# ilya16/MultINN

Measured on AMD Instinct MI355X. Metric: piano-roll timesteps/sec (train step), 5-track LSTM-NADE, higher is better.
Workload: dtype fp16; 1 GPU; TGT joint LSTM-NADE [1024,256,88,5]; global_batch=1024, per_gpu_batch=1024, seq_len=256, pitches=88, tracks=5, nade_hidden=256, optimizer=TF-Adam lr 0.01 eps 1e-4 clip 5.0, parallelism=dp1

## Files before the change

### include/multinn_hip.h

```cpp
#ifndef MULTINN_HIP_H
#define MULTINN_HIP_H

#include <stddef.h>
#include <stdint.h>

#ifdef __cplusplus
extern "C" {
#endif

#define MNN_OK 0
#define MNN_ERR_INVALID (-1)
#define MNN_ERR_HIP (-2)

typedef void* mnn_stream_t;

typedef enum { MNN_F32 = 0, MNN_BF16 = 1, MNN_U8 = 2, MNN_F16 = 3 } mnn_dtype;

enum { MNN_STREAM_DROPOUT = 0, MNN_STREAM_NADE = 1, MNN_STREAM_RBM_H = 2, MNN_STREAM_RBM_V = 3,
       MNN_STREAM_DBN_ENC = 4, MNN_STREAM_DBN_DEC = 5 };

#define MNN_ABI_VERSION 124
int mnn_version(void);
const char* mnn_last_error(void);

// ... 46 lines not shown
                     const void* wh_p, const float* gates, const float* c, const float* c0, float* dz,
                     void* dz_T , float* dh0, float* dc0, void* workspace, void* dzT_t, int ld_t,
                     float* db_p);

typedef struct { int units; const float* xproj; const void* wh_t; const void* h0; const float* c0; float* gates; float* c; void* h;
                 void* hT; int ld_hT; void* y; const uint8_t* mask; const void* wx_t; int ld_w; const float* bias_p;
                 void* yT; int ld_yT;
                 int xproj_bf16;
                 int f16;
               } mnn_lstm_fwd_layer;
typedef struct { int units; const float* dh_ext; const void* wh_p; const float* gates; const float* c; const float* c0; float* dz;
                 void* dz_T; void* workspace; void* dzT_t; int ld_t; float* db_p; const uint8_t* mask; const void* wx_p;
                 int f16;
               } mnn_lstm_bwd_layer;
int mnn_lstm2_seq_fwd(mnn_stream_t s, int T, int B, const mnn_lstm_fwd_layer* L1, const mnn_lstm_fwd_layer* L2, float keep_prob,
                      int s_begin, int s_end);
int mnn_lstm2_seq_bwd(mnn_stream_t s, int T, int B, const mnn_lstm_bwd_layer* L1, const mnn_lstm_bwd_layer* L2, float keep_prob,
                      int k_begin, int k_end);

int mnn_lstm2_persist_ok(int B, int units1, int units2);
int mnn_lstm_rows_gate_minor(mnn_stream_t s, int dtype, int units, int ld, const void* wx_t, const float* bias_p, void* wx_gm, float* bias_gm);
size_t mnn_lstm2_persist_workspace_bytes(int T, int B, int units1, int units2);
int mnn_lstm2_persist_status(const void* workspace, int B, int units1, int units2, int* status);
int mnn_lstm2_persist_fwd(mnn_stream_t s, int T, int B, const mnn_lstm_fwd_layer* L1, const mnn_lstm_fwd_layer* L2, float keep_prob,
                          void* workspace);
int mnn_lstm2_persist_bwd(mnn_stream_t s, int T, int B, const mnn_lstm_bwd_layer* L1, const mnn_lstm_bwd_layer* L2, float keep_prob,
                          void* workspace);
int mnn_lstm_rowpar_ok(int B, int units);
size_t mnn_lstm_rowpar_workspace_bytes(int T, int B, int units);
int mnn_lstm_rowpar_status(const void* workspace, int* status);
int mnn_lstm_rowpar_fwd(mnn_stream_t s, int T, int B, const mnn_lstm_fwd_layer* L, float keep_prob, void* workspace);
int mnn_lstm_rowpar_bwd(mnn_stream_t s, int T, int B, const mnn_lstm_bwd_layer* L, float keep_prob, void* workspace);
int mnn_lstm_resident_ok(int B, int units);
int mnn_lstm_resident_fwd(mnn_stream_t s, int T, int B, const mnn_lstm_fwd_layer* L, float keep_prob);
int mnn_lstm_resident_bwd(mnn_stream_t s, int T, int B, const mnn_lstm_bwd_layer* L, float keep_prob);
int mnn_lstm_resident_bwd_state(mnn_stream_t s, int T, int B, const mnn_lstm_bwd_layer* L, float keep_prob, float* dc0);
int mnn_lstm_cluster_ok(int B, int units);
int mnn_lstm_cluster_fwd(mnn_stream_t s, int T, int B, const mnn_lstm_fwd_layer* L, float keep_prob, void* workspace);
int mnn_lstm_cluster_bwd_ok(int B, int units);
int mnn_lstm_cluster_bwd(mnn_stream_t s, int T, int B, const mnn_lstm_bwd_layer* L, float keep_prob, void* workspace);
int mnn_lstm_cluster_bwd_state(mnn_stream_t s, int T, int B, const mnn_lstm_bwd_layer* L, float keep_prob, void* workspace, float* dc0);
int mnn_lstm_resident_fwd_multi(mnn_stream_t s, int T, int B, int njobs, const mnn_lstm_fwd_layer* L, float keep_prob);
int mnn_lstm_resident_bwd_multi(mnn_stream_t s, int T, int B, int njobs, const mnn_lstm_bwd_layer* L, float keep_prob);
int mnn_lstm_cluster_fwd_multi(mnn_stream_t s, int T, int B, int njobs, const mnn_lstm_fwd_layer* L, float keep_prob, void* const* workspaces);
int mnn_lstm_cluster_bwd_multi(mnn_stream_t s, int T, int B, int njobs, const mnn_lstm_bwd_layer* L, float keep_prob, void* const* workspaces);
int mnn_lstm_cluster_bwd_multi_ok(int B, int units, int njobs);
int mnn_lstm_resident_bwd_state_multi(mnn_stream_t s, int T, int B, int njobs, const mnn_lstm_bwd_layer* L, float keep_prob, float* const* dc0);
int mnn_lstm_cluster_bwd_state_multi(mnn_stream_t s, int T, int B, int njobs, const mnn_lstm_bwd_layer* L, float keep_prob, void* const* workspaces,
                                     float* const* dc0);
int mnn_dropout_mask(mnn_stream_t s, uint8_t* mask, int T, int B, int units, float keep_prob, uint64_t seed, const int32_t* step_dev,
                     uint32_t row0, int layer);

int mnn_dropout_fwd(mnn_stream_t s, int dtype, const void* h, void* y, int T, int B, int units, float keep_prob,
                    uint64_t seed, const int32_t* step_dev, uint32_t row0, int layer, int t_offset);
int mnn_dropout_bwd(mnn_stream_t s, const float* dy, float* dh, int T, int B, int units, float keep_prob, uint64_t seed,
                    const int32_t* step_dev, uint32_t row0, int layer, int accumulate, int t_offset);

int mnn_nade_mfma_ok(int Hn);
int mnn_nade_logprob_fwd_mfma(mnn_stream_t s, int tracks, int N, int D, int Hn, const uint8_t* v, long v_track_stride, const float* bias,
                              int ld_bias, const float* w_enc, const void* w_dec_bf16, const float* row_weight, float* nll, float* cond_p,
                              float* d_bias, float* a_final);
#define MNN_DENSITY_SLOTS 256
int mnn_density_gate(mnn_stream_t s, const uint8_t* v, long n, long threshold, int* gate, unsigned* count);
int mnn_nade_logprob_fwd_gated(mnn_stream_t s, int tracks, int N, int D, int Hn, const uint8_t* v, long v_track_stride,
                               const float* bias, int ld_bias, const float* w_enc, const float* w_dec, const float* row_weight,
                               float* nll, float* cond_p, float* d_bias, float* a_final, const int* gate, int run_if,
                               const int* n_rows_dev ,
                               int* unsafe );
int mnn_nade_logprob_fwd_mfma_gated(mnn_stream_t s, int tracks, int N, int D, int Hn, const uint8_t* v, long v_track_stride, const float* bias,
                                    int ld_bias, const float* w_enc, const void* w_dec_bf16, const float* row_weight, float* nll, float* cond_p,
                                    float* d_bias, float* a_final, const int* gate, int run_if, const int* n_rows_dev);
int mnn_nade_f32_pack(mnn_stream_t s, const float* w_dec, long rows, int Hn, float* w_dec_packed);
int mnn_nade_logprob_fwd_mfma_f32(mnn_stream_t s, int tracks, int N, int D, int Hn, const uint8_t* v, long v_track_stride, const float* bias,
                                  int ld_bias, const float* w_enc, const void* w_dec_packed, const float* row_weight, float* nll, float* cond_p,
                                  float* d_bias, float* a_final, const int* gate, int run_if, const int* n_rows_dev);

int mnn_nade_logprob_fwd(mnn_stream_t s, int tracks, int N, int D, int Hn, const uint8_t* v, long v_track_stride,
                         const float* bias, int ld_bias, const float* w_enc, const float* w_dec, const float* row_weight,
                         float* nll, float* cond_p, float* d_bias, float* a_final);
int mnn_nade_logprob_bwd(mnn_stream_t s, int tracks, int N, int D, int Hn, const uint8_t* v, long v_track_stride,
                         const float* bias, int ld_bias, const float* w_enc, const float* w_dec, const float* a_final,
                         float* d_bias, float* d_w_enc, float* d_w_dec, const int* n_rows_dev ,
                         const int* unsafe );
int mnn_nade_sample(mnn_stream_t s, int tracks, int N, int D, int Hn, const float* bias, int ld_bias, const float* w_enc,
                    const float* w_dec, float temperature, uint64_t seed, uint32_t row0, uint32_t sub, uint8_t* samples,
                    long s_track_stride, int s_row_stride, int s_elem_stride, float* nll, const uint8_t* given);
#define MNN_TEMPS_MAX 8
typedef struct {
    int n;
    int by_visible;
    float t[MNN_TEMPS_MAX];
} mnn_temps;
int mnn_nade_sample_temps(mnn_stream_t s, int tracks, int N, int D, int Hn, const float* bias, int ld_bias, const float* w_enc,
                          const float* w_dec, const mnn_temps* temps, uint64_t seed, uint32_t row0, uint32_t sub, uint8_t* samples,
                          long s_track_stride, int s_row_stride, int s_elem_stride, float* nll, const uint8_t* given);
typedef struct {
    const float* bias; int ld_bias;
    const float* w_enc; const float* w_dec;
    uint64_t seed;
    uint8_t* samples; float* nll;
    const uint8_t* given;
} mnn_nade_sample_job;
int mnn_nade_sample_multi(mnn_stream_t s, int njobs, const mnn_nade_sample_job* jobs, int N, int D, int Hn, float temperature,
                          uint32_t row0, uint32_t sub, long s_row_stride, int s_elem_stride);
int mnn_nade_sample_multi_temps(mnn_stream_t s, int njobs, const mnn_nade_sample_job* jobs, int N, int D, int Hn, const mnn_temps* temps,
                                uint32_t row0, uint32_t sub, long s_row_stride, int s_elem_stride);

size_t mnn_rbm_workspace_bytes(int D, int Hn);
int mnn_rbm_gibbs(mnn_stream_t s, int N, int D, int Hn, int k, const uint8_t* v0, const float* W, const float* bh, int ld_bh,
                  const float* bv, int ld_bv, uint64_t seed, uint32_t row0, const uint32_t* row_ids, uint32_t sub0,
                  float* p_v, uint8_t* v_out, void* workspace, const uint8_t* given, int ld_given);
int mnn_rbm_gibbs_temp(mnn_stream_t s, int N, int D, int Hn, int k, const uint8_t* v0, const float* W, const float* bh, int ld_bh,
                       const float* bv, int ld_bv, uint64_t seed, uint32_t row0, const uint32_t* row_ids, uint32_t sub0,
                       float* p_v, uint8_t* v_out, void* workspace, const uint8_t* given, int ld_given, float temperature);
int mnn_rbm_gibbs_stepped(mnn_stream_t s, int N, int D, int Hn, int k, const uint8_t* v0, const float* W, const float* bh, int ld_bh,
                  const float* bv, int ld_bv, uint64_t seed, uint32_t row0, const uint32_t* row_ids, uint32_t sub0,
                  float* p_v, uint8_t* v_out, void* workspace, const int* seed_step);
int mnn_rbm_hidden(mnn_stream_t s, int N, int D, int Hn, const void* v, int v_dtype, const float* W, const float* bh,
                   int ld_bh, int stream_id, uint64_t seed, uint32_t row0, uint32_t sub, float* p_h, uint8_t* h);
int mnn_rbm_visible(mnn_stream_t s, int N, int D, int Hn, const void* h, int h_dtype, const float* W, const float* bv,
                    int ld_bv, int stream_id, uint64_t seed, uint32_t row0, uint32_t sub, float* p_v, uint8_t* v,
                    void* workspace);
int mnn_rbm_free_energy(mnn_stream_t s, int N, int D, int Hn, const uint8_t* v, const float* W, const float* bh, int ld_bh,
                        const float* bv, int ld_bv, float* F, float* p_h );
typedef struct {
    const float* W;
    const float* bh;
    const float* bv;
    uint64_t seed;
    const uint8_t* v0;
    float* p_v;
    uint8_t* v_out;
    const uint8_t* given;
} mnn_rbm_gibbs_job;
int mnn_rbm_gibbs_multi(mnn_stream_t s, int njobs, const mnn_rbm_gibbs_job* jobs, int N, int D, int Hn, int k, int ld_bh, int ld_bv,
                        uint32_t row0, const uint32_t* row_ids, uint32_t sub0, const int* seed_step, long row_stride, int elem_stride,
                        long given_row_stride, void* workspace);
int mnn_rbm_gibbs_multi_temps(mnn_stream_t s, int njobs, const mnn_rbm_gibbs_job* jobs, int N, int D, int Hn, int k, int ld_bh, int ld_bv,
                              uint32_t row0, const uint32_t* row_ids, uint32_t sub0, const int* seed_step, long row_stride, int elem_stride,
                              long given_row_stride, void* workspace, const float* temps);
typedef struct {
    const uint8_t* v;
    const float* W;
    const float* bh;
    const float* bv;
    float* F;
    float* p_h;
} mnn_rbm_free_energy_job;
int mnn_rbm_free_energy_multi(mnn_stream_t s, int njobs, const mnn_rbm_free_energy_job* jobs, int N, int D, int Hn, int ld_bh, int ld_bv);
int mnn_rbm_cd_bias_delta(mnn_stream_t s, int N, int D, int Hn, const uint8_t* v, const float* p_v, const uint8_t* h, const float* p_h,
                          float scale, float* dbv, float* dbh);
int mnn_axpby_f32(mnn_stream_t s, long n, float a, const float* x, float b, const float* y, float* out);
int mnn_rbm_visible_bias_init(mnn_stream_t s, int D, const float* colsum, float count, float* bv);
int mnn_rbm_cd_rows(mnn_stream_t s, int N, int D, int Hn, int ld, const uint8_t* v, const uint8_t* v_s, const float* sv, const float* ss,
                    const float* row_weight, float scale, float* d_out, float* pos, float* neg);

size_t mnn_rbm_ais_workspace_bytes(int N, int D, int Hn, int n_chains, int n_betas);
int mnn_rbm_ais(mnn_stream_t s, int N, int D, int Hn, int n_chains, int n_betas, const float* betas, const float* W, const float* bh, int ld_bh,
                const float* bv, int ld_bv, uint64_t seed, uint32_t row0, const uint32_t* row_ids, float* log_z, float* log_w, uint8_t* v_out,
                float* stats, void* workspace);

int mnn_rbm_raise(mnn_stream_t s, int N, int D, int Hn, int n_chains, int n_betas, const float* betas, const float* W, const float* bh, int ld_bh,
                  const float* bv, int ld_bv, const uint8_t* v, uint64_t seed, uint32_t row0, const uint32_t* row_ids, float* log_z, float* log_w,
                  uint8_t* v_out, float* stats, void* workspace);

int mnn_sigmoid_grad_f32(mnn_stream_t s, long n, const float* dy, const float* y, float* dz);
// ... 76 lines not shown
```

### multinn_amd/_lib.py

```python
import ctypes as C
import os

HERE = os.path.dirname(os.path.abspath(__file__))
LIB_PATH = os.environ.get("MULTINN_HIP_LIB", os.path.join(HERE, "libmultinn_hip.so"))

ABI_VERSION = 124
F32, BF16, U8, F16 = 0, 1, 2, 3
GEMM_ACCUMULATE, GEMM_ATOMIC, GEMM_A_KBLOCK32 = 1, 2, 8

_p, _i, _l, _f, _u64, _u32, _sz = C.c_void_p, C.c_int, C.c_long, C.c_float, C.c_uint64, C.c_uint32, C.c_size_t

SIGNATURES = {
    "mnn_version": (_i, []),
    "mnn_last_error": (C.c_char_p, []),
    "mnn_gemm_tn": (_i, [_p, _i, _i, _i, _i, _p, _i, _p, _i, _p, _i, _i, _p, _i, _i]),
    "mnn_gemm_tn_rows": (_i, [_p, _i, _i, _i, _i, _p, _i, _p, _i, _p, _i, _i, _p, _i, _i, _p, _p]),
    "mnn_transpose": (_i, [_p, _p, _i, _i, _i, _i, _p, _i, _i]),
    "mnn_convert2d": (_i, [_p, _p, _i, _i, _p, _i, _i, _i, _i]),
    "mnn_pianoroll_shift_timemajor": (_i, [_p, _p, _i, _i, _i, _p, _p, _i, _i, _p, _p, _l]),
    "mnn_pianoroll_shift_timemajor_t": (_i, [_p, _p, _i, _i, _i, _p, _p, _i, _p, _i, _p, _p, _l, _i, _p, _p, _p]),
    "mnn_ragged_index": (_i, [_p, _p, _i, _i, _p, _f, _p, _p, _p]),
    "mnn_rows_gather16": (_i, [_p, _p, _i, _p, _p, _i, _i, _p, _i, _p, _i]),
    "mnn_rows_scatter_f32": (_i, [_p, _p, _p, _p, _i, _i, _p]),
    "mnn_pianoroll_split_tracks": (_i, [_p, _p, _i, _i, _i, _i, _p]),
    "mnn_lstm_pack_weights": (_i, [_p, _p, _p, _i, _i, _i, _i, _p, _p, _p, _p, _p]),
    "mnn_lstm_unpack_grads": (_i, [_p, _p, _p, _p, _i, _i, _i, _p, _p]),
    "mnn_lstm_unpack_grads_consume": (_i, [_p, _p, _p, _p, _i, _i, _i, _p, _p]),
    "mnn_lstm_unpack_grads_cat": (_i, [_p, _p, _p, _i, _i, _i, _p, _p]),
    "mnn_lstm_seq_fwd": (_i, [_p, _i, _i, _i, _i, _i, _i, _p, _p, _p, _p, _p, _p, _p, _p, _i]),
    "mnn_lstm_fused_outputs": (_i, [_i, _i]),
    "mnn_lstm_seq_bwd_workspace_bytes": (_sz, [_i, _i]),
    "mnn_lstm_seq_bwd": (_i, [_p, _i, _i, _i, _i, _i, _i, _p, _p, _p, _p, _p, _p, _p, _p, _p, _p, _p, _i, _p]),
    "mnn_dropout_fwd": (_i, [_p, _i, _p, _p, _i, _i, _i, _f, _u64, _p, _u32, _i, _i]),
    "mnn_dropout_bwd": (_i, [_p, _p, _p, _i, _i, _i, _f, _u64, _p, _u32, _i, _i, _i]),
    "mnn_nade_logprob_fwd": (_i, [_p, _i, _i, _i, _i, _p, _l, _p, _i, _p, _p, _p, _p, _p, _p, _p]),
    "mnn_nade_logprob_bwd": (_i, [_p, _i, _i, _i, _i, _p, _l, _p, _i, _p, _p, _p, _p, _p, _p, _p, _p]),
    "mnn_nade_sample": (_i, [_p, _i, _i, _i, _i, _p, _i, _p, _p, _f, _u64, _u32, _u32, _p, _l, _i, _i, _p, _p]),
    "mnn_rbm_workspace_bytes": (_sz, [_i, _i]),
    "mnn_rbm_gibbs": (_i, [_p, _i, _i, _i, _i, _p, _p, _p, _i, _p, _i, _u64, _u32, _p, _u32, _p, _p, _p, _p, _i]),
    "mnn_rbm_gibbs_stepped": (_i, [_p, _i, _i, _i, _i, _p, _p, _p, _i, _p, _i, _u64, _u32, _p, _u32, _p, _p, _p, _p]),
    "mnn_rbm_hidden": (_i, [_p, _i, _i, _i, _p, _i, _p, _p, _i, _i, _u64, _u32, _u32, _p, _p]),
    "mnn_rbm_visible": (_i, [_p, _i, _i, _i, _p, _i, _p, _p, _i, _i, _u64, _u32, _u32, _p, _p, _p]),
    "mnn_rbm_free_energy": (_i, [_p, _i, _i, _i, _p, _p, _p, _i, _p, _i, _p, _p]),
    "mnn_sumsq": (_i, [_p, _p, _l, _p]),
    "mnn_weighted_sum": (_i, [_p, _p, _p, _l, _p]),
    "mnn_clip_adam_step": (_i, [_p, _p, _p, _p, _p, _l, _p, _f, _f, _f, _f, _f, _i, _p, _i, _p]),
    "mnn_step_increment": (_i, [_p, _p, _p, _f, _p, _p, _i]),
    "mnn_bias_grad": (_i, [_p, _p, _i, _i, _i, _p, _i]),
    "mnn_grad_rows_fanout": (_i, [_p, _p, _i, _i, _i, _i, _p, _i, _p, _i, _p, _i]),
    "mnn_fill_f32": (_i, [_p, _p, _l, _f]),
    "mnn_lstm_step_det": (_i, [_p, _i, _i, _p]),
    "mnn_dense_det": (_i, [_p, _i, _i, _p]),
    "mnn_nade_sample_multi": (_i, [_p, _i, _p, _i, _i, _i, _f, _u32, _u32, _l, _i]),
    "mnn_generate_scan_workspace_bytes": (_sz, [_i, _i, _i, _p, _i]),
    "mnn_det_lstm_pack_bytes": (_sz, [_i, _i]),
    "mnn_det_lstm_pack": (_i, [_p, _p, _i, _i, _p]),
    "mnn_det_dense_pack_bytes": (_sz, [_i, _i]),
    "mnn_det_dense_pack": (_i, [_p, _p, _i, _i, _i, _p]),
    "mnn_generate_scan": (_i, [_p, _i, _i, _i, _p, _i, _i, _p, _p, _p, _i, _i, _i, _i, _p, _p, _f, _u64, _u32, _p, _p, _sz, _p]),
    "mnn_generate_scan_state": (_i, [_p, _i, _i, _i, _p, _i, _i, _p, _p, _p, _i, _i, _i, _i, _p, _p, _f, _u64, _u32, _p, _p, _sz, _p,
                                     C.POINTER(C.c_void_p), C.POINTER(C.c_void_p)]),
    "mnn_comm_unique_id": (_i, [_p]),
    "mnn_comm_init": (_i, [C.POINTER(_p), _i, _i, _p]),
    "mnn_allreduce_flat": (_i, [_p, _p, _p, _l]),
    "mnn_comm_destroy": (_i, [_p]),
}

class DetLstmJob(C.Structure):
    _fields_ = [("x", _p), ("x_dtype", _i), ("n_x", _i), ("ld_x", _i), ("es_x", _i), ("x2", _p), ("n_x2", _i), ("ld_x2", _i), ("h_prev", _p), ("c_prev", _p),
                ("W", _p), ("bias", _p), ("c_out", _p), ("h_out", _p), ("units", _i), ("Wp", _p)]


class NadeSampleJob(C.Structure):
    _fields_ = [("bias", _p), ("ld_bias", _i), ("w_enc", _p), ("w_dec", _p), ("seed", _u64), ("samples", _p), ("nll", _p), ("given", _p)]


class Temps(C.Structure):
    _fields_ = [("n", _i), ("by_visible", _i), ("t", _f * 8)]


class RbmGibbsJob(C.Structure):
    _fields_ = [("W", _p), ("bh", _p), ("bv", _p), ("seed", _u64), ("v0", _p), ("p_v", _p), ("v_out", _p), ("given", _p)]


class RbmFreeEnergyJob(C.Structure):
    _fields_ = [("v", _p), ("W", _p), ("bh", _p), ("bv", _p), ("F", _p), ("p_h", _p)]


class ScanLstmLayer(C.Structure):
    _fields_ = [("W", _p), ("bias", _p), ("units", _i)]


class DetDenseJob(C.Structure):
    _fields_ = [("x", _p), ("ld_x", _i), ("K", _i), ("W", _p), ("ld_w", _i), ("N", _i), ("bias", _p), ("out", _p), ("ld_out", _i), ("Wp", _p)]


class LstmFwdLayer(C.Structure):
    _fields_ = [("units", _i), ("xproj", _p), ("wh_t", _p), ("h0", _p), ("c0", _p), ("gates", _p), ("c", _p), ("h", _p), ("hT", _p), ("ld_hT", _i), ("y", _p), ("mask", _p),
                ("wx_t", _p), ("ld_w", _i), ("bias_p", _p), ("yT", _p), ("ld_yT", _i), ("xproj_bf16", _i), ("f16", _i)]


class LstmBwdLayer(C.Structure):
    _fields_ = [("units", _i), ("dh_ext", _p), ("wh_p", _p), ("gates", _p), ("c", _p), ("c0", _p), ("dz", _p), ("dz_T", _p), ("workspace", _p),
                ("dzT_t", _p), ("ld_t", _i), ("db_p", _p), ("mask", _p), ("wx_p", _p), ("f16", _i)]


SIGNATURES["mnn_lstm2_seq_fwd"] = (_i, [_p, _i, _i, C.POINTER(LstmFwdLayer), C.POINTER(LstmFwdLayer), _f, _i, _i])
SIGNATURES["mnn_lstm2_seq_bwd"] = (_i, [_p, _i, _i, C.POINTER(LstmBwdLayer), C.POINTER(LstmBwdLayer), _f, _i, _i])
SIGNATURES["mnn_lstm_rows_gate_minor"] = (_i, [_p, _i, _i, _i, _p, _p, _p, _p])
SIGNATURES["mnn_lstm2_persist_ok"] = (_i, [_i, _i, _i])
SIGNATURES["mnn_lstm2_persist_workspace_bytes"] = (_sz, [_i, _i, _i, _i])
SIGNATURES["mnn_lstm2_persist_status"] = (_i, [_p, _i, _i, _i, C.POINTER(C.c_int)])
SIGNATURES["mnn_lstm2_persist_fwd"] = (_i, [_p, _i, _i, C.POINTER(LstmFwdLayer), C.POINTER(LstmFwdLayer), _f, _p])
SIGNATURES["mnn_lstm2_persist_bwd"] = (_i, [_p, _i, _i, C.POINTER(LstmBwdLayer), C.POINTER(LstmBwdLayer), _f, _p])
SIGNATURES["mnn_lstm_rowpar_ok"] = (_i, [_i, _i])
SIGNATURES["mnn_lstm_rowpar_workspace_bytes"] = (_sz, [_i, _i, _i])
SIGNATURES["mnn_lstm_rowpar_status"] = (_i, [_p, C.POINTER(C.c_int)])
SIGNATURES["mnn_lstm_rowpar_fwd"] = (_i, [_p, _i, _i, C.POINTER(LstmFwdLayer), _f, _p])
SIGNATURES["mnn_lstm_rowpar_bwd"] = (_i, [_p, _i, _i, C.POINTER(LstmBwdLayer), _f, _p])
SIGNATURES["mnn_lstm_resident_ok"] = (_i, [_i, _i])
SIGNATURES["mnn_lstm_resident_fwd"] = (_i, [_p, _i, _i, C.POINTER(LstmFwdLayer), _f])
SIGNATURES["mnn_lstm_resident_bwd"] = (_i, [_p, _i, _i, C.POINTER(LstmBwdLayer), _f])
SIGNATURES["mnn_lstm_cluster_ok"] = (_i, [_i, _i])
SIGNATURES["mnn_lstm_cluster_bwd_ok"] = (_i, [_i, _i])
SIGNATURES["mnn_lstm_cluster_bwd_multi_ok"] = (_i, [_i, _i, _i])
SIGNATURES["mnn_lstm_resident_fwd_multi"] = (_i, [_p, _i, _i, _i, C.POINTER(LstmFwdLayer), _f])
SIGNATURES["mnn_lstm_resident_bwd_multi"] = (_i, [_p, _i, _i, _i, C.POINTER(LstmBwdLayer), _f])
SIGNATURES["mnn_lstm_cluster_fwd_multi"] = (_i, [_p, _i, _i, _i, C.POINTER(LstmFwdLayer), _f, C.POINTER(C.c_void_p)])
SIGNATURES["mnn_lstm_cluster_bwd_multi"] = (_i, [_p, _i, _i, _i, C.POINTER(LstmBwdLayer), _f, C.POINTER(C.c_void_p)])
SIGNATURES["mnn_lstm_cluster_fwd"] = (_i, [_p, _i, _i, C.POINTER(LstmFwdLayer), _f, _p])
SIGNATURES["mnn_lstm_cluster_bwd"] = (_i, [_p, _i, _i, C.POINTER(LstmBwdLayer), _f, _p])
SIGNATURES["mnn_lstm_resident_bwd_state"] = (_i, [_p, _i, _i, C.POINTER(LstmBwdLayer), _f, _p])
SIGNATURES["mnn_lstm_cluster_bwd_state"] = (_i, [_p, _i, _i, C.POINTER(LstmBwdLayer), _f, _p, _p])
SIGNATURES["mnn_lstm_resident_bwd_state_multi"] = (_i, [_p, _i, _i, _i, C.POINTER(LstmBwdLayer), _f, C.POINTER(C.c_void_p)])
SIGNATURES["mnn_lstm_cluster_bwd_state_multi"] = (_i, [_p, _i, _i, _i, C.POINTER(LstmBwdLayer), _f, C.POINTER(C.c_void_p), C.POINTER(C.c_void_p)])
SIGNATURES["mnn_nade_mfma_ok"] = (_i, [_i])
SIGNATURES["mnn_nade_logprob_fwd_mfma"] = (_i, [_p, _i, _i, _i, _i, _p, _l, _p, _i, _p, _p, _p, _p, _p, _p, _p])
SIGNATURES["mnn_density_gate"] = (_i, [_p, _p, _l, _l, _p, _p])
SIGNATURES["mnn_nade_logprob_fwd_gated"] = (_i, [_p, _i, _i, _i, _i, _p, _l, _p, _i, _p, _p, _p, _p, _p, _p, _p, _p, _i, _p, _p])
SIGNATURES["mnn_nade_logprob_fwd_mfma_gated"] = (_i, [_p, _i, _i, _i, _i, _p, _l, _p, _i, _p, _p, _p, _p, _p, _p, _p, _p, _i, _p])
SIGNATURES["mnn_nade_logprob_fwd_mfma_f32"] = (_i, [_p, _i, _i, _i, _i, _p, _l, _p, _i, _p, _p, _p, _p, _p, _p, _p, _p, _i, _p])
SIGNATURES["mnn_nade_f32_pack"] = (_i, [_p, _p, _l, _i, _p])
SIGNATURES["mnn_musical_bar_stats"] = (_i, [_p, _p, _i, _i, _i, _i, _i, _p, _p, _p, _p, _p, _p, _p, _p])
SIGNATURES["mnn_musical_note_stats"] = (_i, [_p, _p, _i, _i, _i, _i, _i, _p, _p])
SIGNATURES["mnn_eval_counts"] = (_i, [_p, _p, _p, _l, _p])
SIGNATURES["mnn_log_loss_rows"] = (_i, [_p, _p, _p, _i, _i, _i, _p])
SIGNATURES["mnn_rbm_cd_bias_delta"] = (_i, [_p, _i, _i, _i, _p, _p, _p, _p, _f, _p, _p])
SIGNATURES["mnn_rbm_visible_bias_init"] = (_i, [_p, _i, _p, _f, _p])
SIGNATURES["mnn_sigmoid_grad_f32"] = (_i, [_p, _l, _p, _p, _p])
SIGNATURES["mnn_rbm_ais_workspace_bytes"] = (_sz, [_i, _i, _i, _i, _i])
SIGNATURES["mnn_rbm_ais"] = (_i, [_p, _i, _i, _i, _i, _i, _p, _p, _p, _i, _p, _i, _u64, _u32, _p, _p, _p, _p, _p, _p])
SIGNATURES["mnn_rbm_raise"] = (_i, [_p, _i, _i, _i, _i, _i, _p, _p, _p, _i, _p, _i, _p, _u64, _u32, _p, _p, _p, _p, _p, _p])
SIGNATURES["mnn_rbm_gibbs_multi"] = (_i, [_p, _i, _p, _i, _i, _i, _i, _i, _i, _u32, _p, _u32, _p, _l, _i, _l, _p])
SIGNATURES["mnn_rbm_free_energy_multi"] = (_i, [_p, _i, _p, _i, _i, _i, _i, _i])
SIGNATURES["mnn_rbm_cd_rows"] = (_i, [_p, _i, _i, _i, _i, _p, _p, _p, _p, _p, _f, _p, _p, _p])
SIGNATURES["mnn_probe_sigmoid"] = (_i, [_p, _i, _i, _p])
SIGNATURES["mnn_axpby_f32"] = (_i, [_p, _l, _f, _p, _f, _p, _p])
SIGNATURES["mnn_dropout_mask"] = (_i, [_p, _p, _i, _i, _i, _f, _u64, _p, _u32, _i])
SIGNATURES["mnn_nade_sample_temps"] = (_i, [_p, _i, _i, _i, _i, _p, _i, _p, _p, _p, _u64, _u32, _u32, _p, _l, _i, _i, _p, _p])
SIGNATURES["mnn_nade_sample_multi_temps"] = (_i, [_p, _i, _p, _i, _i, _i, _p, _u32, _u32, _l, _i])
SIGNATURES["mnn_generate_scan_temps"] = (_i, [_p, _i, _i, _i, _p, _i, _i, _p, _p, _p, _i, _i, _i, _i, _p, _p, _p, _u64, _u32, _p, _p, _sz, _p,
                                              C.POINTER(C.c_void_p), C.POINTER(C.c_void_p)])
SIGNATURES["mnn_rbm_gibbs_temp"] = (_i, [_p, _i, _i, _i, _i, _p, _p, _p, _i, _p, _i, _u64, _u32, _p, _u32, _p, _p, _p, _p, _i, _f])
SIGNATURES["mnn_rbm_gibbs_multi_temps"] = (_i, [_p, _i, _p, _i, _i, _i, _i, _i, _i, _u32, _p, _u32, _p, _l, _i, _l, _p, C.POINTER(C.c_float)])
TEMPS_MAX = 8

_lib = None


class MnnError(RuntimeError):
    pass


class MnnUnsupported(MnnError, NotImplementedError):
    """A request this build has no path for (e.g. conditional generation of a model that does not live on a ROCm device): caught by both
    `except MnnError` and `except NotImplementedError`."""


def load():
    global _lib
    if _lib is not None:
        return _lib
    if not os.path.exists(LIB_PATH):
        raise MnnError(f"{LIB_PATH} is missing: run `python -c 'import __graft_entry__ as g; g.build()'` "
                       "(multinn_amd has no CPU fallback)")
    lib = C.CDLL(LIB_PATH)
    for name, (res, args) in SIGNATURES.items():
        fn = getattr(lib, name)
        fn.restype, fn.argtypes = res, args
    if lib.mnn_version() != ABI_VERSION:
        raise MnnError(f"{LIB_PATH} has ABI version {lib.mnn_version()}, this loader binds {ABI_VERSION} (include/multinn_hip.h): rebuild it")
    _lib = lib
    return lib


def check(rc, what=""):
    if rc != 0:
        raise MnnError(f"{what} failed ({rc}): {load().mnn_last_error().decode()}")


TIMING = None


def call(name, *args):
    lib = load()
    if TIMING is not None:
        import torch
        e0, e1 = torch.cuda.Event(enable_timing=True), torch.cuda.Event(enable_timing=True)
        e0.record()
        rc = getattr(lib, name)(*args)
        e1.record()
        TIMING.setdefault(name, []).append((e0, e1))
    else:
        rc = getattr(lib, name)(*args)
    if rc != 0:
        raise MnnError(f"{name} failed ({rc}): {lib.mnn_last_error().decode()}")
```

### multinn_amd/csrc/nade.hip

```cpp
#include "common.h"

#define NADE_EPS 1e-6f
#define LN2 0.6931471805599453f

__device__ __forceinline__ float fast_ln(float x) { return __builtin_amdgcn_logf(x) * LN2; }

__device__ __forceinline__ bool nade_rows_beyond(const int* __restrict__ n_rows_dev, int first_row) {
    return n_rows_dev != nullptr && first_row >= *n_rows_dev;
}
__device__ __forceinline__ void nade_zero_rows(float* __restrict__ d_bias, int ld_bias, int col0, int ncol, int row0, int nrow, int N, int nthreads) {
    if (d_bias == nullptr) return;
    for (int e = threadIdx.x; e < nrow * ncol; e += nthreads) {
        const int n = e / ncol, i = e - n * ncol;
        if (row0 + n < N) d_bias[(size_t)(row0 + n) * ld_bias + col0 + i] = 0.f;
    }
}

__device__ __forceinline__ float dpp_xor8(float x) { return __int_as_float(__builtin_amdgcn_update_dpp(0, __float_as_int(x), 0x128, 0xf, 0xf, false)); }
__device__ __forceinline__ float swz_xor4(float x) { return __int_as_float(__builtin_amdgcn_ds_swizzle(__float_as_int(x), 0x101F)); }
__device__ __forceinline__ float dpp_xor4(float x) {
    int t = __builtin_amdgcn_update_dpp(0, __float_as_int(x), 0x104, 0xf, 0x5, false);
    t = __builtin_amdgcn_update_dpp(t, __float_as_int(x), 0x114, 0xf, 0xa, false);
    return __int_as_float(t);
}
__device__ __forceinline__ float dpp_xor2(float x) { return __int_as_float(__builtin_amdgcn_update_dpp(0, __float_as_int(x), 0x4E, 0xf, 0xf, false)); }
__device__ __forceinline__ float dpp_xor1(float x) { return __int_as_float(__builtin_amdgcn_update_dpp(0, __float_as_int(x), 0xB1, 0xf, 0xf, false)); }

__device__ __forceinline__ float rows8(float (&x)[8], int lane) {
#pragma unroll
    for (int k = 0; k < 4; ++k) {
        auto r = __builtin_amdgcn_permlane32_swap(__float_as_uint(x[k]), __float_as_uint(x[k + 4]), false, false);
        x[k] = __uint_as_float(r[0]) + __uint_as_float(r[1]);
    }
#pragma unroll
    for (int k = 0; k < 2; ++k) {
        auto r = __builtin_amdgcn_permlane16_swap(__float_as_uint(x[k]), __float_as_uint(x[k + 2]), false, false);
        x[k] = __uint_as_float(r[0]) + __uint_as_float(r[1]);
    }
    const float t = x[0] + dpp_xor8(x[0]), u = x[1] + dpp_xor8(x[1]);
    return (lane & 8) ? u : t;
}
__device__ __forceinline__ float vis8(float (&y)[8], int lane) {
    const bool b2 = lane & 4, b1 = lane & 2, b0 = lane & 1;
#pragma unroll
    for (int k = 0; k < 4; ++k) {
        const float t = y[k] + swz_xor4(y[k]), u = y[k + 4] + swz_xor4(y[k + 4]);
        y[k] = b2 ? u : t;
    }
#pragma unroll
    for (int k = 0; k < 2; ++k) {
        const float t = y[k] + dpp_xor2(y[k]), u = y[k + 2] + dpp_xor2(y[k + 2]);
        y[k] = b1 ? u : t;
    }
    const float t = y[0] + dpp_xor1(y[0]), u = y[1] + dpp_xor1(y[1]);
    return b0 ? u : t;
}

#define FWD_R 8
template <int HQ>
struct WStage {
    static constexpr int W = HQ * 64;
    static constexpr int NE = (8 * W) / 512;
    float rd[NE], re[NE];
    __device__ __forceinline__ void gload(const float* __restrict__ wd, const float* __restrict__ we, int i0, int D, int Hn, int ld = 0) {
        if (ld == 0) ld = Hn;
#pragma unroll
        for (int k = 0; k < NE; ++k) {
            const int e = threadIdx.x + k * 512;
            const int ii = e / W, j = e - ii * W, i = i0 + ii;
            const bool ok = i >= 0 && i < D && j < Hn;
            const size_t o = (size_t)min(max(i, 0), D - 1) * ld + min(j, Hn - 1);
            const float xd = wd[o], xe = we[o];
            rd[k] = ok ? xd : 0.f;
            re[k] = ok ? xe : 0.f;
        }
    }
    __device__ __forceinline__ void lstore(float* __restrict__ sd, float* __restrict__ se) const {
#pragma unroll
        for (int k = 0; k < NE; ++k) {
            sd[threadIdx.x + k * 512] = rd[k];
            se[threadIdx.x + k * 512] = re[k];
        }
    }
};

template <int HQ, bool UT>
__global__ void __launch_bounds__(512)
nade_fwd_kernel(int tracks, int N, int D, int Hn, const uint8_t* __restrict__ v, long v_track_stride, const float* __restrict__ bias,
                int ld_bias, const float* __restrict__ w_enc, const float* __restrict__ w_dec, const float* __restrict__ row_weight,
                float* __restrict__ nll, float* __restrict__ cond_p, float* __restrict__ d_bias, float* __restrict__ a_final,
                const int* __restrict__ gate, int run_if, const int* __restrict__ n_rows_dev, int* __restrict__ unsafe) {
    constexpr int W = HQ * 64;
    __shared__ float wl[2][2][8 * W];
    if (gate != nullptr && *gate != run_if) {
        if (unsafe != nullptr && blockIdx.x == 0 && blockIdx.y == 0 && threadIdx.x == 0) atomicAdd(unsafe, 1);
        return;
    }
    const int m = blockIdx.y;
    if (nade_rows_beyond(n_rows_dev, blockIdx.x * 64)) {
        nade_zero_rows(d_bias, ld_bias, tracks * Hn + m * D, D, blockIdx.x * 64, 64, N, 512);
        if (nll != nullptr && threadIdx.x < 64 && blockIdx.x * 64 + threadIdx.x < N) nll[(size_t)m * N + blockIdx.x * 64 + threadIdx.x] = 0.f;
        return;
    }
    const int lane = threadIdx.x & 63;
    const int w = __builtin_amdgcn_readfirstlane(threadIdx.x >> 6);
    const int rbase = blockIdx.x * 64 + w * FWD_R;
    const uint8_t* __restrict__ vm = v + (size_t)m * v_track_stride;
    const float* __restrict__ we = w_enc + (size_t)m * D * Hn;
    const float* __restrict__ wd = w_dec + (size_t)m * D * Hn;
    const int bd_off = tracks * Hn + m * D;

    float a[FWD_R][HQ], h[FWD_R][HQ];
#pragma unroll
    for (int r = 0; r < FWD_R; ++r)
#pragma unroll
        for (int q = 0; q < HQ; ++q)
            a[r][q] = bias[(size_t)min(rbase + r, N - 1) * ld_bias + m * Hn + min(lane + 64 * q, Hn - 1)];
#pragma unroll
    for (int r = 0; r < FWD_R; ++r)
#pragma unroll
        for (int q = 0; q < HQ; ++q) {
            const int j = lane + 64 * q, row = rbase + r;
            if (!(row < N && j < Hn)) a[r][q] = 0.f;
            h[r][q] = fast_sigmoid(a[r][q]);
        }
    float u[UT ? FWD_R : 1][UT ? HQ : 1];
    float amax = 0.f;
    bool passed40 = false;
    if constexpr (UT) {
#pragma unroll
        for (int r = 0; r < FWD_R; ++r)
#pragma unroll
            for (int q = 0; q < HQ; ++q) {
                u[r][q] = fast_exp2(-MNN_LOG2E * a[r][q]);
                amax = fmaxf(amax, fabsf(a[r][q]));
            }
    }
    const int frow = rbase + (lane >> 3), fi = lane & 7;
    const bool fvalid = frow < N;
    const int frr = fvalid ? frow : N - 1;
    const float rw = (row_weight != nullptr && fvalid) ? row_weight[frow] : 0.f;
    float lp = 0.f;

    WStage<HQ> st;
    st.gload(wd, we, 0, D, Hn);
    st.lstore(wl[0][0], wl[0][1]);
    bool vcur = fvalid && fi < D && vm[(size_t)frr * D + fi] != 0;
    float bcur = fi < D ? bias[(size_t)frr * ld_bias + bd_off + fi] : 0.f;
    __syncthreads();
    const int nch = (D + 7) / 8;
    for (int c = 0; c < nch; ++c) {
        const int i0 = c * 8;
        const int inext = i0 + 8 + fi;
        st.gload(wd, we, i0 + 8, D, Hn);
        const int inc = min(inext, D - 1);
        const uint8_t vraw = vm[(size_t)frr * D + inc];
        const float braw = bias[(size_t)frr * ld_bias + bd_off + inc];
        const unsigned long long mask = __ballot(vcur);
        const float* __restrict__ sd = wl[c & 1][0];
        const float* __restrict__ se = wl[c & 1][1];
        float y[8];
#pragma unroll
        for (int ii = 0; ii < 8; ++ii) {
            float wdv[HQ], pr[8];
#pragma unroll
            for (int q = 0; q < HQ; ++q) wdv[q] = sd[ii * W + lane + 64 * q];
            if constexpr (UT) {
                const bool any = (mask & (0x0101010101010101ull << ii)) != 0ull;
                float wev[HQ], ewv[HQ];
                if (any) {
#pragma unroll
                    for (int q = 0; q < HQ; ++q) {
                        wev[q] = se[ii * W + lane + 64 * q];
                        ewv[q] = fast_exp2(-MNN_LOG2E * wev[q]);
                    }
                }
#pragma unroll
                for (int r = 0; r < FWD_R; ++r) {
                    float acc = h[r][0] * wdv[0];
#pragma unroll
                    for (int q = 1; q < HQ; ++q) acc = fmaf(h[r][q], wdv[q], acc);
                    pr[r] = acc;
                    if ((mask >> (r * 8 + ii)) & 1ull) {
#pragma unroll
                        for (int q = 0; q < HQ; ++q) {
                            a[r][q] += wev[q];
                            u[r][q] *= ewv[q];
                            h[r][q] = fast_rcp(1.0f + u[r][q]);
                            amax = fmaxf(amax, fabsf(a[r][q]));
                        }
                    }
                }
                if (any && __any(amax > 40.0f)) {
                    amax = 0.f;
                    passed40 = true;
#pragma unroll
                    for (int r = 0; r < FWD_R; ++r)
#pragma unroll
                        for (int q = 0; q < HQ; ++q) {
                            u[r][q] = fast_exp2(-MNN_LOG2E * a[r][q]);
                            h[r][q] = fast_rcp(1.0f + u[r][q]);
                        }
                }
            } else {
#pragma unroll
                for (int r = 0; r < FWD_R; ++r) {
                    float acc = h[r][0] * wdv[0];
#pragma unroll
                    for (int q = 1; q < HQ; ++q) acc = fmaf(h[r][q], wdv[q], acc);
                    pr[r] = acc;
                    if ((mask >> (r * 8 + ii)) & 1ull) {
#pragma unroll
                        for (int q = 0; q < HQ; ++q) {
                            a[r][q] += se[ii * W + lane + 64 * q];
                            h[r][q] = fast_sigmoid(a[r][q]);
                        }
                    }
                }
            }
            y[ii] = rows8(pr, lane);
        }
        const float tot = vis8(y, lane);
        const int i = i0 + fi;
        if (i < D) {
            const float l = bcur + tot;
            const float pr = fast_sigmoid(l);
            const float qr = fast_sigmoid(-l);
            lp += vcur ? fast_ln(NADE_EPS + pr) : fast_ln(NADE_EPS + qr);
            if (fvalid) {
                if (cond_p != nullptr) cond_p[((size_t)m * N + frow) * D + i] = pr;
                if (d_bias != nullptr) {
                    const float dnll_dp = vcur ? -fast_rcp(NADE_EPS + pr) : fast_rcp(NADE_EPS + qr);
                    d_bias[(size_t)frow * ld_bias + bd_off + i] = rw * dnll_dp * pr * qr;
                }
            }
        }
        st.lstore(wl[(c + 1) & 1][0], wl[(c + 1) & 1][1]);
        vcur = fvalid && inext < D && vraw != 0;
        bcur = inext < D ? braw : 0.f;
        __syncthreads();
    }
    lp += dpp_xor1(lp);
    lp += dpp_xor2(lp);
    lp += swz_xor4(lp);
    if (fi == 0 && fvalid && nll != nullptr) nll[(size_t)m * N + frow] = -lp;
    if (a_final != nullptr) {
#pragma unroll
        for (int r = 0; r < FWD_R; ++r)
#pragma unroll
            for (int q = 0; q < HQ; ++q) {
                const int j = lane + 64 * q, row = rbase + r;
                if (row < N && j < Hn) a_final[((size_t)m * N + row) * Hn + j] = a[r][q];
            }
    }
    if (unsafe != nullptr) {
        const bool ok = UT ? !__any(passed40 || amax > 40.0f) : !(blockIdx.x == 0 && blockIdx.y == 0 && w == 0);
        if (!ok && lane == 0) atomicAdd(unsafe, 1);
    }
}

extern "C" int mnn_nade_logprob_fwd(mnn_stream_t s, int tracks, int N, int D, int Hn, const uint8_t* v, long v_track_stride,
                                    const float* bias, int ld_bias, const float* w_enc, const float* w_dec, const float* row_weight,
                                    float* nll, float* cond_p, float* d_bias, float* a_final) {
    return mnn_nade_logprob_fwd_gated(s, tracks, N, D, Hn, v, v_track_stride, bias, ld_bias, w_enc, w_dec, row_weight, nll, cond_p, d_bias, a_final,
                                      nullptr, 0, nullptr, nullptr);
}

extern "C" int mnn_nade_logprob_fwd_gated(mnn_stream_t s, int tracks, int N, int D, int Hn, const uint8_t* v, long v_track_stride,
                                          const float* bias, int ld_bias, const float* w_enc, const float* w_dec, const float* row_weight,
                                          float* nll, float* cond_p, float* d_bias, float* a_final, const int* gate, int run_if, const int* n_rows_dev,
                                          int* unsafe) {
    MNN_REQUIRE(tracks > 0 && N > 0 && D > 0 && Hn > 0 && Hn <= 256, "mnn_nade_logprob_fwd: need tracks,N,D>0 and 0<Hn<=256 (Hn=%d)", Hn);
    MNN_REQUIRE(v && bias && w_enc && w_dec, "mnn_nade_logprob_fwd: null pointer");
    MNN_REQUIRE(ld_bias >= tracks * (Hn + D), "mnn_nade_logprob_fwd: ld_bias %d < tracks*(Hn+D)", ld_bias);
    MNN_REQUIRE(d_bias == nullptr || row_weight != nullptr, "mnn_nade_logprob_fwd: d_bias needs row_weight");
    dim3 grid(cdiv(N, 64), tracks);
    hipStream_t st = (hipStream_t)s;
#define FWD(HQ, UT) hipLaunchKernelGGL((nade_fwd_kernel<HQ, UT>), grid, dim3(512), 0, st, tracks, N, D, Hn, v, v_track_stride, bias, ld_bias, w_enc, \
                                       w_dec, row_weight, nll, cond_p, d_bias, a_final, gate, run_if, n_rows_dev, unsafe)
    if (unsafe != nullptr) MNN_HIP(mnn_zero_async(unsafe, sizeof(int), sizeof(int), 1, st));
    static const bool no_ut = getenv("MNN_NADE_FWD_NO_UT") != nullptr;
    if (Hn <= 64) FWD(1, false);
    else if (Hn <= 128) FWD(2, false);
    else if (gate != nullptr && run_if == 1 && !no_ut) FWD(4, true);
    else FWD(4, false);
#undef FWD
    MNN_LAUNCH_CHECK();
    return MNN_OK;
}

template <int HQ> struct LaneVec;
template <> struct LaneVec<2> { typedef float2 T; };
template <> struct LaneVec<4> { typedef float4 T; };
template <int HQ>
__device__ __forceinline__ void lv_store(float* p, const float (&x)[HQ]) {
    if constexpr (HQ == 4) *reinterpret_cast<float4*>(p) = make_float4(x[0], x[1], x[2], x[3]);
    else *reinterpret_cast<float2*>(p) = make_float2(x[0], x[1]);
}
template <int HQ>
__device__ __forceinline__ void lv_load(const float* p, float (&x)[HQ]) {
    if constexpr (HQ == 4) { const float4 t = *reinterpret_cast<const float4*>(p); x[0] = t.x; x[1] = t.y; x[2] = t.z; x[3] = t.w; }
    else { const float2 t = *reinterpret_cast<const float2*>(p); x[0] = t.x; x[1] = t.y; }
}
template <int HQ>
__device__ __forceinline__ void bwd_gload(WStage<HQ>& st, const float* __restrict__ wd, const float* __restrict__ we, int i0, int D, int Hn, int ld) {
    if constexpr (HQ >= 2) {
        const int i = i0 + (int)__builtin_amdgcn_readfirstlane(threadIdx.x >> 6), l = threadIdx.x & 63;
        const int ic = min(max(i, 0), D - 1);
        const float* __restrict__ pd = wd + (size_t)ic * ld;
        const float* __restrict__ pe = we + (size_t)ic * ld;
#pragma unroll
        for (int q = 0; q < HQ; ++q) {
            const int col = min(l + 64 * q, Hn - 1);
            st.rd[q] = pd[col];
            st.re[q] = pe[col];
        }
    } else {
        st.gload(wd, we, i0, D, Hn, ld);
    }
}
template <int HQ>
__device__ __forceinline__ void bwd_lstore(const WStage<HQ>& st, float* __restrict__ sd, float* __restrict__ se) {
    if constexpr (HQ >= 2) {
        const int pos = (int)(threadIdx.x >> 6) * (64 * HQ) + HQ * (int)(threadIdx.x & 63);
        lv_store<HQ>(sd + pos, st.rd);
        lv_store<HQ>(se + pos, st.re);
    } else {
        st.lstore(sd, se);
    }
}

template <int HQ, int RG, bool USEU>
__global__ void __launch_bounds__(512)
nade_bwd_kernel(int tracks, int N, int D, int HnT, int nslice, const uint8_t* __restrict__ v, long v_track_stride, const float* __restrict__ bias,
                int ld_bias, const float* __restrict__ w_enc, const float* __restrict__ w_dec, const float* __restrict__ a_final,
                float* __restrict__ d_bias, float* __restrict__ d_w_enc, float* __restrict__ d_w_dec, const int* __restrict__ n_rows_dev,
                const int* __restrict__ unsafe) {
    constexpr int W = HQ * 64;
    __shared__ __attribute__((aligned(16))) float wl[2][2][8 * W];
    if (unsafe != nullptr && (*unsafe == 0) != USEU) return;
    constexpr int NRED = HQ <= 2 ? 2 : 1;
    __shared__ __attribute__((aligned(16))) float red_[NRED][8][4][2][W];
    const int m = blockIdx.y / nslice, hb = (blockIdx.y - m * nslice) * W;
    const int Hn = min(W, HnT - hb);
    if (nade_rows_beyond(n_rows_dev, blockIdx.x * (64 * RG))) {
        nade_zero_rows(d_bias, ld_bias, m * HnT + hb, Hn, blockIdx.x * (64 * RG), 64 * RG, N, 512);
        return;
    }
    const int Nv = n_rows_dev != nullptr ? min(*n_rows_dev, N) : N;
    const int lane = threadIdx.x & 63;
    const int w = __builtin_amdgcn_readfirstlane(threadIdx.x >> 6);
    constexpr int BWD_R = 8 * RG;
    const int rbase = blockIdx.x * (64 * RG) + w * BWD_R;
    const uint8_t* __restrict__ vm = v + (size_t)m * v_track_stride;
    const float* __restrict__ we = w_enc + (size_t)m * D * HnT + hb;
    const float* __restrict__ wd = w_dec + (size_t)m * D * HnT + hb;
    const int dl_off = tracks * HnT + m * D;

    constexpr bool useu = USEU;
    float a[BWD_R][HQ], h[BWD_R][HQ], c[BWD_R][HQ], G[BWD_R][HQ];
#pragma unroll
    for (int r = 0; r < BWD_R; ++r)
#pragma unroll
        for (int q = 0; q < HQ; ++q)
            a[r][q] = a_final[((size_t)m * N + min(rbase + r, N - 1)) * HnT + hb + min(lane + 64 * q, Hn - 1)];
#pragma unroll
    for (int r = 0; r < BWD_R; ++r)
#pragma unroll
        for (int q = 0; q < HQ; ++q) {
            const int j = lane + 64 * q, row = rbase + r;
            if (!(row < Nv && j < Hn)) a[r][q] = 0.f;
            h[r][q] = fast_sigmoid(a[r][q]);
            if constexpr (useu) a[r][q] = fast_exp2(-MNN_LOG2E * a[r][q]);
            G[r][q] = 0.f;
            c[r][q] = 0.f;
        }
    const int fi = lane & 7;
    int frr[RG];
    bool fvalid[RG];
#pragma unroll
    for (int g = 0; g < RG; ++g) {
        const int frow = rbase + 8 * g + (lane >> 3);
        fvalid[g] = frow < N;
        frr[g] = fvalid[g] ? frow : N - 1;
    }
    const int nch = (D + 7) / 8;
    WStage<HQ> st;
    bwd_gload<HQ>(st, wd, we, (nch - 1) * 8, D, Hn, HnT);
    bwd_lstore<HQ>(st, wl[0][0], wl[0][1]);
    const int icur = (nch - 1) * 8 + fi;
    bool vcur[RG];
    float dcur[RG];
#pragma unroll
    for (int g = 0; g < RG; ++g) {
        vcur[g] = fvalid[g] && icur < D && vm[(size_t)frr[g] * D + icur] != 0;
        dcur[g] = (fvalid[g] && icur < D) ? d_bias[(size_t)frr[g] * ld_bias + dl_off + icur] : 0.f;
    }
    __syncthreads();
    for (int cc = 0; cc < nch; ++cc) {
        const int i0 = (nch - 1 - cc) * 8;
        const int inext = i0 - 8 + fi;
        bwd_gload<HQ>(st, wd, we, i0 - 8, D, Hn, HnT);
        uint8_t vraw[RG];
        float draw[RG];
        unsigned long long mask[RG], many = 0ull;
        const int inc = max(inext, 0);
#pragma unroll
        for (int g = 0; g < RG; ++g) {
            vraw[g] = vm[(size_t)frr[g] * D + inc];
            draw[g] = d_bias[(size_t)frr[g] * ld_bias + dl_off + inc];
            mask[g] = __ballot(vcur[g]);
            many |= mask[g];
        }
        const float* __restrict__ sd = wl[cc & 1][0];
        const float* __restrict__ se = wl[cc & 1][1];
#pragma unroll
        for (int half = 1; half >= 0; --half) {
            float accd[4][HQ], acce[4][HQ];
#pragma unroll
            for (int k = 3; k >= 0; --k) {
                const int ii = half * 4 + k;
                const int i = i0 + ii;
#pragma unroll
                for (int q = 0; q < HQ; ++q) { accd[k][q] = 0.f; acce[k][q] = 0.f; }
                if (i >= D) continue;
                float wev[HQ], wdv[HQ];
                if constexpr (HQ >= 2) {
                    lv_load<HQ>(sd + ii * W + HQ * lane, wdv);
                    lv_load<HQ>(se + ii * W + HQ * lane, wev);
// ... 35 lines not shown
                                    h[r][q] = fast_sigmoid(a[r][q]);
                                }
                            }
                        }
                    }
                }
#pragma unroll
                for (int r = 0; r < BWD_R; ++r) {
                    const float dl = __int_as_float(__builtin_amdgcn_readlane(__float_as_int(dcur[r >> 3]), (r & 7) * 8 + ii));
#pragma unroll
                    for (int q = 0; q < HQ; ++q) {
                        accd[k][q] = fmaf(dl, h[r][q], accd[k][q]);
                        c[r][q] = fmaf(dl, wdv[q], c[r][q]);
                    }
                }
            }
            if (half == 1) bwd_lstore<HQ>(st, wl[(cc + 1) & 1][0], wl[(cc + 1) & 1][1]);
            float (*red)[4][2][W] = red_[(2 * cc + 1 - half) & (NRED - 1)];
            if (NRED == 1) __syncthreads();
            if constexpr (HQ >= 2) {
#pragma unroll
                for (int k = 0; k < 4; ++k) {
                    lv_store<HQ>(&red[w][k][0][HQ * lane], accd[k]);
                    lv_store<HQ>(&red[w][k][1][HQ * lane], acce[k]);
                }
                __syncthreads();
                {
                    const int k = threadIdx.x >> 7, which = (threadIdx.x >> 6) & 1;
                    const int i = i0 + half * 4 + k;
                    float sum[HQ];
#pragma unroll
                    for (int q = 0; q < HQ; ++q) sum[q] = 0.f;
#pragma unroll
                    for (int ww = 0; ww < 8; ++ww) {
                        float pq[HQ];
                        lv_load<HQ>(&red[ww][k][which][HQ * lane], pq);
#pragma unroll
                        for (int q = 0; q < HQ; ++q) sum[q] += pq[q];
                    }
                    if (i < D) {
                        float* dst = (which == 0 ? d_w_dec : d_w_enc) + ((size_t)m * D + i) * HnT + hb + lane;
#ifdef NADE_BWD_NO_ATOMIC
                        if (sum[0] == 1.2345e30f) dst[0] = sum[0];
#else
#pragma unroll
                        for (int q = 0; q < HQ; ++q)
                            if (lane + 64 * q < Hn) atomicAdd(dst + 64 * q, sum[q]);
#endif
                    }
                }
            } else {
#pragma unroll
                for (int k = 0; k < 4; ++k)
#pragma unroll
                    for (int q = 0; q < HQ; ++q) {
                        red[w][k][0][lane + 64 * q] = accd[k][q];
                        red[w][k][1][lane + 64 * q] = acce[k][q];
                    }
                __syncthreads();
                for (int e = threadIdx.x; e < 4 * 2 * W; e += 512) {
                    const int k = e / (2 * W), which = (e / W) & 1, j = e % W;
                    const int i = i0 + half * 4 + k;
                    if (j < Hn && i < D) {
                        float sum = 0.f;
#pragma unroll
                        for (int ww = 0; ww < 8; ++ww) sum += red[ww][k][which][j];
                        atomicAdd((which == 0 ? d_w_dec : d_w_enc) + ((size_t)m * D + i) * HnT + hb + j, sum);
                    }
                }
            }
        }
#pragma unroll
        for (int g = 0; g < RG; ++g) {
            const bool ok = fvalid[g] && inext >= 0;
            vcur[g] = ok && vraw[g] != 0;
            dcur[g] = ok ? draw[g] : 0.f;
        }
        if (NRED == 1) __syncthreads();
    }
#pragma unroll
    for (int r = 0; r < BWD_R; ++r)
#pragma unroll
        for (int q = 0; q < HQ; ++q) G[r][q] = fmaf(c[r][q], fmaf(-h[r][q], h[r][q], h[r][q]), G[r][q]);
#pragma unroll
    for (int r = 0; r < BWD_R; ++r)
#pragma unroll
        for (int q = 0; q < HQ; ++q) {
            const int j = lane + 64 * q, row = rbase + r;
            if (row < N && j < Hn) __builtin_nontemporal_store(G[r][q], &d_bias[(size_t)row * ld_bias + m * HnT + hb + j]);
        }
}

extern "C" int mnn_nade_logprob_bwd(mnn_stream_t s, int tracks, int N, int D, int Hn, const uint8_t* v, long v_track_stride,
                                    const float* bias, int ld_bias, const float* w_enc, const float* w_dec, const float* a_final,
                                    float* d_bias, float* d_w_enc, float* d_w_dec, const int* n_rows_dev, const int* unsafe) {
    MNN_REQUIRE(tracks > 0 && N > 0 && D > 0 && Hn > 0 && Hn <= 256, "mnn_nade_logprob_bwd: need tracks,N,D>0 and 0<Hn<=256 (Hn=%d)", Hn);
    MNN_REQUIRE(v && bias && w_enc && w_dec && a_final && d_bias && d_w_enc && d_w_dec, "mnn_nade_logprob_bwd: null pointer");
    MNN_REQUIRE(ld_bias >= tracks * (Hn + D), "mnn_nade_logprob_bwd: ld_bias too small");
    hipStream_t st = (hipStream_t)s;
#define BWD(HQ, NS, U, S) hipLaunchKernelGGL((nade_bwd_kernel<HQ, 1, U>), dim3(cdiv(N, 64), tracks * (NS)), dim3(512), 0, st, tracks, N, D, Hn, NS, v, \
                                             v_track_stride, bias, ld_bias, w_enc, w_dec, a_final, d_bias, d_w_enc, d_w_dec, n_rows_dev, S)
    if (Hn <= 64) BWD(1, 1, false, nullptr);
    else {
        if (unsafe != nullptr) BWD(2, cdiv(Hn, 128), true, unsafe);
        BWD(2, cdiv(Hn, 128), false, unsafe);
    }
#undef BWD
    MNN_LAUNCH_CHECK();
    return MNN_OK;
}

__device__ __forceinline__ float wave_xor_sum(float x) {
    {
        auto r = __builtin_amdgcn_permlane32_swap(__float_as_uint(x), __float_as_uint(x), false, false);
        x = __uint_as_float(r[0]) + __uint_as_float(r[1]);
    }
    {
        auto r = __builtin_amdgcn_permlane16_swap(__float_as_uint(x), __float_as_uint(x), false, false);
        x = __uint_as_float(r[0]) + __uint_as_float(r[1]);
    }
    x = x + dpp_xor8(x);
    x = x + dpp_xor4(x);
    x = x + dpp_xor2(x);
    x = x + dpp_xor1(x);
    return x;
}

__device__ __forceinline__ float sig_approx(float x) {
    return __builtin_amdgcn_rcpf(1.0f + __builtin_amdgcn_exp2f(-x * 1.4426950408889634f));
}
__device__ __forceinline__ bool draw_below(float u, float x) {
    const float r = sig_approx(x);
    const float d = u - r;
    if (__builtin_amdgcn_ballot_w64(fabsf(d) > 1e-4f * r + 1e-30f) != 0ull) return __builtin_amdgcn_ballot_w64(d < 0.f) != 0ull;
    return __builtin_amdgcn_ballot_w64(u < det_sigmoid(x)) != 0ull;
}
__device__ __forceinline__ bool prob_at_least_half(float x) {
    const float d = sig_approx(x) - 0.5f;
    if (__builtin_amdgcn_ballot_w64(fabsf(d) > 1e-4f) != 0ull) return __builtin_amdgcn_ballot_w64(d > 0.f) != 0ull;
    return __builtin_amdgcn_ballot_w64(det_sigmoid(x) >= 0.5f) != 0ull;
}

struct SampleJob {
    const float* bias; int ld_bias; int enc_off, dec_off;
    const float* w_enc; const float* w_dec;
    uint64_t seed; uint32_t elem0;
    uint8_t* samples; float* nll;
    const uint8_t* given;
};
#define SAMPLE_MAX_JOBS 8
struct SampleJobs { SampleJob job[SAMPLE_MAX_JOBS]; };
struct SampleTemps { float t[SAMPLE_MAX_JOBS]; int n; int by_visible; };
__device__ __forceinline__ void sample_temps_park(const SampleTemps& TT, int lane, float* stt) {
    float tv = TT.t[0];
#pragma unroll
    for (int k = 1; k < SAMPLE_MAX_JOBS; ++k) tv = (lane & (SAMPLE_MAX_JOBS - 1)) == k ? TT.t[k] : tv;
    if (lane < SAMPLE_MAX_JOBS) stt[lane] = tv;
}

template <int TMODE, bool FULL, bool SPEC, bool GIVEN>
__global__ void __launch_bounds__(256)
nade_sample_kernel(SampleJobs J, int N, int D, int Hn, SampleTemps TT, uint32_t row0, uint32_t sub, long s_row_stride, int s_elem_stride) {
    extern __shared__ __attribute__((aligned(16))) unsigned char nade_sample_smem[];
    const SampleJob& jb = J.job[blockIdx.y];
    const float* __restrict__ bias = jb.bias;
    const int ld_bias = jb.ld_bias;
    const uint64_t seed = jb.seed;
    uint8_t* __restrict__ samples = jb.samples;
    float* __restrict__ nll = jb.nll;
    const int lane = threadIdx.x & 63, wv = threadIdx.x >> 6;
    const int row = blockIdx.x * 4 + wv;
    if (row >= N) return;
    const int Dp = (D + 3) & ~3;
    float* sp = reinterpret_cast<float*>(nade_sample_smem) + (size_t)wv * Dp;
    float* sbd = reinterpret_cast<float*>(nade_sample_smem) + (size_t)(4 + wv) * Dp;
    unsigned char* son = nade_sample_smem + (size_t)32 * Dp + (size_t)wv * Dp;
    float* su = reinterpret_cast<float*>(nade_sample_smem + (size_t)36 * Dp) + wv * 256;
    unsigned char* sg = nade_sample_smem + (size_t)36 * Dp + 4096 + (size_t)wv * Dp;
    float* stt = reinterpret_cast<float*>(nade_sample_smem + (size_t)36 * Dp + 4096 + (GIVEN ? (size_t)4 * Dp : 0));
    const float* __restrict__ we = jb.w_enc;
    const float* __restrict__ wd = jb.w_dec;
    const float* __restrict__ bd = bias + (size_t)row * ld_bias + jb.dec_off;
    float a[4], h[4];
    bool in[4];
// ... 488 lines not shown
```

### multinn_amd/csrc/nade_mfma.hip

```cpp
#include "common.h"
typedef float nm_f4 __attribute__((ext_vector_type(4)));
#define NM_ST4(dst, a) __builtin_nontemporal_store((nm_f4){a[0], a[1], a[2], a[3]}, reinterpret_cast<nm_f4*>(dst))
#define NM_ST1(dst, x) __builtin_nontemporal_store((float)(x), dst)
#include <algorithm>
#include <type_traits>

typedef __bf16 bf16x8_t __attribute__((ext_vector_type(8)));
typedef float f32x4_t __attribute__((ext_vector_type(4)));
typedef __attribute__((address_space(1))) const void* gas_ptr_t;
typedef __attribute__((address_space(3))) void* lds_ptr_t;

#ifdef NM_TRACE
__device__ long long nm_trace[16];
#define NM_T(k) do { if (tid == 0 && blockIdx.x == NM_TRACE) { const long long now_ = wall_clock64(); nm_trace[k] += now_ - tprev_; tprev_ = now_; } } while (0)
#else
#define NM_T(k) do { } while (0)
#endif
#define NADE_EPS 1e-6f
#define LN2F 0.6931471805599453f
#define NM_H 256
#define NM_PITCH 264
#define NM_LP 36

__device__ __forceinline__ void lds_barrier() { asm volatile("s_waitcnt lgkmcnt(0)\n\ts_barrier" ::: "memory"); }

__device__ __forceinline__ float nm_ln(float x) { return __builtin_amdgcn_logf(x) * LN2F; }

typedef _Float16 f16x8_t __attribute__((ext_vector_type(8)));
struct NmPairB { f16x8_t hi, lo; };
template <bool SPLIT> struct NmState;
template <> struct NmState<false> { typedef bf16_t T; static constexpr int PITCH = NM_PITCH; };
template <> struct NmState<true> { typedef unsigned T; static constexpr int PITCH = 260; };
__device__ __forceinline__ unsigned nm_pack_hl(float x) {
    const float hi = __uint_as_float(__float_as_uint(x) & 0xFFFFE000u);
    return __builtin_bit_cast(unsigned, __builtin_amdgcn_cvt_pkrtz(hi, x - hi));
}

template <bool SPLIT>
struct NadeFwdSmemT {
    float sA[SPLIT ? 1 : 32][NM_H];
    typename NmState<SPLIT>::T sH[32][NmState<SPLIT>::PITCH];
    typename NmState<SPLIT>::T sF[32][NmState<SPLIT>::PITCH];
    float sLb[32][NM_LP];
    float sLf[32][NM_LP];
    unsigned sMask[2][32];
    unsigned sSb[2][33];
    unsigned short sFl[2][1024];
    unsigned short sPs[2][34];
    unsigned sAct[2][32];
};

__device__ __forceinline__ void nm_load_a(const bf16_t (*tile)[NM_PITCH], int mi, int lane, bf16x8_t (&a)[8]) {
    const bf16_t* p = &tile[16 * mi + (lane & 15)][8 * (lane >> 4)];
#pragma unroll
    for (int s = 0; s < 8; ++s) a[s] = *reinterpret_cast<const bf16x8_t*>(p + 32 * s);
}
template <bool SPLIT> __device__ __forceinline__ typename NmState<SPLIT>::T nm_state(float h) {
    if constexpr (SPLIT) return nm_pack_hl(h);
    else return f32_to_bf16(h);
}
__device__ __forceinline__ f32x4_t nm_dot(const bf16x8_t (&af)[8], const bf16x8_t (&bfr)[8]) {
    f32x4_t acc = {0.f, 0.f, 0.f, 0.f};
#pragma unroll
    for (int s = 0; s < 8; ++s) acc = __builtin_amdgcn_mfma_f32_16x16x32_bf16(af[s], bfr[s], acc, 0, 0, 0);
    return acc;
}
__device__ __forceinline__ f32x4_t nm_dot_hl(const unsigned (*tile)[260], int mi, int lane, const NmPairB (&bw)[8]) {
    const unsigned* p = &tile[16 * mi + (lane & 15)][8 * (lane >> 4)];
    f32x4_t accm = {0.f, 0.f, 0.f, 0.f}, accs = {0.f, 0.f, 0.f, 0.f};
#pragma unroll
    for (int s = 0; s < 8; ++s) {
        const uint4 q0 = *reinterpret_cast<const uint4*>(p + 32 * s), q1 = *reinterpret_cast<const uint4*>(p + 32 * s + 4);
        uint4 uh, ul;
        uh.x = __builtin_amdgcn_perm(q0.y, q0.x, 0x05040100u); ul.x = __builtin_amdgcn_perm(q0.y, q0.x, 0x07060302u);
        uh.y = __builtin_amdgcn_perm(q0.w, q0.z, 0x05040100u); ul.y = __builtin_amdgcn_perm(q0.w, q0.z, 0x07060302u);
        uh.z = __builtin_amdgcn_perm(q1.y, q1.x, 0x05040100u); ul.z = __builtin_amdgcn_perm(q1.y, q1.x, 0x07060302u);
        uh.w = __builtin_amdgcn_perm(q1.w, q1.z, 0x05040100u); ul.w = __builtin_amdgcn_perm(q1.w, q1.z, 0x07060302u);
        const f16x8_t ah = __builtin_bit_cast(f16x8_t, uh), al = __builtin_bit_cast(f16x8_t, ul);
        accs = __builtin_amdgcn_mfma_f32_16x16x32_f16(ah, bw[s].lo, accs, 0, 0, 0);
        accm = __builtin_amdgcn_mfma_f32_16x16x32_f16(ah, bw[s].hi, accm, 0, 0, 0);
        accs = __builtin_amdgcn_mfma_f32_16x16x32_f16(al, bw[s].hi, accs, 0, 0, 0);
    }
    return accm + accs;
}
template <bool SPLIT, typename Tile, typename B>
__device__ __forceinline__ void nm_logit_tile(const Tile& tile, int w, int lane, const B& bfr, float (*out)[NM_LP]) {
    const int ni = w >> 1, mi = w & 1;
    f32x4_t acc;
    if constexpr (SPLIT) {
        acc = nm_dot_hl(tile, mi, lane, bfr);
    } else {
        bf16x8_t af[8];
        nm_load_a(tile, mi, lane, af);
        acc = nm_dot(af, bfr);
    }
#pragma unroll
    for (int i = 0; i < 4; ++i) out[16 * mi + 4 * (lane >> 4) + i][16 * ni + (lane & 15)] = acc[i];
}

template <bool SPLIT>
__device__ __forceinline__ void
nade_fwd_mfma_body(int tracks, int N, int D, const uint8_t* __restrict__ v, long v_track_stride, const float* __restrict__ bias, int ld_bias,
                     const float* __restrict__ w_enc, const bf16_t* __restrict__ w_dec_bf, const float* __restrict__ row_weight,
                     float* __restrict__ nll, float* __restrict__ cond_p, float* __restrict__ d_bias, float* __restrict__ a_final,
                     const int* __restrict__ gate, int run_if, const int* __restrict__ n_rows_dev) {
    extern __shared__ __attribute__((aligned(16))) char smem_raw[];
    typedef NadeFwdSmemT<SPLIT> NadeFwdSmem;
    typedef typename NmState<SPLIT>::T state_t;
    typedef typename std::conditional<SPLIT, NmPairB, bf16x8_t>::type bfrag_t;
    constexpr int KS = 8;
    NadeFwdSmem& S = *reinterpret_cast<NadeFwdSmem*>(smem_raw);
    if (gate != nullptr && *gate != run_if) return;
    constexpr int Hn = NM_H;
    const int m = blockIdx.y;
    const int tid = threadIdx.x, lane = tid & 63, w = __builtin_amdgcn_readfirstlane(tid >> 6);
    const int ni = w >> 1;
    const int rb = blockIdx.x * 32;
    const uint8_t* __restrict__ vm = v + (size_t)m * v_track_stride;
    const float* __restrict__ we = w_enc + (size_t)m * D * Hn;
    const bf16_t* __restrict__ wd = w_dec_bf + (size_t)m * D * Hn * (SPLIT ? 2 : 1);
    const int bd_off = tracks * Hn + m * D;
    const int ntile = (D + 31) / 32;
    if (n_rows_dev != nullptr && rb >= *n_rows_dev) {
        if (d_bias != nullptr)
            for (int e = tid; e < 32 * D; e += 256) {
                const int n = e / D, i = e - n * D;
                if (rb + n < N) d_bias[(size_t)(rb + n) * ld_bias + bd_off + i] = 0.f;
            }
        if (nll != nullptr && tid < 32 && rb + tid < N) nll[(size_t)m * N + rb + tid] = 0.f;
        return;
    }

    float areg[SPLIT ? 32 : 1];
    {
        float av[32];
#pragma unroll
        for (int n = 0; n < 32; ++n) av[n] = bias[(size_t)min(rb + n, N - 1) * ld_bias + m * Hn + tid];
#pragma unroll
        for (int n = 0; n < 32; ++n) {
            const float x = rb + n < N ? av[n] : 0.f;
            if constexpr (SPLIT) areg[n] = x;
            else S.sA[n][tid] = x;
            S.sH[n][tid] = nm_state<SPLIT>(fast_sigmoid(x));
        }
    }
    auto load_v = [&](int c, unsigned char (&vb)[4]) {
#pragma unroll
        for (int i = 0; i < 4; ++i) {
            const int row = min(rb + 8 * w + 2 * i + (lane >> 5), N - 1), dd = min(32 * c + (lane & 31), D - 1);
            vb[i] = vm[(size_t)row * D + dd];
        }
    };
    auto ballots = [&](int c, const unsigned char (&vb)[4], unsigned (&msk)[32]) {
#pragma unroll
        for (int i = 0; i < 4; ++i) {
            const int row = rb + 8 * w + 2 * i + (lane >> 5), dd = 32 * c + (lane & 31);
            const unsigned long long bal = __ballot(row < N && dd < D && vb[i] != 0);
            if (lane == 0) { msk[8 * w + 2 * i] = (unsigned)bal; msk[8 * w + 2 * i + 1] = (unsigned)(bal >> 32); }
        }
    };
    auto build_list = [&](int buf) {
        if (w == 0) {
            const unsigned mk = lane < 32 ? S.sMask[buf][lane] : 0u;
            const int cnt = __popc(mk);
            unsigned rest = mk;
            int base = 0;
            for (int j = 0; j < 32; ++j) {
                const unsigned act = (unsigned)__ballot(cnt > j);
                if (lane == 0) { S.sPs[buf][j] = (unsigned short)base; S.sAct[buf][j] = act; }
                if (act == 0u) break;
                if (cnt > j) {
                    const int pos = base + __popc(act & ((1u << lane) - 1u));
                    const int dpos = __builtin_ctz(rest);
                    rest &= rest - 1;
                    S.sFl[buf][pos] = (unsigned short)((lane << 5) | dpos);
                }
                base += __popc(act);
            }
            if (lane == 0) S.sSb[buf][32] = (unsigned)base;
        }
    };
    auto load_b = [&](int c, bfrag_t (&b)[KS]) {
        const int d = min(32 * c + 16 * ni + (lane & 15), D - 1);
        if constexpr (SPLIT) {
            const f16_t* p = reinterpret_cast<const f16_t*>(wd) + (size_t)d * 2 * Hn + 8 * (lane >> 4);
#pragma unroll
            for (int s = 0; s < KS; ++s) {
                b[s].hi = *reinterpret_cast<const f16x8_t*>(p + 32 * s);
                b[s].lo = *reinterpret_cast<const f16x8_t*>(p + Hn + 32 * s);
            }
        } else {
            const bf16_t* p = wd + (size_t)d * Hn + 8 * (lane >> 4);
#pragma unroll
            for (int s = 0; s < KS; ++s) b[s] = *reinterpret_cast<const bf16x8_t*>(p + 32 * s);
        }
    };
    const __amdgpu_buffer_rsrc_t we_rs = __builtin_amdgcn_make_buffer_rsrc(const_cast<float*>(we), 0, D * Hn * 4, 0x00020000);
    auto load_we = [&](int c, int buf, int k0, float (&wv)[32]) {
        const int F = (int)S.sSb[buf][32];
        const int entv = (int)S.sFl[buf][(k0 + (lane & 31) < F) ? k0 + (lane & 31) : 0];
#pragma unroll
        for (int u = 0; u < 32; ++u) {
            const int e = __builtin_amdgcn_readlane(entv, u);
            wv[u] = __builtin_bit_cast(float, __builtin_amdgcn_raw_buffer_load_b32(we_rs, tid * 4, min(32 * c + (e & 31), D - 1) * (Hn * 4), 0));
        }
    };
    unsigned char vb[4];
    bfrag_t bfr[KS];
    float wev[32];
    load_v(0, vb);
    load_b(0, bfr);
    ballots(0, vb, S.sMask[0]);
    if (ntile > 1) load_v(1, vb);
    __syncthreads();
    build_list(0);
    __syncthreads();
    load_we(0, 0, 0, wev);

    const int en = tid >> 3, ed0 = 4 * (tid & 7), erow = rb + en;
    const bool evalid = erow < N;
    const int err = evalid ? erow : N - 1;
    const float rw = (row_weight != nullptr && evalid) ? row_weight[erow] : 0.f;
    float lp = 0.f;
#ifdef NM_TRACE
    long long tprev_ = wall_clock64();
#endif
    for (int c = 0; c < ntile; ++c) {
        const int buf = c & 1, nbuf = buf ^ 1;
        float bdec[4];
        {
            const float* bp = bias + (size_t)err * ld_bias + bd_off + 32 * c + ed0;
            if (32 * c + ed0 + 3 < D && (((size_t)bp) & 15) == 0) {
                const float4 b4 = *reinterpret_cast<const float4*>(bp);
                bdec[0] = b4.x; bdec[1] = b4.y; bdec[2] = b4.z; bdec[3] = b4.w;
            } else {
#pragma unroll
                for (int k = 0; k < 4; ++k) bdec[k] = bias[(size_t)err * ld_bias + bd_off + min(32 * c + ed0 + k, D - 1)];
            }
        }
        __builtin_amdgcn_sched_barrier(0);
        nm_logit_tile<SPLIT>(S.sH, w, lane, bfr, S.sLb);
        if (c + 1 < ntile) {
            ballots(c + 1, vb, S.sMask[nbuf]);
            if (c + 2 < ntile) load_v(c + 2, vb);
        }
        NM_T(0);
        lds_barrier();
        NM_T(1);
        const int F = (int)S.sSb[buf][32];
        const unsigned mk = S.sMask[buf][en];
        float lsel[4];
        int jj[4];
#pragma unroll
        for (int k = 0; k < 4; ++k) {
            jj[k] = __popc(mk & ((1u << (ed0 + k)) - 1u));
            lsel[k] = S.sLb[en][ed0 + k];
        }
        int slot_of[4];
#pragma unroll
        for (int k = 0; k < 4; ++k) {
            const int pj = max(jj[k] - 1, 0);
            slot_of[k] = jj[k] > 0 ? (int)S.sPs[buf][pj] + __popc(S.sAct[buf][pj] & ((1u << en) - 1u)) : -1;
        }
        for (int k0 = 0; k0 < F; k0 += 32) {
            if (k0 > 0) load_we(c, buf, k0, wev);
            const int cnt = min(32, F - k0);
            const int flv = (int)S.sFl[buf][min(k0 + (lane & 31), F - 1)];
#pragma unroll
            for (int u0 = 0; u0 < 32; u0 += 8) {
                if (u0 < cnt) {
                    int n[8];
#pragma unroll
                    for (int i = 0; i < 8; ++i) n[i] = __builtin_amdgcn_readlane(flv, u0 + i) >> 5;
                    if constexpr (SPLIT) {
                        float x[8];
#pragma unroll
                        for (int i = 0; i < 8; ++i) {
                            x[i] = areg[n[i]] + ((u0 + i < cnt) ? wev[u0 + i] : 0.f);
                            areg[n[i]] = x[i];
                        }
                        state_t hb[8];
#pragma unroll
                        for (int i = 0; i < 8; ++i) hb[i] = nm_state<SPLIT>(fast_sigmoid(x[i]));
#pragma unroll
                        for (int i = 0; i < 8; ++i) {
                            if (u0 + i < cnt) {
                                S.sF[u0 + i][tid] = hb[i];
                                S.sH[n[i]][tid] = hb[i];
                            }
                        }
                    } else {
                        bool indep = u0 + 8 <= cnt;
#pragma unroll
                        for (int i = 0; i < 7; ++i) indep = indep && n[i] < n[i + 1];
                        if (indep) {
                            float x[8];
#pragma unroll
                            for (int i = 0; i < 8; ++i) x[i] = S.sA[n[i]][tid];
#pragma unroll
                            for (int i = 0; i < 8; ++i) x[i] += wev[u0 + i];
                            state_t hb[8];
#pragma unroll
                            for (int i = 0; i < 8; ++i) hb[i] = nm_state<SPLIT>(fast_sigmoid(x[i]));
#pragma unroll
                            for (int i = 0; i < 8; ++i) {
                                S.sA[n[i]][tid] = x[i];
                                S.sF[u0 + i][tid] = hb[i];
                                S.sH[n[i]][tid] = hb[i];
                            }
                        } else {
#pragma unroll
                            for (int i = 0; i < 8; ++i) {
                                if (u0 + i < cnt) {
                                    const float av = S.sA[n[i]][tid] + wev[u0 + i];
                                    S.sA[n[i]][tid] = av;
                                    const state_t hb1 = nm_state<SPLIT>(fast_sigmoid(av));
                                    S.sF[u0 + i][tid] = hb1;
                                    S.sH[n[i]][tid] = hb1;
                                }
                            }
                        }
                    }
                }
            }
            NM_T(2);
            if (k0 == 0 && c + 1 < ntile) build_list(nbuf);
            NM_T(3);
            lds_barrier();
            NM_T(4);
            nm_logit_tile<SPLIT>(S.sF, w, lane, bfr, S.sLf);
            if (k0 == 0 && F <= 32 && c + 1 < ntile) load_we(c + 1, nbuf, 0, wev);
            NM_T(5);
            lds_barrier();
            NM_T(6);
#pragma unroll
            for (int k = 0; k < 4; ++k) {
                const int slot = slot_of[k] - k0;
                if (slot_of[k] >= 0 && slot >= 0 && slot < 32) lsel[k] = S.sLf[slot][ed0 + k];
            }
        }
        if (F == 0 && c + 1 < ntile) {
            build_list(nbuf);
            lds_barrier();
            load_we(c + 1, nbuf, 0, wev);
        } else if (F > 32 && c + 1 < ntile) {
            load_we(c + 1, nbuf, 0, wev);
        }
#pragma unroll
        for (int k = 0; k < 4; ++k) asm volatile("" :: "v"(bdec[k]));
        if (c + 1 < ntile) load_b(c + 1, bfr);
        NM_T(7);
        float prv[4], dbv[4];
#pragma unroll
        for (int k = 0; k < 4; ++k) {
            const int dpos = ed0 + k, gd = 32 * c + dpos;
            prv[k] = 0.f; dbv[k] = 0.f;
            if (gd >= D) continue;
            const float l = bdec[k] + lsel[k];
            const bool on = (mk >> dpos) & 1u;
            const float pr = fast_sigmoid(l);
            const float qr = fast_sigmoid(-l);
            lp += on ? nm_ln(NADE_EPS + pr) : nm_ln(NADE_EPS + qr);
            prv[k] = pr;
            const float dnll_dp = on ? -fast_rcp(NADE_EPS + pr) : fast_rcp(NADE_EPS + qr);
            dbv[k] = rw * dnll_dp * pr * qr;
        }
        if (evalid) {
            const int gd0 = 32 * c + ed0;
            const bool full = gd0 + 3 < D;
            if (cond_p != nullptr) {
                float* dst = cond_p + ((size_t)m * N + erow) * D + gd0;
                if (full && (((size_t)dst) & 15) == 0) NM_ST4(dst, prv);
                else {
#pragma unroll
                    for (int k = 0; k < 4; ++k) if (gd0 + k < D) dst[k] = prv[k];
                }
            }
            if (d_bias != nullptr) {
                float* dst = d_bias + (size_t)erow * ld_bias + bd_off + gd0;
                if (full && (((size_t)dst) & 15) == 0) NM_ST4(dst, dbv);
                else {
#pragma unroll
                    for (int k = 0; k < 4; ++k) if (gd0 + k < D) dst[k] = dbv[k];
                }
            }
        }
        NM_T(8);
    }
    lp += __shfl_xor(lp, 1);
    lp += __shfl_xor(lp, 2);
    lp += __shfl_xor(lp, 4);
    if ((tid & 7) == 0 && evalid && nll != nullptr) nll[(size_t)m * N + erow] = -lp;
    if (a_final != nullptr) {
#pragma unroll
        for (int n = 0; n < 32; ++n)
            if (rb + n < N) NM_ST1(&a_final[((size_t)m * N + rb + n) * Hn + tid], SPLIT ? areg[SPLIT ? n : 0] : S.sA[SPLIT ? 0 : n][tid]);
    }
}

template <bool SPLIT> __global__ void nade_fwd_mfma_kernel(int, int, int, const uint8_t*, long, const float*, int, const float*, const bf16_t*, const float*,
                                                           float*, float*, float*, float*, const int*, int, const int*);
template <>
__global__ void __launch_bounds__(256)
nade_fwd_mfma_kernel<false>(int tracks, int N, int D, const uint8_t* __restrict__ v, long v_track_stride, const float* __restrict__ bias, int ld_bias,
                            const float* __restrict__ w_enc, const bf16_t* __restrict__ w_dec_bf, const float* __restrict__ row_weight,
                            float* __restrict__ nll, float* __restrict__ cond_p, float* __restrict__ d_bias, float* __restrict__ a_final,
                            const int* __restrict__ gate, int run_if, const int* __restrict__ n_rows_dev) {
    nade_fwd_mfma_body<false>(tracks, N, D, v, v_track_stride, bias, ld_bias, w_enc, w_dec_bf, row_weight, nll, cond_p, d_bias, a_final, gate, run_if, n_rows_dev);
}
template <>
__global__ void __launch_bounds__(256) __attribute__((amdgpu_waves_per_eu(2, 2)))
nade_fwd_mfma_kernel<true>(int tracks, int N, int D, const uint8_t* __restrict__ v, long v_track_stride, const float* __restrict__ bias, int ld_bias,
                           const float* __restrict__ w_enc, const bf16_t* __restrict__ w_dec_bf, const float* __restrict__ row_weight,
                           float* __restrict__ nll, float* __restrict__ cond_p, float* __restrict__ d_bias, float* __restrict__ a_final,
                           const int* __restrict__ gate, int run_if, const int* __restrict__ n_rows_dev) {
    nade_fwd_mfma_body<true>(tracks, N, D, v, v_track_stride, bias, ld_bias, w_enc, w_dec_bf, row_weight, nll, cond_p, d_bias, a_final, gate, run_if, n_rows_dev);
}

extern "C" int mnn_nade_mfma_ok(int Hn) { return Hn == NM_H ? 1 : 0; }

extern "C" int mnn_nade_logprob_fwd_mfma(mnn_stream_t s, int tracks, int N, int D, int Hn, const uint8_t* v, long v_track_stride,
                                         const float* bias, int ld_bias, const float* w_enc, const void* w_dec_bf16, const float* row_weight,
                                         float* nll, float* cond_p, float* d_bias, float* a_final) {
    return mnn_nade_logprob_fwd_mfma_gated(s, tracks, N, D, Hn, v, v_track_stride, bias, ld_bias, w_enc, w_dec_bf16, row_weight, nll, cond_p, d_bias,
                                           a_final, nullptr, 0, nullptr);
}

template <bool SPLIT>
static int nm_launch(mnn_stream_t s, int tracks, int N, int D, int Hn, const uint8_t* v, long v_track_stride, const float* bias, int ld_bias,
                     const float* w_enc, const void* w_dec16, const float* row_weight, float* nll, float* cond_p, float* d_bias, float* a_final,
                     const int* gate, int run_if, const int* n_rows_dev) {
    MNN_REQUIRE(tracks > 0 && N > 0 && D > 0 && Hn == NM_H, "mnn_nade_logprob_fwd_mfma: need tracks,N,D>0 and Hn == 256 (Hn=%d)", Hn);
    MNN_REQUIRE(v && bias && w_enc && w_dec16, "mnn_nade_logprob_fwd_mfma: null pointer");
    MNN_REQUIRE(ld_bias >= tracks * (Hn + D), "mnn_nade_logprob_fwd_mfma: ld_bias %d < tracks*(Hn+D)", ld_bias);
    MNN_REQUIRE(d_bias == nullptr || row_weight != nullptr, "mnn_nade_logprob_fwd_mfma: d_bias needs row_weight");
    MNN_REQUIRE(((uintptr_t)w_dec16 & 15) == 0, "mnn_nade_logprob_fwd_mfma: the 16-bit decoder weights must be 16-byte aligned");
    static bool attr_set[64];
    int dev = 0;
    MNN_HIP(hipGetDevice(&dev));
    MNN_REQUIRE(dev >= 0 && dev < 64, "mnn_nade_logprob_fwd_mfma: device index %d", dev);
    if (!attr_set[dev]) {
        MNN_HIP(hipFuncSetAttribute((const void*)nade_fwd_mfma_kernel<SPLIT>, hipFuncAttributeMaxDynamicSharedMemorySize, (int)sizeof(NadeFwdSmemT<SPLIT>)));
        attr_set[dev] = true;
    }
    dim3 grid(cdiv(N, 32), tracks);
    hipLaunchKernelGGL(nade_fwd_mfma_kernel<SPLIT>, grid, dim3(256), sizeof(NadeFwdSmemT<SPLIT>), (hipStream_t)s, tracks, N, D, v, v_track_stride, bias,
                       ld_bias, w_enc, (const bf16_t*)w_dec16, row_weight, nll, cond_p, d_bias, a_final, gate, run_if, n_rows_dev);
    MNN_LAUNCH_CHECK();
    return MNN_OK;
}

extern "C" int mnn_nade_logprob_fwd_mfma_gated(mnn_stream_t s, int tracks, int N, int D, int Hn, const uint8_t* v, long v_track_stride,
                                               const float* bias, int ld_bias, const float* w_enc, const void* w_dec_bf16, const float* row_weight,
                                               float* nll, float* cond_p, float* d_bias, float* a_final, const int* gate, int run_if, const int* n_rows_dev) {
    return nm_launch<false>(s, tracks, N, D, Hn, v, v_track_stride, bias, ld_bias, w_enc, w_dec_bf16, row_weight, nll, cond_p, d_bias, a_final, gate, run_if, n_rows_dev);
}

extern "C" int mnn_nade_logprob_fwd_mfma_f32(mnn_stream_t s, int tracks, int N, int D, int Hn, const uint8_t* v, long v_track_stride,
                                             const float* bias, int ld_bias, const float* w_enc, const void* w_dec_packed, const float* row_weight,
                                             float* nll, float* cond_p, float* d_bias, float* a_final, const int* gate, int run_if, const int* n_rows_dev) {
    return nm_launch<true>(s, tracks, N, D, Hn, v, v_track_stride, bias, ld_bias, w_enc, w_dec_packed, row_weight, nll, cond_p, d_bias, a_final, gate, run_if, n_rows_dev);
}

__global__ void __launch_bounds__(256) nade_f32_pack_kernel(const float* __restrict__ w, long n, int Hn, float* __restrict__ out) {
    f16_t* o = reinterpret_cast<f16_t*>(out);
    for (long e = blockIdx.x * 256L + threadIdx.x; e < n; e += (long)gridDim.x * 256) {
        const long row = e / Hn;
        const int k = (int)(e - row * Hn);
        const float x = w[e];
        const f16_t hi = (f16_t)x;
        o[row * 2 * Hn + k] = hi;
        o[row * 2 * Hn + Hn + k] = (f16_t)(x - (float)hi);
    }
}
extern "C" int mnn_nade_f32_pack(mnn_stream_t s, const float* w_dec, long rows, int Hn, float* out) {
    MNN_REQUIRE(w_dec && out && rows > 0 && Hn > 0 && Hn % 8 == 0, "mnn_nade_f32_pack: bad arguments (Hn must be a multiple of 8)");
    MNN_REQUIRE(((uintptr_t)out & 15) == 0, "mnn_nade_f32_pack: the packed buffer must be 16-byte aligned");
    const long n = rows * Hn;
    hipLaunchKernelGGL(nade_f32_pack_kernel, dim3((int)std::min(2048L, (n + 255) / 256)), dim3(256), 0, (hipStream_t)s, w_dec, n, Hn, out);
    MNN_LAUNCH_CHECK();
    return MNN_OK;
}
```

### multinn_amd/generators.py

```python
import abc
import collections
import math
import os

import weakref

import torch

from . import ops
from .common import Model, RNN, NADE, RBM, ParamStore, ScanGraphs, sampling_temperature, temperature_key, glorot_uniform, zeros_init, default_device, capture_train_step
from .training import compute_gradients, world, dp_active, AdamOptimizer
from ._lib import MnnUnsupported
from .lstm_stack import LstmStack, _SINGLE, drive, drive_group, _det_f32, det_steps

_RnnEstimatorStateTuple = collections.namedtuple("RnnEstimatorStateTuple", ("b_enc", "b_dec", "rnn_state"))


class RnnEstimatorStateTuple(_RnnEstimatorStateTuple):
    dense = None

    @property
    def dtype(self):
        return self.b_enc.dtype

# ... 291 lines not shown
            self.backward()
            return self._loss

        def opt():
            self._grad_sumsq = compute_gradients(optimizer, self.store, self.clip_norm, lr, reduce=False)
        return capture_train_step(feed, step, warmup, [self], lambda: [self.store], split=dp_active(), fwd_bwd=fwd_bwd, opt=opt, **kw)

    def estimate_nll(self, x, lengths=None, num_chains=64, num_betas=1000, betas=None, seed=None, method="ais"):
        nll_sides(method)
        refuse_host_model(self.store.device, "estimate_nll")
        dev = self.store.device if self.store.device is not None else default_device()
        inputs, targets = shifted_sequences(x.to(dev))
        self.build(inputs, targets, lengths, is_train=False, mode="eval")
        return self._nll_rows_built(num_chains=num_chains, num_betas=num_betas, betas=betas, seed=seed, method=method)

    def _step_input(self, B, device):
        buf = getattr(self, "_xstep", None)
        if buf is None or buf.shape[0] != B or buf.device != torch.device(device) or buf.shape[1] != self._stack.ld0 \
                or torch.cuda.is_current_stream_capturing() != getattr(self, "_xstep_captured", False):
            buf = self._xstep = torch.zeros((B, self._stack.ld0), device=device, dtype=self.dtype)
            self._xstep_captured = torch.cuda.is_current_stream_capturing()
        return buf

    def generate(self, x, num_steps, given=None, temperature=1.0):
        if given is not None:
            n_out = getattr(self, "_num_output", self.num_dims)
            if given.dtype != torch.uint8 or tuple(given.shape) != (x.shape[0], int(num_steps), n_out):
                raise ValueError(f"given must be u8 [{x.shape[0]}, {int(num_steps)}, {n_out}], got {given.dtype} {tuple(given.shape)}")
            given = given.contiguous()
        temperature = self._temperature(temperature)
        if not ScanGraphs.enabled(x):
            return self._generate_scan(x, num_steps, given, temperature)
        if getattr(self, "_scan_graphs", None) is None:
            self._scan_graphs = ScanGraphs()
        key = (tuple(x.shape), x.dtype, int(num_steps), self.seed, self.row0)
        if given is not None:
            key = key + ("given",)
        key = key + temperature_key(temperature)

        def scan(sx, sg=None):
            self._packed_step = -1
            return self._generate_scan(sx, num_steps, sg, temperature)

        def after():
            self._packed_step = -1

        def warm(sx, sg=None):
            n = min(int(num_steps), 2)
            return self._generate_scan(sx, n, None if sg is None else sg[:, :n].contiguous(), temperature)

        return self._scan_graphs.run(key, x, scan, warm, after, extra=given)

    def _generate_scan(self, x, num_steps, given=None, temperature=1.0):
        self._materialize(x.shape[-1])
        self._rnn.build_cell(False)
        if self.det_sampling:
            whole = self._scan_in_one_call(x, num_steps, given, temperature)
            if whole is not None:
                return whole
            state = self.steps(x)
        else:
            self._ensure_packed()
            state = self._get_state(x, lengths=None, last_outputs=True)
        intro = x[:, -1, :]
        out = []
        for s in range(num_steps):
            self._gen_step = s
            kw = {} if temperature == 1.0 else dict(temperature=temperature)
            if given is not None:
                kw["given"] = given[:, s]
            samples, _ = self.sample_single(intro, state, **kw)
            state = self.single_step(samples, state)
            intro = samples
            out.append(samples)
        return torch.stack(out, 1)


class RnnNade(RnnEstimator):

    def __init__(self, num_dims, num_hidden, num_hidden_rnn, keep_prob=1.0, internal_bias=False, name="rnn-nade", track_name="all", **kw):
        self._tracks = getattr(self, "_tracks", ["all"])
        super().__init__(num_dims, num_hidden, num_hidden_rnn, keep_prob, internal_bias, name, track_name, **kw)
        self._num_output = self.num_tracks * self.num_dims

    tracks = property(lambda self: self._tracks)
    num_tracks = property(lambda self: len(self._tracks))

    def _init_estimator(self):
        self._nades = [NADE(self.num_dims, self.num_hidden[-1], internal_bias=False, name=f"nade_{m}") for m in range(self.num_tracks)]
        self._nade = self._nades[0]

    def _declare(self, num_inputs):
        M, D, Hn, R = self.num_tracks, self.num_dims, self.num_hidden[-1], self.num_hidden_rnn[-1]
        self._rnn.declare(self.store, num_inputs, self._gen)
        from .common import truncated_normal
        std = 1.0 / (D ** 0.5)
        self.store.declare("nade/w_enc", (M, D, Hn), truncated_normal(self._gen, std))
        self.store.declare("nade/w_dec", (M, D, Hn), truncated_normal(self._gen, std))
        if self.internal_bias:
            self.store.declare("nade/b_enc", (M, Hn), truncated_normal(self._gen, std))
            self.store.declare("nade/b_dec", (M, D), truncated_normal(self._gen, std))
        n_out = M * (D + Hn)
        self.store.declare("dense/kernel", (R, n_out), glorot_uniform(self._gen, R, n_out))
        self.store.declare("dense/bias", (n_out,), zeros_init)
        self.n_out = n_out
        self.ldo = ops.round_up(n_out, 64)

    def _materialize(self, num_inputs):
        first = self.store.theta is None
        super()._materialize(num_inputs)
        if first:
            for m, nd in enumerate(self._nades):
                nd._w_enc_t, nd._w_dec_t = self.store["nade/w_enc"][m], self.store["nade/w_dec"][m]

    def _pack_estimator(self):
        dev = self.store.theta.device
        R = self.num_hidden_rnn[-1]
        self._fc_t = torch.empty((self.n_out, R), device=dev, dtype=self.dtype)
        ops.transpose(self.store["dense/kernel"], self._fc_t)
        self._fc_p = torch.zeros((R, self.ldo), device=dev, dtype=self.dtype)
        ops.convert2d(self.store["dense/kernel"], self._fc_p[:, :self.n_out])
        if self.internal_bias:
            self._fc_bias = torch.empty(self.n_out, device=dev)
            ops.axpby(1.0, self.store["dense/bias"], 1.0, self._internal_flat(self.store.theta), self._fc_bias)
        else:
            self._fc_bias = self.store["dense/bias"]
        if self._nade_mfma():
            M, D, Hn = self.num_tracks, self.num_dims, self.num_hidden[-1]
            if self._nade_exact():
                self._wdec_bf = torch.empty((M, D, Hn), device=dev, dtype=torch.float32)
                ops.nade_f32_pack(self.store["nade/w_dec"].view(M * D, Hn), self._wdec_bf.view(M * D, Hn))
            else:
                self._wdec_bf = torch.empty((M, D, Hn), device=dev, dtype=torch.bfloat16)
                ops.convert2d(self.store["nade/w_dec"].view(M * D, Hn), self._wdec_bf.view(M * D, Hn))

    def _internal_flat(self, flat):
        o = self.store.offset("nade/b_enc")
        return flat[o:o + self.n_out]

    nade_mfma = os.environ.get("MULTINN_NADE_MFMA", "1") != "0"

    nade_dense_above = float(os.environ.get("MULTINN_NADE_DENSE_ABOVE", "0.07"))

    def _nade_fwd(self, v, out, rw, nll, cond_p, d_out, a_fin, n_rows_dev=None, unsafe=None):
        M, D, Hn = self.num_tracks, self.num_dims, self.num_hidden[-1]
        exact = self._nade_exact()
        if self.nade_dense_above >= 1.0:
            return ops.nade_logprob_fwd_auto(v, out, self.store["nade/w_enc"], self.store["nade/w_dec"], self._wdec_bf, M, D, Hn, None, None,
                                             1.0, rw, nll, cond_p, d_out, a_fin, exact=exact, n_rows_dev=n_rows_dev)
        if getattr(self, "_gate", None) is None or self._gate.device != out.device:
            self._gate = torch.zeros(1 + ops.DENSITY_SLOTS, device=out.device, dtype=torch.int32)
        counted = bool(getattr(self, "_v_counted", False)) and rw is not None
        return ops.nade_logprob_fwd_auto(v, out, self.store["nade/w_enc"], self.store["nade/w_dec"], self._wdec_bf, M, D, Hn, self._gate[:1],
                                         self._gate[1:], self.nade_dense_above, rw, nll, cond_p, d_out, a_fin, exact=exact, counted=counted,
                                         n_rows_dev=n_rows_dev, unsafe=unsafe)

    nade_exact = os.environ.get("MULTINN_NADE_EXACT_MFMA", "1") != "0"

    def _nade_mfma(self):
        if not (self.nade_mfma and ops.nade_mfma_ok(self.num_hidden[-1])):
            return False
        return self.dtype == torch.bfloat16 or (self.dtype == torch.float16 and self.nade_exact)

    def _nade_exact(self):
        return self.dtype == torch.float16

    def build(self, x=None, y=None, lengths=None, is_train=None, mode="eval"):
        return drive(self._build_co(x, y, lengths, is_train, mode))

    def _build_co(self, x=None, y=None, lengths=None, is_train=None, mode="eval"):
        Generator.build(self, x, y, lengths, is_train, mode)
        self._materialize(x.shape[-1] if x is not None else self._num_inputs)
        self._rnn.build_cell(is_train)
        if mode in ("train", "eval"):
            B, T, _ = x.shape
            M, D = self.num_tracks, self.num_dims
            x_tm = self._to_time_major_inputs(x)
            v = y.to(torch.uint8).transpose(0, 1).reshape(T, B, D, M).permute(3, 0, 1, 2).contiguous() if M > 1 \
                else y.to(torch.uint8).transpose(0, 1).contiguous().view(1, T, B, D)
            compact = None
            if lengths is not None and mode == "train" and self.dtype in ops.H16 and self.ragged_compact and x.is_cuda:
                dev = x.device
                len_dev = lengths.to(device=dev, dtype=torch.int32).contiguous()
                n_total_dev = None
                if dp_active():
                    n_total_dev = len_dev.clamp(0, T).sum().float().reshape(1)
                    torch.distributed.all_reduce(n_total_dev)
                idx, inv, hdr = ops.ragged_index(len_dev, B, T, n_total_dev, self._stack.loss_scale_rows if self.dtype == torch.float16 else 0.0)
                compact = dict(idx=idx, inv=inv, hdr=hdr, hdr_f=hdr.view(torch.float32))
                v = v.view(M, T * B, D).index_select(1, idx.long()).view(M, T, B, D)
                k = torch.arange(T * B, device=dev, dtype=torch.int32)
                rw = torch.where(k < hdr[0], compact["hdr_f"][1], torch.zeros((), device=dev))
                lengths = len_dev
                self._n_valid = None
            else:
                rw = self._row_weight(lengths, B, T, x.device)
            yield from self._forward_tm_co(x_tm, v, rw, lengths, B, T, train=(mode == "train"), compact=compact)
        self._is_built = True

    ragged_compact = os.environ.get("MULTINN_RAGGED_COMPACT", "1") != "0"
    ragged_gemm_rows = os.environ.get("MULTINN_RAGGED_GEMM_ROWS", "1") != "0"

    def build_pianoroll(self, x_u8, lengths=None, is_train=True, mode="train", n_total_dev=None):
        if self.num_tracks != 1:
            raise ValueError("build_pianoroll is the joint (single NADE) path")
        B, T, P, Mtr = x_u8.shape
        D = P * Mtr
        self._materialize(D)
        Generator.build(self, None, None, lengths, is_train, mode)
        self._rnn.build_cell(is_train)
        dev = x_u8.device
        x_tm = torch.empty((T, B, self._stack.ld0), device=dev, dtype=self.dtype)
        v = torch.empty((T, B, D), device=dev, dtype=torch.uint8)
        rw = torch.empty(T * B, device=dev)
        compact = None
        if lengths is not None and mode == "train" and self.dtype in ops.H16 and self.ragged_compact:
            len_dev = lengths.to(device=dev, dtype=torch.int32).contiguous()
            if n_total_dev is None and dp_active():
                n_total_dev = len_dev.clamp(0, T).sum().float().reshape(1)
                torch.distributed.all_reduce(n_total_dev)
            idx, inv, hdr = ops.ragged_index(len_dev, B, T, n_total_dev, self._stack.loss_scale_rows if self.dtype == torch.float16 else 0.0)
            compact = dict(idx=idx, inv=inv, hdr=hdr, hdr_f=hdr.view(torch.float32))
            lengths = len_dev
            n_valid = 0
            self._n_valid = None
        elif lengths is not None:
            n_tot = lengths.sum().to(dev).float()
            if dp_active():
                torch.distributed.all_reduce(n_tot)
            n_valid = int(n_tot)
            self._n_valid = max(n_valid, 1)
        else:
            n_valid = B * T * world()[1]
            self._n_valid = max(n_valid, 1)
        x_tmT = None
        if mode == "train" and self.dtype in ops.H16:
            self._ensure_packed()
            x_tmT = self._stack.input_T(T, B, dev)
            if x_tmT is None:
                Np = ops.round_up(T * B, 64)
                x_tmT = (torch.zeros if Np != T * B else torch.empty)((self._stack.ld0, Np), device=dev, dtype=self.dtype)
        cnt = None
        if x_tmT is not None and self._nade_mfma() and self.nade_dense_above < 1.0:
            if getattr(self, "_gate", None) is None or self._gate.device != dev:
                self._gate = torch.zeros(1 + ops.DENSITY_SLOTS, device=dev, dtype=torch.int32)
            cnt = self._gate[1:]
        self._v_counted = ops.pianoroll_shift_timemajor(x_u8.view(B, T, D), lengths, x_tm, v, rw, n_valid, inputs_t=x_tmT, count=cnt,
                                                        compact=(compact["inv"], compact["hdr"]) if compact else None)
        self._forward_tm(x_tm, v.view(1, T, B, D), rw, lengths, B, T, train=(mode == "train"), x_tmT=x_tmT, compact=compact)
        self._v_counted = False
        self._is_built = True

    def _forward_tm(self, x_tm, v, rw, lengths, B, T, train, x_tmT=None, compact=None):
        return drive(self._forward_tm_co(x_tm, v, rw, lengths, B, T, train, x_tmT, compact))

    def _forward_tm_co(self, x_tm, v, rw, lengths, B, T, train, x_tmT=None, compact=None):
        M, D, Hn = self.num_tracks, self.num_dims, self.num_hidden[-1]
        N, dev = T * B, x_tm.device
        self._ensure_packed()
        kp = self._rnn.effective_keep_prob()
        y, ctx, _ = yield from self._stack.forward_co(x_tm, kp, self.seed, self.row0, save=train, state0=self._state0(B),
                                                      step_dev=self.store.step_dev, state_grad=train)
        if ctx and x_tmT is not None:
            ctx[0]["inT"] = x_tmT
        nrows = None
        if compact is not None:
            R = y.shape[-1]
            Np = ops.round_up(N, 64)
            y_c = torch.empty((N, R), device=dev, dtype=self.dtype)
            y_cT = (torch.zeros if Np != N else torch.empty)((R, Np), device=dev, dtype=self.dtype) if train else None
            ops.rows_gather16(y.view(N, R), compact["idx"], compact["hdr"], y_c, y_cT)
            compact["y_cT"] = y_cT
            y_dense, nrows = y_c, compact["hdr"]
        else:
            y_dense = y.view(N, -1)
        out = torch.empty((N, self.ldo), device=dev)
        ops.gemm_tn(y_dense, self._fc_t, out[:, :self.n_out], bias=self._fc_bias, m_rows=nrows if self.ragged_gemm_rows else None)
        nll = torch.empty((M, N), device=dev)
        cond_p = None if train else torch.empty((M, N, D), device=dev)
        rw_m = rw / M if M > 1 else rw
        d_out = None
        if train:
            d_out = torch.empty((N, self.ldo), device=dev)
            if self.ldo != self.n_out and self.dtype == torch.float32:
                d_out[:, self.n_out:].zero_()
        a_fin = torch.empty((M, N, Hn), device=dev) if train else None
        dyn = self.store.ls_dyn if (train and self.dtype == torch.float16) else None
        if compact is not None:
            ls = compact["hdr_f"][2:3] if (train and self.dtype == torch.float16) else 1.0
            if torch.is_tensor(ls):
                rw_g = rw_m * (ls * dyn[0:1] * self.grad_scale)
                ls = compact["hdr_f"][3:4] * dyn[1:2]
            else:
                rw_g = rw_m if self.grad_scale == 1.0 else rw_m * self.grad_scale
        elif train and self._n_valid is None and self.dtype == torch.float16:
            rw_g = rw_m * (self._ls_dev * dyn[0:1] * self.grad_scale)
            ls = dyn[1:2] / self._ls_dev
        else:
            ls = self._stack.loss_scale(self._n_valid) if (train and self._n_valid is not None) else 1.0
            gs = self.grad_scale * ls
            if dyn is not None:
                rw_g = rw_m * (dyn[0:1] * gs)
                ls = dyn[1:2] * (1.0 / ls)
            else:
                rw_g = rw_m if gs == 1.0 else rw_m * gs
        if self._nade_mfma():
            unsafe = torch.empty(1, device=dev, dtype=torch.int32) if (train and self.nade_dense_above < 1.0) else None
            self._nade_fwd(v.view(M, N, D), out, rw_g if train else None, nll, cond_p, d_out, a_fin, n_rows_dev=nrows, unsafe=unsafe)
        else:
            assert compact is None or Hn <= 256, "compacted rows: the f32 scan covers Hn <= 256"
            ops.nade_logprob_fwd(v.view(M, N, D), out, self.store["nade/w_enc"], self.store["nade/w_dec"], M, D, Hn,
                                 rw_g if train else None, nll, cond_p, d_out, a_fin, n_rows_dev=nrows)
        loss = torch.zeros(1, device=dev)
        ops.weighted_sum(nll.view(-1), rw_m.repeat(M) if M > 1 else rw_m, loss)
        self._ctx = dict(x_tm=x_tm, v=v, rw=rw_m, y=y, lstm=ctx, out=out, d_out=d_out, a_fin=a_fin, kp=kp, seed=self.seed, B=B, T=T, ls=ls,
                         compact=compact, unsafe=unsafe if self._nade_mfma() else None)
        self._nll_tm, self._cond_tm, self._loss = nll, cond_p, loss
        self._flat_idx = None
        self._lengths = lengths
        self._metrics = {"batch/loss": loss, "log_likelihood": loss}
        self._metrics_upd = []

    def _idx(self):
        if self._flat_idx is None:
            fi = flat_index(self._lengths, self._ctx["B"], self._ctx["T"], self._loss.device)
            cp = self._ctx.get("compact")
            self._flat_idx = cp["inv"].long()[fi] if cp is not None else fi
        return self._flat_idx

    @property
    def log_probs(self):
        r = [self._nll_tm[m][self._idx()] for m in range(self.num_tracks)]
        return r[0] if self.num_tracks == 1 else r

    def _nll_rows_built(self, method="ais", **ais):
        nll_sides(method)
        idx = self._idx()
        est = NllEstimate(sum(self._nll_tm[m][idx] for m in range(self.num_tracks)))
        return nll_result(method, (est, est))

    @property
    def cond_probs(self):
        if self._cond_tm is None:
            cx = self._ctx
            M, D, Hn = self.num_tracks, self.num_dims, self.num_hidden[-1]
            N = cx["B"] * cx["T"]
            cp = torch.empty((M, N, D), device=cx["out"].device)
            if self._nade_mfma():
                self._nade_fwd(cx["v"].view(M, N, D), cx["out"], None, None, cp, None, None,
                               n_rows_dev=cx["compact"]["hdr"] if cx.get("compact") else None)
            else:
                ops.nade_logprob_fwd(cx["v"].view(M, N, D), cx["out"], self.store["nade/w_enc"], self.store["nade/w_dec"], M, D, Hn, None, None, cp, None,
                                     None)
            self._cond_tm = cp
        r = [self._cond_tm[m][self._idx()] for m in range(self.num_tracks)]
        return r[0] if self.num_tracks == 1 else r

    @property
    def _outputs(self):
        cp = self.cond_probs
        return (cp >= 0.5).float() if self.num_tracks == 1 else [(c >= 0.5).float() for c in cp]

    def build_metrics(self, targets, predictions, cond_probs=None, log_probs=None):
        return self._nade.build_metrics(targets, predictions, cond_probs, log_probs)

    def backward(self):
        return drive(self._backward_co())

    def _backward_co(self):
        cx = self._ctx
        if cx["d_out"] is None:
            raise RuntimeError("build(..., mode='train') must run before train()")
        M, D, Hn, R = self.num_tracks, self.num_dims, self.num_hidden[-1], self.num_hidden_rnn[-1]
        B, T = cx["B"], cx["T"]
        N, dev = B * T, cx["out"].device
        g = self.store.gviews
        self.store.grad.zero_()
        d_out = cx["d_out"]
        compact = cx.get("compact")
        ops.nade_logprob_bwd(cx["v"].view(M, N, D), cx["out"], self.store["nade/w_enc"], self.store["nade/w_dec"], M, D, Hn, cx["a_fin"],
                             d_out, g["nade/w_enc"], g["nade/w_dec"], n_rows_dev=compact["hdr"] if compact else None,
                             unsafe=cx.get("unsafe"))
        Np = ops.round_up(N, 64)
        zalloc = torch.zeros if Np != N else torch.empty
        yT = cx["lstm"][-1].get("yT") if cx["lstm"] else None
        if compact is not None:
            yT = compact["y_cT"]
        if yT is None:
            yT = zalloc((R, Np), device=dev, dtype=self.dtype)
            ops.transpose(cx["y"].view(N, R), yT)
        doT = zalloc((self.n_out, Np), device=dev, dtype=self.dtype)
        if self.dtype == torch.float32:
            ops.transpose(d_out[:, :self.n_out], doT)
            ops.bias_grad(d_out[:, :self.n_out], g["dense/bias"], accumulate=True)
            do_c = d_out
        else:
            do_c = torch.empty((N, self.ldo), device=dev, dtype=self.dtype)
            ops.grad_rows_fanout(d_out, self.n_out, do_c, doT, g["dense/bias"])
        if self.internal_bias:
            gi = self._internal_flat(self.store.grad)
            ops.axpby(1.0, gi, 1.0, g["dense/bias"], gi)
        nrows = compact["hdr"] if (compact is not None and self.ragged_gemm_rows) else None
        ops.gemm_tn(yT, doT, g["dense/kernel"], accumulate=True, split_k=LstmStack._split_k(R, self.n_out, Np), k_rows=nrows)
        del yT, doT
        dy = torch.empty((N, R), device=dev)
        ops.gemm_tn(do_c, self._fc_p, dy, m_rows=nrows)
        if compact is not None:
            dy_c, dy = dy, torch.empty((N, R), device=dev)
            ops.rows_scatter_f32(dy_c, compact["inv"], compact["hdr"], dy)
        self._dx = yield from self._lstm_backward_co(dy, cx)
        self._unscale(cx.get("ls", 1.0))

    def train_step(self, x_u8, lengths, optimizer, lr=None):
        self.build_pianoroll(x_u8, lengths, is_train=True, mode="train")
        self.train(optimizer, lr)
        return self._loss

    def capturable(self, shape, ragged):
        B, T = shape[0], shape[1]
        stack = getattr(self, "_stack", None)
        if stack is None or stack.packed is None or not (stack._persist(B, T) or stack._rowpar(B, T)):
            return False
        if self.learn_zero_state and not stack._rowpar_state0(B, T):
            return False
        return not ragged or (self.ragged_compact and self.dtype in ops.H16 and self.num_tracks == 1)

    def graphed_train_step(self, x_u8, optimizer, lr=None, warmup=2, lengths=None):
        static_x = x_u8.clone()
        ragged = lengths is not None
        if ragged and not (self.dtype in ops.H16 and self.ragged_compact):
            raise ValueError("graphed_train_step(lengths=...) needs the compacted ragged path (16-bit precision, MULTINN_RAGGED_COMPACT unset)")
        dev = x_u8.device
        T = x_u8.shape[1]
        static_len = lengths.to(device=dev, dtype=torch.int32).clone() if ragged else None
        multi = dp_active()
        static_ntot = torch.zeros(1, device=dev) if (ragged and multi) else None

        def set_total():
            if static_ntot is not None:
                static_ntot.copy_(static_len.clamp(0, T).sum().float().reshape(1))
                torch.distributed.all_reduce(static_ntot)

        me = weakref.ref(self)

        def feed(x=None, lengths=None):
            if x is not None:
                static_x.copy_(x)
            if lengths is not None:
                if not ragged:
                    raise ValueError("this step was captured for full-length windows: capture it with lengths= to feed ragged ones")
                static_len.copy_(lengths.to(device=dev, dtype=torch.int32))
                set_total()
                me().lengths_fed()

        set_total()
        run = self._capture_step(feed, lambda: self.build_pianoroll(static_x, static_len, is_train=True, mode="train", n_total_dev=static_ntot),
                                 optimizer, lr, warmup)
        run.ragged = ragged
        return run

    def zero_state(self, batch_size):
        self._materialize(self._num_inputs)
        dev = self.store.theta.device
        z = lambda n: torch.zeros((batch_size, n), device=dev)
        be = z(self.num_hidden[-1]) if self.num_tracks == 1 else [z(self.num_hidden[-1]) for _ in self._tracks]
        bd = z(self.num_dims) if self.num_tracks == 1 else [z(self.num_dims) for _ in self._tracks]
        return RnnEstimatorStateTuple(be, bd, self._get_rnn_zero_state(batch_size))

    def _build_biases(self, outputs):
        M, D, Hn = self.num_tracks, self.num_dims, self.num_hidden[-1]
        be = [outputs[:, m * Hn:(m + 1) * Hn] for m in range(M)]
        bd = [outputs[:, M * Hn + m * D:M * Hn + (m + 1) * D] for m in range(M)]
        return (be[0], bd[0]) if M == 1 else (be, bd)

    def _dense(self, h):
# ... 633 lines not shown
```

### multinn_amd/ops.py

```python
import ctypes as C
import math

import torch

from . import _lib
from ._lib import F32, BF16, U8, F16, GEMM_ACCUMULATE, GEMM_A_KBLOCK32


def call(name, *args):
    return _lib.call(name, *args)

_DT = {torch.float32: F32, torch.bfloat16: BF16, torch.uint8: U8, torch.float16: F16}
H16 = (torch.bfloat16, torch.float16)
DENSITY_SLOTS = 256


def dtype_code(t):
    return _DT[t.dtype if isinstance(t, torch.Tensor) else t]


def _stream():
    if not torch.cuda.is_available():
        raise _lib.MnnError("multinn_amd has no CPU path: no ROCm device is available")
    return C.c_void_p(torch.cuda.current_stream().cuda_stream)
# ... 385 lines not shown
    arr = ((_lib.LstmFwdLayer if fwd else _lib.LstmBwdLayer) * n)(*descs)
    dptr = None
    if dc0s is not None and any(d is not None for d in dc0s):
        _req(not fwd and len(dc0s) == n, "lstm_recurrence_multi: dc0s goes with a backward kind, one entry per job")
        for d, L in zip(dc0s, descs):
            if d is not None:
                _dc0_ok(d, B, L.units)
        dptr = (C.c_void_p * n)(*[_p0(d) for d in dc0s])
    if kind.startswith("resident"):
        if dptr is not None:
            call("mnn_lstm_resident_bwd_state_multi", _stream(), T, B, n, arr, float(keep_prob), dptr)
        else:
            call("mnn_lstm_resident_%s_multi" % ("fwd" if fwd else "bwd"), _stream(), T, B, n, arr, float(keep_prob))
    else:
        _req(wss is not None and len(wss) == n, "lstm_recurrence_multi: one workspace per job")
        for ws, d in zip(wss, descs):
            _rp_ws_ok(ws, T, B, d.units)
        ptrs = (C.c_void_p * n)(*[ws.data_ptr() for ws in wss])
        if dptr is not None:
            call("mnn_lstm_cluster_bwd_state_multi", _stream(), T, B, n, arr, float(keep_prob), ptrs, dptr)
        else:
            call("mnn_lstm_cluster_%s_multi" % ("fwd" if fwd else "bwd"), _stream(), T, B, n, arr, float(keep_prob), ptrs)
    return arr


def lstm_cluster_bwd_multi_ok(B, units, njobs):
    return bool(_lib.load().mnn_lstm_cluster_bwd_multi_ok(int(B), int(units), int(njobs)))


def lstm_cluster_fwd(T, B, L, keep_prob, ws):
    _rp_ws_ok(ws, T, B, L.units)
    call("mnn_lstm_cluster_fwd", _stream(), T, B, C.byref(L), float(keep_prob), _ptr(ws))


def lstm_cluster_bwd(T, B, L, keep_prob, ws, dc0=None):
    _rp_ws_ok(ws, T, B, L.units)
    if dc0 is None:
        call("mnn_lstm_cluster_bwd", _stream(), T, B, C.byref(L), float(keep_prob), _ptr(ws))
    else:
        _dc0_ok(dc0, B, L.units)
        call("mnn_lstm_cluster_bwd_state", _stream(), T, B, C.byref(L), float(keep_prob), _ptr(ws), _ptr(dc0))


def lstm_rowpar_check(ws):
    st = C.c_int(0)
    call("mnn_lstm_rowpar_status", _ptr(ws), C.byref(st))
    if st.value != 0:
        raise _lib.MnnError("row-parallel LSTM launch timed out waiting for a neighbouring wave (grid not co-resident?)")


def dropout_mask(mask, keep_prob, seed, row0, layer, step_dev=None):
    T, B, u = mask.shape
    _req(mask.dtype == torch.uint8 and mask.is_contiguous() and u % 4 == 0 and 0 < keep_prob < 1, "dropout_mask: u8 [T,B,u], 0<kp<1")
    _step_ok(step_dev)
    call("mnn_dropout_mask", _stream(), _ptr(mask), T, B, u, float(keep_prob), int(seed), _ptr(step_dev), int(row0), int(layer))


def dropout_fwd(h, y, keep_prob, seed, row0, layer, step_dev=None, t_offset=0):
    T, B, u = h.shape
    _req(h.is_contiguous() and y.is_contiguous() and h.shape == y.shape and h.dtype == y.dtype and u % 4 == 0, "dropout_fwd: shapes")
    _step_ok(step_dev)
    call("mnn_dropout_fwd", _stream(), dtype_code(h), _ptr(h), _ptr(y), T, B, u, float(keep_prob), int(seed), _ptr(step_dev), int(row0),
         int(layer), int(t_offset))


def dropout_bwd(dy, dh, keep_prob, seed, row0, layer, accumulate=False, step_dev=None, t_offset=0):
    T, B, u = dy.shape
    _req(dy.dtype == torch.float32 and dh.dtype == torch.float32 and dy.is_contiguous() and dh.is_contiguous() and dy.shape == dh.shape,
         "dropout_bwd: f32 [T,B,u]")
    _step_ok(step_dev)
    call("mnn_dropout_bwd", _stream(), _ptr(dy), _ptr(dh), T, B, u, float(keep_prob), int(seed), _ptr(step_dev), int(row0), int(layer),
         int(accumulate), int(t_offset))


def _nade_check(tracks, N, D, Hn, v, bias, w_enc, w_dec):
    _req(v.dtype == torch.uint8 and v.is_contiguous() and v.numel() == tracks * N * D, "nade: v must be contiguous u8 [tracks,N,D]")
    _req(bias.dtype == torch.float32 and bias.dim() == 2 and bias.shape[0] == N and bias.stride(1) == 1
         and bias.shape[1] >= tracks * (Hn + D), "nade: bias f32 [N, >=tracks*(Hn+D)]")
    for w in (w_enc, w_dec):
        _req(w.dtype == torch.float32 and w.is_contiguous() and w.numel() == tracks * D * Hn, "nade: weights f32 [tracks,D,Hn]")
    _req(0 < Hn <= 256, "nade: Hn must be in 1..256")


def nade_logprob_fwd(v, bias, w_enc, w_dec, tracks, D, Hn, row_weight=None, nll=None, cond_p=None, d_bias=None, a_final=None, n_rows_dev=None,
                     gate=None, run_if=0, unsafe=None):
    N = bias.shape[0]
    _nade_check(tracks, N, D, Hn, v, bias, w_enc, w_dec)
    if nll is not None:
        _req(nll.dtype == torch.float32 and nll.numel() == tracks * N and nll.is_contiguous(), "nade: nll f32 [tracks,N]")
    if cond_p is not None:
        _req(cond_p.dtype == torch.float32 and cond_p.numel() == tracks * N * D and cond_p.is_contiguous(), "nade: cond_p f32 [tracks,N,D]")
    if d_bias is not None:
        _req(row_weight is not None and d_bias.shape == bias.shape and d_bias.stride() == bias.stride() and d_bias.dtype == torch.float32,
             "nade: d_bias must mirror bias and needs row_weight")
    if row_weight is not None:
        _req(row_weight.dtype == torch.float32 and row_weight.numel() == N, "nade: row_weight f32 [N]")
    if a_final is not None:
        _req(a_final.dtype == torch.float32 and a_final.numel() == tracks * N * Hn and a_final.is_contiguous(), "nade: a_final f32 [tracks,N,Hn]")
    _req(unsafe is None or (unsafe.dtype == torch.int32 and unsafe.numel() == 1), "nade: unsafe int32[1]")
    if n_rows_dev is not None or gate is not None or unsafe is not None:
        call("mnn_nade_logprob_fwd_gated", _stream(), tracks, N, D, Hn, _ptr(v), N * D, _ptr(bias), bias.stride(0), _ptr(w_enc), _ptr(w_dec),
             _ptr(row_weight), _ptr(nll), _ptr(cond_p), _ptr(d_bias), _ptr(a_final), _ptr(gate), int(run_if), _ptr(n_rows_dev), _ptr(unsafe))
        return
    call("mnn_nade_logprob_fwd", _stream(), tracks, N, D, Hn, _ptr(v), N * D, _ptr(bias), bias.stride(0), _ptr(w_enc), _ptr(w_dec),
         _ptr(row_weight), _ptr(nll), _ptr(cond_p), _ptr(d_bias), _ptr(a_final))


def nade_mfma_ok(Hn):
    return bool(_lib.load().mnn_nade_mfma_ok(int(Hn)))


def nade_logprob_fwd_mfma(v, bias, w_enc, w_dec_bf, tracks, D, Hn, row_weight=None, nll=None, cond_p=None, d_bias=None, a_final=None):
    N = bias.shape[0]
    _nade_check(tracks, N, D, Hn, v, bias, w_enc, w_enc)
    _req(w_dec_bf.dtype == torch.bfloat16 and w_dec_bf.is_contiguous() and w_dec_bf.numel() == tracks * D * Hn, "nade mfma: w_dec_bf bf16 [tracks,D,Hn]")
    if nll is not None:
        _req(nll.dtype == torch.float32 and nll.numel() == tracks * N and nll.is_contiguous(), "nade: nll f32 [tracks,N]")
    if cond_p is not None:
        _req(cond_p.dtype == torch.float32 and cond_p.numel() == tracks * N * D and cond_p.is_contiguous(), "nade: cond_p f32 [tracks,N,D]")
    if d_bias is not None:
        _req(row_weight is not None and d_bias.shape == bias.shape and d_bias.stride() == bias.stride() and d_bias.dtype == torch.float32,
             "nade: d_bias must mirror bias and needs row_weight")
    if row_weight is not None:
        _req(row_weight.dtype == torch.float32 and row_weight.numel() == N, "nade: row_weight f32 [N]")
    if a_final is not None:
        _req(a_final.dtype == torch.float32 and a_final.numel() == tracks * N * Hn and a_final.is_contiguous(), "nade: a_final f32 [tracks,N,Hn]")
    call("mnn_nade_logprob_fwd_mfma", _stream(), tracks, N, D, Hn, _ptr(v), N * D, _ptr(bias), bias.stride(0), _ptr(w_enc), _ptr(w_dec_bf),
         _ptr(row_weight), _ptr(nll), _ptr(cond_p), _ptr(d_bias), _ptr(a_final))


def nade_f32_pack(w_dec, out):
    _rowmajor(w_dec, "f32_pack w_dec"); _rowmajor(out, "f32_pack out")
    rows, Hn = w_dec.shape
    _req(w_dec.dtype == torch.float32 and w_dec.is_contiguous() and out.dtype == torch.float32 and out.is_contiguous()
         and out.shape == (rows, Hn) and Hn % 8 == 0, "f32_pack: w_dec f32 [rows,Hn] -> out f32 [rows,Hn], Hn % 8 == 0")
    call("mnn_nade_f32_pack", _stream(), _ptr(w_dec), rows, Hn, _ptr(out))
    return out


def nade_logprob_fwd_auto(v, bias, w_enc, w_dec, w_dec_bf, tracks, D, Hn, gate, count, dense_above=0.07, row_weight=None, nll=None,
                          cond_p=None, d_bias=None, a_final=None, exact=False, counted=False, n_rows_dev=None, unsafe=None):
    N = bias.shape[0]
    _nade_check(tracks, N, D, Hn, v, bias, w_enc, w_dec)
    _req(w_dec_bf.dtype == (torch.float32 if exact else torch.bfloat16) and w_dec_bf.is_contiguous() and w_dec_bf.numel() == tracks * D * Hn,
         "nade auto: w_dec_bf bf16 [tracks,D,Hn] (exact form: the f32-sized [tracks,D,Hn] output of nade_f32_pack)")
    _req(gate is None or (gate.dtype == torch.int32 and gate.numel() == 1 and count.dtype == torch.int32 and count.numel() == DENSITY_SLOTS and count.is_contiguous()),
         "nade auto: gate int32[1], count int32[DENSITY_SLOTS]")
    for t, n in ((nll, tracks * N), (cond_p, tracks * N * D), (a_final, tracks * N * Hn)):
        _req(t is None or (t.dtype == torch.float32 and t.numel() == n and t.is_contiguous()), "nade auto: f32 outputs")
    if d_bias is not None:
        _req(row_weight is not None and d_bias.shape == bias.shape and d_bias.stride() == bias.stride() and d_bias.dtype == torch.float32,
             "nade: d_bias must mirror bias and needs row_weight")
    if row_weight is not None:
        _req(row_weight.dtype == torch.float32 and row_weight.numel() == N, "nade: row_weight f32 [N]")
    common = (tracks, N, D, Hn, _ptr(v), N * D, _ptr(bias), bias.stride(0), _ptr(w_enc))
    tail = (_ptr(row_weight), _ptr(nll), _ptr(cond_p), _ptr(d_bias), _ptr(a_final), _ptr(gate))
    mfma = "mnn_nade_logprob_fwd_mfma_f32" if exact else "mnn_nade_logprob_fwd_mfma_gated"
    nr = _ptr(n_rows_dev)
    if gate is None:
        call(mfma, _stream(), *common, _ptr(w_dec_bf), *tail, 0, nr)
        return
    call("mnn_density_gate", _stream(), None if counted else _ptr(v), v.numel(), int(dense_above * v.numel()), _ptr(gate), _ptr(count))
    call(mfma, _stream(), *common, _ptr(w_dec_bf), *tail, 0, nr)
    _req(unsafe is None or (unsafe.dtype == torch.int32 and unsafe.numel() == 1), "nade auto: unsafe int32[1]")
    call("mnn_nade_logprob_fwd_gated", _stream(), *common, _ptr(w_dec), *tail, 1, nr, _ptr(unsafe))


def nade_logprob_bwd(v, bias, w_enc, w_dec, tracks, D, Hn, a_final, d_bias, d_w_enc, d_w_dec, n_rows_dev=None, unsafe=None):
    _req(unsafe is None or (unsafe.dtype == torch.int32 and unsafe.numel() == 1), "nade bwd: unsafe int32[1]")
    N = bias.shape[0]
    _nade_check(tracks, N, D, Hn, v, bias, w_enc, w_dec)
    _req(d_bias.shape == bias.shape and d_bias.stride() == bias.stride() and d_bias.dtype == torch.float32, "nade bwd: d_bias")
    for w in (d_w_enc, d_w_dec):
        _req(w.dtype == torch.float32 and w.is_contiguous() and w.numel() == tracks * D * Hn, "nade bwd: grad weights f32 [tracks,D,Hn]")
    _req(a_final.dtype == torch.float32 and a_final.numel() == tracks * N * Hn and a_final.is_contiguous(), "nade bwd: a_final f32 [tracks,N,Hn]")
    call("mnn_nade_logprob_bwd", _stream(), tracks, N, D, Hn, _ptr(v), N * D, _ptr(bias), bias.stride(0), _ptr(w_enc), _ptr(w_dec),
         _ptr(a_final), _ptr(d_bias), _ptr(d_w_enc), _ptr(d_w_dec), _ptr(n_rows_dev), _ptr(unsafe))


def _temps(temperature, n_per_job, by_visible, what):
    if temperature is None or isinstance(temperature, (int, float)):
        return None
    t = tuple(float(x) for x in temperature)
    _req(1 <= len(t) <= _lib.TEMPS_MAX and all(math.isfinite(x) and x > 0.0 for x in t),
         f"{what}: 1..{_lib.TEMPS_MAX} positive finite temperatures")
    _req(by_visible or len(t) in (1, n_per_job), f"{what}: one temperature, or one per track / job ({n_per_job})")
    st = _lib.Temps()
    st.n, st.by_visible = len(t), 1 if by_visible else 0
    for i, x in enumerate(t):
        st.t[i] = x
    return st


def nade_sample(bias, w_enc, w_dec, tracks, D, Hn, temperature, seed, row0, sub, samples, track_minor=False, nll=None, given=None,
                by_visible=False):
    N = bias.shape[0]
    _req(bias.dtype == torch.float32 and bias.dim() == 2 and bias.stride(1) == 1 and bias.shape[1] >= tracks * (Hn + D), "sample: bias")
    _req(samples.dtype == torch.uint8 and samples.shape == (N, tracks * D) and samples.is_contiguous(), "sample: samples u8 [N,tracks*D]")
    for w in (w_enc, w_dec):
        _req(w.dtype == torch.float32 and w.is_contiguous() and w.numel() == tracks * D * Hn, "sample: weights")
    if nll is not None:
        _req(nll.dtype == torch.float32 and nll.numel() == tracks * N, "sample: nll")
    if given is not None:
        _req(given.dtype == torch.uint8 and tuple(given.shape) == (N, tracks * D) and given.is_contiguous() and given.device == samples.device,
             "sample: given u8 [N, tracks*D], contiguous")
    ts, es = (1, tracks) if track_minor else (D, 1)
    tt = _temps(temperature, tracks, by_visible, "sample")
    if tt is not None:
        call("mnn_nade_sample_temps", _stream(), tracks, N, D, Hn, _ptr(bias), bias.stride(0), _ptr(w_enc), _ptr(w_dec), C.byref(tt), int(seed),
             int(row0), int(sub), _ptr(samples), ts, tracks * D, es, _ptr(nll), _ptr(given))
        return
    call("mnn_nade_sample", _stream(), tracks, N, D, Hn, _ptr(bias), bias.stride(0), _ptr(w_enc), _ptr(w_dec),
         float(-1.0 if temperature is None else temperature), int(seed), int(row0), int(sub), _ptr(samples), ts, tracks * D, es, _ptr(nll), _ptr(given))


def nade_sample_multi(jobs, D, Hn, temperature, row0, sub):
    _req(1 <= len(jobs) <= 8, "nade_sample_multi: 1..8 jobs")
    arr = (_lib.NadeSampleJob * len(jobs))()
    N = jobs[0]["bias"].shape[0]
    rs, es = jobs[0]["samples"].stride()
    for a, j in zip(arr, jobs):
        b, smp, nll = j["bias"], j["samples"], j.get("nll")
        _req(b.dtype == torch.float32 and b.dim() == 2 and b.stride(1) == 1 and b.shape == (N, b.shape[1]) and b.shape[1] >= Hn + D, "sample_multi: bias")
        _req(smp.dtype == torch.uint8 and tuple(smp.shape) == (N, D) and smp.stride() == (rs, es) and es >= 1, "sample_multi: samples u8 [N, D] views of equal strides")
        for w in (j["w_enc"], j["w_dec"]):
            _req(w.dtype == torch.float32 and w.is_contiguous() and w.numel() == D * Hn, "sample_multi: weights f32 [D, Hn]")
        _req(nll is None or (nll.dtype == torch.float32 and nll.is_contiguous() and nll.numel() == N), "sample_multi: nll f32 [N]")
        gv = j.get("given")
        _req(gv is None or (gv.dtype == torch.uint8 and tuple(gv.shape) == (N, D) and gv.stride() == (rs, es) and gv.device == smp.device),
             "sample_multi: given u8 [N, D] with the strides of samples")
        a.bias, a.ld_bias, a.w_enc, a.w_dec, a.seed, a.samples, a.nll = _ptr(b), b.stride(0), _ptr(j["w_enc"]), _ptr(j["w_dec"]), int(j["seed"]), _ptr(smp), _ptr(nll)
        a.given = _ptr(gv)
    tt = _temps(temperature, len(jobs), False, "sample_multi")
    if tt is not None:
        call("mnn_nade_sample_multi_temps", _stream(), len(jobs), arr, N, D, Hn, C.byref(tt), int(row0), int(sub), rs, es)
        return
    call("mnn_nade_sample_multi", _stream(), len(jobs), arr, N, D, Hn, float(-1.0 if temperature is None else temperature), int(row0), int(sub), rs, es)


def _ldb(b, n):
    _req(b.dtype == torch.float32 and b.dim() == 2 and b.stride(1) == 1 and b.shape[1] >= n, "rbm: bias must be f32 [N or 1, n]")
    return 0 if b.shape[0] == 1 else b.stride(0)


def rbm_workspace(D, Hn, device):
    return torch.empty(_lib.load().mnn_rbm_workspace_bytes(D, Hn), dtype=torch.uint8, device=device)


def _rbm_temperature(t, what):
    _req(isinstance(t, (int, float)) and math.isfinite(t) and t > 0.0, f"{what}: the temperature of an RBM chain is a positive finite number")
    return float(t)


def rbm_gibbs(v0, W, bh, bv, k, seed, row0=0, row_ids=None, sub0=0, p_v=None, v_out=None, seed_step=None, given=None, temperature=1.0):
    N, D = v0.shape
    Hn = W.shape[1]
    _req(v0.dtype == torch.uint8 and v0.is_contiguous(), "gibbs: v0 u8 [N,D]")
    _req(W.dtype == torch.float32 and W.shape == (D, Hn) and W.is_contiguous(), "gibbs: W f32 [D,Hn]")
# ... 456 lines not shown
```

Measured before the change: 20.22 million timesteps/s.

## Fuse dense-layer gradient epilogue into NADE forward/backward kernels

The NADE forward and backward kernels gain an optional ops path. When it is enabled they also write the dense layer's output gradient in 16-bit, both row-major and transposed, and accumulate the per-column bias-gradient sums through wave reductions and atomics into slot buffers. This removes the separate transpose, conversion and bias_grad passes over d_out in the model's backward step, and can skip the f32 d_bias write when keep_f32 is off. In exchange it adds register and shared-memory pressure, scattered transposed stores and atomic contention on the bias sums inside already heavy kernels.

Result: faster. 20.56 million timesteps/s, median of 5 (+1.7%).

```diff
diff --git a/include/multinn_hip.h b/include/multinn_hip.h
--- a/include/multinn_hip.h
+++ b/include/multinn_hip.h
@@ -152,6 +152,27 @@
                          const float* bias, int ld_bias, const float* w_enc, const float* w_dec, const float* a_final,
                          float* d_bias, float* d_w_enc, float* d_w_dec, const int* n_rows_dev ,
                          const int* unsafe );
+typedef struct {
+    void* out_c; int ld_c;
+    void* out_t; int ld_t;
+    float* db;
+    int dtype;
+    int keep_f32;
+    int db_slots;
+} mnn_nade_ops;
+int mnn_nade_logprob_fwd_gated_ops(mnn_stream_t s, int tracks, int N, int D, int Hn, const uint8_t* v, long v_track_stride,
+                                   const float* bias, int ld_bias, const float* w_enc, const float* w_dec, const float* row_weight,
+                                   float* nll, float* cond_p, float* d_bias, float* a_final, const int* gate, int run_if,
+                                   const int* n_rows_dev, int* unsafe, const mnn_nade_ops* ops);
+int mnn_nade_logprob_fwd_mfma_gated_ops(mnn_stream_t s, int tracks, int N, int D, int Hn, const uint8_t* v, long v_track_stride, const float* bias,
+                                        int ld_bias, const float* w_enc, const void* w_dec_bf16, const float* row_weight, float* nll, float* cond_p,
+                                        float* d_bias, float* a_final, const int* gate, int run_if, const int* n_rows_dev, const mnn_nade_ops* ops);
+int mnn_nade_logprob_fwd_mfma_f32_ops(mnn_stream_t s, int tracks, int N, int D, int Hn, const uint8_t* v, long v_track_stride, const float* bias,
+                                      int ld_bias, const float* w_enc, const void* w_dec_packed, const float* row_weight, float* nll, float* cond_p,
+                                      float* d_bias, float* a_final, const int* gate, int run_if, const int* n_rows_dev, const mnn_nade_ops* ops);
+int mnn_nade_logprob_bwd_ops(mnn_stream_t s, int tracks, int N, int D, int Hn, const uint8_t* v, long v_track_stride,
+                             const float* bias, int ld_bias, const float* w_enc, const float* w_dec, const float* a_final,
+                             float* d_bias, float* d_w_enc, float* d_w_dec, const int* n_rows_dev, const int* unsafe, const mnn_nade_ops* ops);
 int mnn_nade_sample(mnn_stream_t s, int tracks, int N, int D, int Hn, const float* bias, int ld_bias, const float* w_enc,
                     const float* w_dec, float temperature, uint64_t seed, uint32_t row0, uint32_t sub, uint8_t* samples,
                     long s_track_stride, int s_row_stride, int s_elem_stride, float* nll, const uint8_t* given);
diff --git a/multinn_amd/_lib.py b/multinn_amd/_lib.py
--- a/multinn_amd/_lib.py
+++ b/multinn_amd/_lib.py
@@ -77,6 +77,10 @@
 
 class Temps(C.Structure):
     _fields_ = [("n", _i), ("by_visible", _i), ("t", _f * 8)]
+
+
+class NadeOps(C.Structure):
+    _fields_ = [("out_c", _p), ("ld_c", _i), ("out_t", _p), ("ld_t", _i), ("db", _p), ("dtype", _i), ("keep_f32", _i), ("db_slots", _i)]
 
 
 class RbmGibbsJob(C.Structure):
@@ -163,6 +167,9 @@
                                               C.POINTER(C.c_void_p), C.POINTER(C.c_void_p)])
 SIGNATURES["mnn_rbm_gibbs_temp"] = (_i, [_p, _i, _i, _i, _i, _p, _p, _p, _i, _p, _i, _u64, _u32, _p, _u32, _p, _p, _p, _p, _i, _f])
 SIGNATURES["mnn_rbm_gibbs_multi_temps"] = (_i, [_p, _i, _p, _i, _i, _i, _i, _i, _i, _u32, _p, _u32, _p, _l, _i, _l, _p, C.POINTER(C.c_float)])
+for _n in ("mnn_nade_logprob_fwd_gated", "mnn_nade_logprob_fwd_mfma_gated", "mnn_nade_logprob_fwd_mfma_f32"):
+    SIGNATURES[_n + "_ops"] = (_i, SIGNATURES[_n][1] + [C.POINTER(NadeOps)])
+SIGNATURES["mnn_nade_logprob_bwd_ops"] = (_i, SIGNATURES["mnn_nade_logprob_bwd"][1] + [C.POINTER(NadeOps)])
 TEMPS_MAX = 8
 
 _lib = None
diff --git a/multinn_amd/csrc/nade.hip b/multinn_amd/csrc/nade.hip
--- a/multinn_amd/csrc/nade.hip
+++ b/multinn_amd/csrc/nade.hip
@@ -1,4 +1,5 @@
 #include "common.h"
+#include "nade_ops.h"
 
 #define NADE_EPS 1e-6f
 #define LN2 0.6931471805599453f
@@ -84,14 +85,17 @@
     }
 };
 
-template <int HQ, bool UT>
+template <int HQ, bool UT, bool OPS>
 __global__ void __launch_bounds__(512)
 nade_fwd_kernel(int tracks, int N, int D, int Hn, const uint8_t* __restrict__ v, long v_track_stride, const float* __restrict__ bias,
                 int ld_bias, const float* __restrict__ w_enc, const float* __restrict__ w_dec, const float* __restrict__ row_weight,
                 float* __restrict__ nll, float* __restrict__ cond_p, float* __restrict__ d_bias, float* __restrict__ a_final,
-                const int* __restrict__ gate, int run_if, const int* __restrict__ n_rows_dev, int* __restrict__ unsafe) {
+                const int* __restrict__ gate, int run_if, const int* __restrict__ n_rows_dev, int* __restrict__ unsafe,
+                h16_t* __restrict__ out_c, int ld_c, h16_t* __restrict__ out_t, int ld_t, float* __restrict__ db, int f16, int slot_mask) {
     constexpr int W = HQ * 64;
     __shared__ float wl[2][2][8 * W];
+    __shared__ float dbs[OPS ? 2 : 1][8][8];
+    const NadeOps ops = {out_c, out_t, db + (size_t)(blockIdx.x & slot_mask) * (tracks * (Hn + D)), ld_c, ld_t, f16, 0, 0};
     if (gate != nullptr && *gate != run_if) {
         if (unsafe != nullptr && blockIdx.x == 0 && blockIdx.y == 0 && threadIdx.x == 0) atomicAdd(unsafe, 1);
         return;
@@ -99,6 +103,7 @@
     const int m = blockIdx.y;
     if (nade_rows_beyond(n_rows_dev, blockIdx.x * 64)) {
         nade_zero_rows(d_bias, ld_bias, tracks * Hn + m * D, D, blockIdx.x * 64, 64, N, 512);
+        if constexpr (OPS) nops_zero_block(out_c, ld_c, out_t, ld_t, tracks * Hn + m * D, D, blockIdx.x * 64, 64, N, 512, true);
         if (nll != nullptr && threadIdx.x < 64 && blockIdx.x * 64 + threadIdx.x < N) nll[(size_t)m * N + blockIdx.x * 64 + threadIdx.x] = 0.f;
         return;
     }
@@ -149,9 +154,17 @@
     float bcur = fi < D ? bias[(size_t)frr * ld_bias + bd_off + fi] : 0.f;
     __syncthreads();
     const int nch = (D + 7) / 8;
+    auto add_sums = [&](int cd) {
+        if (threadIdx.x < 8 && cd * 8 + (int)threadIdx.x < D) {
+            const float (*p)[8] = dbs[cd & 1];
+            const int t = threadIdx.x;
+            NOPS_ADD(ops.db + bd_off + cd * 8 + t, ((p[0][t] + p[1][t]) + (p[2][t] + p[3][t])) + ((p[4][t] + p[5][t]) + (p[6][t] + p[7][t])));
+        }
+    };
     for (int c = 0; c < nch; ++c) {
         const int i0 = c * 8;
         const int inext = i0 + 8 + fi;
+        if (OPS && c > 0) add_sums(c - 1);
         st.gload(wd, we, i0 + 8, D, Hn);
         const int inc = min(inext, D - 1);
         const uint8_t vraw = vm[(size_t)frr * D + inc];
@@ -222,6 +235,7 @@
         }
         const float tot = vis8(y, lane);
         const int i = i0 + fi;
+        float dbx = 0.f;
         if (i < D) {
             const float l = bcur + tot;
             const float pr = fast_sigmoid(l);
@@ -231,15 +245,34 @@
                 if (cond_p != nullptr) cond_p[((size_t)m * N + frow) * D + i] = pr;
                 if (d_bias != nullptr) {
                     const float dnll_dp = vcur ? -fast_rcp(NADE_EPS + pr) : fast_rcp(NADE_EPS + qr);
-                    d_bias[(size_t)frow * ld_bias + bd_off + i] = rw * dnll_dp * pr * qr;
-                }
-            }
+                    dbx = rw * dnll_dp * pr * qr;
+                    d_bias[(size_t)frow * ld_bias + bd_off + i] = dbx;
+                    if constexpr (OPS) {
+                        const h16_t hx = nops_cvt(ops, dbx);
+                        (ops.out_c + bd_off + i0)[__umul24(frow, ld_c) + fi] = hx;
+                        (ops.out_t + (size_t)(bd_off + i0) * ops.ld_t)[__umul24(fi, ld_t) + frow] = hx;
+                    }
+                }
+            }
+        }
+        if constexpr (OPS) {
+            {
+                auto r = __builtin_amdgcn_permlane32_swap(__float_as_uint(dbx), __float_as_uint(dbx), false, false);
+                dbx = __uint_as_float(r[0]) + __uint_as_float(r[1]);
+            }
+            {
+                auto r = __builtin_amdgcn_permlane16_swap(__float_as_uint(dbx), __float_as_uint(dbx), false, false);
+                dbx = __uint_as_float(r[0]) + __uint_as_float(r[1]);
+            }
+            dbx += dpp_xor8(dbx);
+            if (lane < 8) dbs[c & 1][w][lane] = dbx;
         }
         st.lstore(wl[(c + 1) & 1][0], wl[(c + 1) & 1][1]);
         vcur = fvalid && inext < D && vraw != 0;
         bcur = inext < D ? braw : 0.f;
         __syncthreads();
     }
+    if constexpr (OPS) add_sums(nch - 1);
     lp += dpp_xor1(lp);
     lp += dpp_xor2(lp);
     lp += swz_xor4(lp);
@@ -270,25 +303,42 @@
                                           const float* bias, int ld_bias, const float* w_enc, const float* w_dec, const float* row_weight,
                                           float* nll, float* cond_p, float* d_bias, float* a_final, const int* gate, int run_if, const int* n_rows_dev,
                                           int* unsafe) {
+    return mnn_nade_logprob_fwd_gated_ops(s, tracks, N, D, Hn, v, v_track_stride, bias, ld_bias, w_enc, w_dec, row_weight, nll, cond_p, d_bias, a_final,
+                                          gate, run_if, n_rows_dev, unsafe, nullptr);
+}
+
+extern "C" int mnn_nade_logprob_fwd_gated_ops(mnn_stream_t s, int tracks, int N, int D, int Hn, const uint8_t* v, long v_track_stride,
+                                              const float* bias, int ld_bias, const float* w_enc, const float* w_dec, const float* row_weight,
+                                              float* nll, float* cond_p, float* d_bias, float* a_final, const int* gate, int run_if,
+                                              const int* n_rows_dev, int* unsafe, const mnn_nade_ops* ops_abi) {
     MNN_REQUIRE(tracks > 0 && N > 0 && D > 0 && Hn > 0 && Hn <= 256, "mnn_nade_logprob_fwd: need tracks,N,D>0 and 0<Hn<=256 (Hn=%d)", Hn);
     MNN_REQUIRE(v && bias && w_enc && w_dec, "mnn_nade_logprob_fwd: null pointer");
     MNN_REQUIRE(ld_bias >= tracks * (Hn + D), "mnn_nade_logprob_fwd: ld_bias %d < tracks*(Hn+D)", ld_bias);
     MNN_REQUIRE(d_bias == nullptr || row_weight != nullptr, "mnn_nade_logprob_fwd: d_bias needs row_weight");
+    NadeOps ops;
+    const char* why = "";
+    MNN_REQUIRE(nops_from_abi(ops_abi, tracks, N, D, Hn, &ops, &why), "mnn_nade_logprob_fwd: ops: %s", why);
+    MNN_REQUIRE(ops.out_c == nullptr || d_bias != nullptr, "mnn_nade_logprob_fwd: ops need d_bias (and row_weight)");
+    MNN_REQUIRE(ops.out_c == nullptr || ((long)N * ops.ld_c < (1L << 31) && 8L * ops.ld_t + N < (1L << 31)), "mnn_nade_logprob_fwd: ops: extents past 32-bit offsets");
     dim3 grid(cdiv(N, 64), tracks);
     hipStream_t st = (hipStream_t)s;
-#define FWD(HQ, UT) hipLaunchKernelGGL((nade_fwd_kernel<HQ, UT>), grid, dim3(512), 0, st, tracks, N, D, Hn, v, v_track_stride, bias, ld_bias, w_enc, \
-                                       w_dec, row_weight, nll, cond_p, d_bias, a_final, gate, run_if, n_rows_dev, unsafe)
+#define FWD_(HQ, UT, OPS) hipLaunchKernelGGL((nade_fwd_kernel<HQ, UT, OPS>), grid, dim3(512), 0, st, tracks, N, D, Hn, v, v_track_stride, bias, ld_bias, w_enc, \
+                                       w_dec, row_weight, nll, cond_p, d_bias, a_final, gate, run_if, n_rows_dev, unsafe, ops.out_c, ops.ld_c, ops.out_t, ops.ld_t, ops.db, \
+                                       ops.f16, ops.slot_mask)
+#define FWD(HQ, UT) do { if (ops.out_c != nullptr) FWD_(HQ, UT, true); else FWD_(HQ, UT, false); } while (0)
     if (unsafe != nullptr) MNN_HIP(mnn_zero_async(unsafe, sizeof(int), sizeof(int), 1, st));
     static const bool no_ut = getenv("MNN_NADE_FWD_NO_UT") != nullptr;
-    if (Hn <= 64) FWD(1, false);
+    if (Hn <= 64) FWD_(1, false, false);
     else if (Hn <= 128) FWD(2, false);
     else if (gate != nullptr && run_if == 1 && !no_ut) FWD(4, true);
     else FWD(4, false);
 #undef FWD
+#undef FWD_
     MNN_LAUNCH_CHECK();
     return MNN_OK;
 }
 
+typedef unsigned nade_u4 __attribute__((ext_vector_type(4)));
 template <int HQ> struct LaneVec;
 template <> struct LaneVec<2> { typedef float2 T; };
 template <> struct LaneVec<4> { typedef float4 T; };
@@ -335,8 +385,10 @@
 nade_bwd_kernel(int tracks, int N, int D, int HnT, int nslice, const uint8_t* __restrict__ v, long v_track_stride, const float* __restrict__ bias,
                 int ld_bias, const float* __restrict__ w_enc, const float* __restrict__ w_dec, const float* __restrict__ a_final,
                 float* __restrict__ d_bias, float* __restrict__ d_w_enc, float* __restrict__ d_w_dec, const int* __restrict__ n_rows_dev,
-                const int* __restrict__ unsafe) {
+                const int* __restrict__ unsafe, h16_t* __restrict__ out_c, int ld_c, h16_t* __restrict__ out_t, int ld_t, float* __restrict__ db,
+                int f16, int keep_f32, int slot_mask) {
     constexpr int W = HQ * 64;
+    const NadeOps ops = {out_c, out_t, db + (size_t)(blockIdx.x & slot_mask) * (tracks * (HnT + D)), ld_c, ld_t, f16, keep_f32, 0};
     __shared__ __attribute__((aligned(16))) float wl[2][2][8 * W];
     if (unsafe != nullptr && (*unsafe == 0) != USEU) return;
     constexpr int NRED = HQ <= 2 ? 2 : 1;
@@ -344,7 +396,9 @@
     const int m = blockIdx.y / nslice, hb = (blockIdx.y - m * nslice) * W;
     const int Hn = min(W, HnT - hb);
     if (nade_rows_beyond(n_rows_dev, blockIdx.x * (64 * RG))) {
-        nade_zero_rows(d_bias, ld_bias, m * HnT + hb, Hn, blockIdx.x * (64 * RG), 64 * RG, N, 512);
+        if (out_c == nullptr || keep_f32) nade_zero_rows(d_bias, ld_bias, m * HnT + hb, Hn, blockIdx.x * (64 * RG), 64 * RG, N, 512);
+        nops_zero_block(out_c, ld_c, out_t, ld_t, m * HnT + hb, Hn, blockIdx.x * (64 * RG), 64 * RG, N, 512, true);
+        if (blockIdx.y == 0) nops_zero_block(out_c, ld_c, out_t, ld_t, tracks * (HnT + D), ld_c - tracks * (HnT + D), blockIdx.x * (64 * RG), 64 * RG, N, 512, false);
         return;
     }
     const int Nv = n_rows_dev != nullptr ? min(*n_rows_dev, N) : N;
@@ -546,6 +600,53 @@
     for (int r = 0; r < BWD_R; ++r)
 #pragma unroll
         for (int q = 0; q < HQ; ++q) G[r][q] = fmaf(c[r][q], fmaf(-h[r][q], h[r][q], h[r][q]), G[r][q]);
+    if (ops.out_c != nullptr) {
+        constexpr int TP = 64 * RG + 8;
+        h16_t* tt = reinterpret_cast<h16_t*>(&red_[0][0][0][0][0]);
+        float* rs = reinterpret_cast<float*>(tt + W * TP);
+        static_assert(W * TP * 2 + 8 * W * 4 <= (int)sizeof(red_), "the epilogue's tile and sums fit in red_");
+        float sum[HQ];
+        __syncthreads();
+#pragma unroll
+        for (int q = 0; q < HQ; ++q) {
+            const int j = lane + 64 * q;
+            sum[q] = 0.f;
+#pragma unroll
+            for (int g = 0; g < RG; ++g) {
+                __builtin_amdgcn_sched_barrier(0);
+                uint32_t hv[8];
+#pragma unroll
+                for (int e = 0; e < 8; ++e) hv[e] = rbase + 8 * g + e < N ? (uint32_t)nops_cvt(ops, G[8 * g + e][q]) : 0u;
+                *reinterpret_cast<nade_u4*>(tt + j * TP + w * BWD_R + 8 * g) =
+                    (nade_u4){hv[0] | (hv[1] << 16), hv[2] | (hv[3] << 16), hv[4] | (hv[5] << 16), hv[6] | (hv[7] << 16)};
+#pragma unroll
+                for (int e = 0; e < 8; ++e) {
+                    const int row = rbase + 8 * g + e;
+                    h16_t* rowp = ops.out_c + (size_t)row * ops.ld_c + m * HnT + hb;
+                    if (row < N && j < Hn) rowp[(unsigned)j] = (h16_t)hv[e];
+                }
+                const float (&x)[BWD_R][HQ] = G;
+                sum[q] += ((x[8 * g][q] + x[8 * g + 1][q]) + (x[8 * g + 2][q] + x[8 * g + 3][q])) +
+                          ((x[8 * g + 4][q] + x[8 * g + 5][q]) + (x[8 * g + 6][q] + x[8 * g + 7][q]));
+            }
+        }
+#pragma unroll
+        for (int q = 0; q < HQ; ++q) rs[w * W + lane + 64 * q] = sum[q];
+        if (blockIdx.y == 0) nops_zero_block(out_c, ld_c, out_t, ld_t, tracks * (HnT + D), ld_c - tracks * (HnT + D), blockIdx.x * (64 * RG), 64 * RG, N, 512, false);
+        __syncthreads();
+        for (int e = threadIdx.x; e < W * 8 * RG; e += 512) {
+            const int u = e / (8 * RG), part = e - u * (8 * RG);
+            if (u < Hn)
+                NOPS_ST_T(*reinterpret_cast<const nade_u4*>(tt + u * TP + 8 * part),
+                          reinterpret_cast<nade_u4*>(ops.out_t + (size_t)(m * HnT + hb + u) * ops.ld_t + blockIdx.x * (64 * RG) + 8 * part));
+        }
+        if ((int)threadIdx.x < Hn) {
+            const float* p = rs + threadIdx.x;
+            NOPS_ADD(ops.db + m * HnT + hb + threadIdx.x,
+                     ((p[0] + p[W]) + (p[2 * W] + p[3 * W])) + ((p[4 * W] + p[5 * W]) + (p[6 * W] + p[7 * W])));
+        }
+        if (!ops.keep_f32) return;
+    }
 #pragma unroll
     for (int r = 0; r < BWD_R; ++r)
 #pragma unroll
@@ -558,12 +659,24 @@
 extern "C" int mnn_nade_logprob_bwd(mnn_stream_t s, int tracks, int N, int D, int Hn, const uint8_t* v, long v_track_stride,
                                     const float* bias, int ld_bias, const float* w_enc, const float* w_dec, const float* a_final,
                                     float* d_bias, float* d_w_enc, float* d_w_dec, const int* n_rows_dev, const int* unsafe) {
+    return mnn_nade_logprob_bwd_ops(s, tracks, N, D, Hn, v, v_track_stride, bias, ld_bias, w_enc, w_dec, a_final, d_bias, d_w_enc, d_w_dec, n_rows_dev, unsafe,
+                                    nullptr);
+}
+
+extern "C" int mnn_nade_logprob_bwd_ops(mnn_stream_t s, int tracks, int N, int D, int Hn, const uint8_t* v, long v_track_stride,
+                                        const float* bias, int ld_bias, const float* w_enc, const float* w_dec, const float* a_final,
+                                        float* d_bias, float* d_w_enc, float* d_w_dec, const int* n_rows_dev, const int* unsafe,
+                                        const mnn_nade_ops* ops_abi) {
     MNN_REQUIRE(tracks > 0 && N > 0 && D > 0 && Hn > 0 && Hn <= 256, "mnn_nade_logprob_bwd: need tracks,N,D>0 and 0<Hn<=256 (Hn=%d)", Hn);
     MNN_REQUIRE(v && bias && w_enc && w_dec && a_final && d_bias && d_w_enc && d_w_dec, "mnn_nade_logprob_bwd: null pointer");
     MNN_REQUIRE(ld_bias >= tracks * (Hn + D), "mnn_nade_logprob_bwd: ld_bias too small");
+    NadeOps ops;
+    const char* why = "";
+    MNN_REQUIRE(nops_from_abi(ops_abi, tracks, N, D, Hn, &ops, &why), "mnn_nade_logprob_bwd: ops: %s", why);
     hipStream_t st = (hipStream_t)s;
 #define BWD(HQ, NS, U, S) hipLaunchKernelGGL((nade_bwd_kernel<HQ, 1, U>), dim3(cdiv(N, 64), tracks * (NS)), dim3(512), 0, st, tracks, N, D, Hn, NS, v, \
-                                             v_track_stride, bias, ld_bias, w_enc, w_dec, a_final, d_bias, d_w_enc, d_w_dec, n_rows_dev, S)
+                                             v_track_stride, bias, ld_bias, w_enc, w_dec, a_final, d_bias, d_w_enc, d_w_dec, n_rows_dev, S, ops.out_c, ops.ld_c, \
+                                             ops.out_t, ops.ld_t, ops.db, ops.f16, ops.keep_f32, ops.slot_mask)
     if (Hn <= 64) BWD(1, 1, false, nullptr);
     else {
         if (unsafe != nullptr) BWD(2, cdiv(Hn, 128), true, unsafe);
diff --git a/multinn_amd/csrc/nade_mfma.hip b/multinn_amd/csrc/nade_mfma.hip
--- a/multinn_amd/csrc/nade_mfma.hip
+++ b/multinn_amd/csrc/nade_mfma.hip
@@ -1,7 +1,9 @@
 #include "common.h"
+#include "nade_ops.h"
 typedef float nm_f4 __attribute__((ext_vector_type(4)));
 #define NM_ST4(dst, a) __builtin_nontemporal_store((nm_f4){a[0], a[1], a[2], a[3]}, reinterpret_cast<nm_f4*>(dst))
 #define NM_ST1(dst, x) __builtin_nontemporal_store((float)(x), dst)
+typedef unsigned nm_u2 __attribute__((ext_vector_type(2)));
 #include <algorithm>
 #include <type_traits>
 
@@ -24,6 +26,7 @@
 
 __device__ __forceinline__ void lds_barrier() { asm volatile("s_waitcnt lgkmcnt(0)\n\ts_barrier" ::: "memory"); }
 
+template <int CTRL> __device__ __forceinline__ float nm_dpp(float x) { return __int_as_float(__builtin_amdgcn_update_dpp(0, __float_as_int(x), CTRL, 0xf, 0xf, false)); }
 __device__ __forceinline__ float nm_ln(float x) { return __builtin_amdgcn_logf(x) * LN2F; }
 
 typedef _Float16 f16x8_t __attribute__((ext_vector_type(8)));
@@ -98,12 +101,12 @@
     for (int i = 0; i < 4; ++i) out[16 * mi + 4 * (lane >> 4) + i][16 * ni + (lane & 15)] = acc[i];
 }
 
-template <bool SPLIT>
+template <bool SPLIT, bool OPS>
 __device__ __forceinline__ void
 nade_fwd_mfma_body(int tracks, int N, int D, const uint8_t* __restrict__ v, long v_track_stride, const float* __restrict__ bias, int ld_bias,
                      const float* __restrict__ w_enc, const bf16_t* __restrict__ w_dec_bf, const float* __restrict__ row_weight,
                      float* __restrict__ nll, float* __restrict__ cond_p, float* __restrict__ d_bias, float* __restrict__ a_final,
-                     const int* __restrict__ gate, int run_if, const int* __restrict__ n_rows_dev) {
+                     const int* __restrict__ gate, int run_if, const int* __restrict__ n_rows_dev, const NadeOps ops) {
     extern __shared__ __attribute__((aligned(16))) char smem_raw[];
     typedef NadeFwdSmemT<SPLIT> NadeFwdSmem;
     typedef typename NmState<SPLIT>::T state_t;
@@ -126,6 +129,10 @@
             for (int e = tid; e < 32 * D; e += 256) {
                 const int n = e / D, i = e - n * D;
                 if (rb + n < N) d_bias[(size_t)(rb + n) * ld_bias + bd_off + i] = 0.f;
+                if constexpr (OPS) {
+                    if (rb + n < N) ops.out_c[(size_t)(rb + n) * ops.ld_c + bd_off + i] = 0;
+                    ops.out_t[(size_t)(bd_off + (e >> 5)) * ops.ld_t + rb + (e & 31)] = 0;
+                }
             }
         if (nll != nullptr && tid < 32 && rb + tid < N) nll[(size_t)m * N + rb + tid] = 0.f;
         return;
@@ -222,6 +229,27 @@
     const int err = evalid ? erow : N - 1;
     const float rw = (row_weight != nullptr && evalid) ? row_weight[erow] : 0.f;
     float lp = 0.f;
+    constexpr bool opsb = OPS;
+    float4 dprev = make_float4(0.f, 0.f, 0.f, 0.f);
+    auto park = [en, ed0](float (*tile)[NM_LP], float4 x) { *reinterpret_cast<float4*>(&tile[en][ed0]) = x; };
+    auto emit_t = [&](const float (*tile)[NM_LP], int ct) {
+        const int tc = tid >> 3, rq = tid & 7, gd = 32 * ct + tc;
+        float x[4];
+#pragma unroll
+        for (int j = 0; j < 4; ++j) x[j] = tile[4 * rq + j][tc];
+        float sum = (x[0] + x[1]) + (x[2] + x[3]);
+        sum += nm_dpp<0xB1>(sum);
+        sum += nm_dpp<0x4E>(sum);
+        sum += nm_dpp<0x141>(sum);
+        if (gd < D) {
+            const int r0 = rb + 4 * rq;
+            nm_u2 pk;
+            pk.x = (r0 < N ? (uint32_t)nops_cvt(ops, x[0]) : 0u) | ((r0 + 1 < N ? (uint32_t)nops_cvt(ops, x[1]) : 0u) << 16);
+            pk.y = (r0 + 2 < N ? (uint32_t)nops_cvt(ops, x[2]) : 0u) | ((r0 + 3 < N ? (uint32_t)nops_cvt(ops, x[3]) : 0u) << 16);
+            NOPS_ST_T(pk, reinterpret_cast<nm_u2*>(ops.out_t + (size_t)(bd_off + gd) * ops.ld_t + r0));
+            if (rq == 0) NOPS_ADD(ops.db + bd_off + gd, sum);
+        }
+    };
 #ifdef NM_TRACE
     long long tprev_ = wall_clock64();
 #endif
@@ -262,6 +290,7 @@
             const int pj = max(jj[k] - 1, 0);
             slot_of[k] = jj[k] > 0 ? (int)S.sPs[buf][pj] + __popc(S.sAct[buf][pj] & ((1u << en) - 1u)) : -1;
         }
+        if (opsb && c > 0) park(F > 0 ? S.sLb : S.sLf, dprev);
         for (int k0 = 0; k0 < F; k0 += 32) {
             if (k0 > 0) load_we(c, buf, k0, wev);
             const int cnt = min(32, F - k0);
@@ -330,6 +359,7 @@
             NM_T(4);
             nm_logit_tile<SPLIT>(S.sF, w, lane, bfr, S.sLf);
             if (k0 == 0 && F <= 32 && c + 1 < ntile) load_we(c + 1, nbuf, 0, wev);
+            if (opsb && c > 0 && k0 == 0) emit_t(S.sLb, c - 1);
             NM_T(5);
             lds_barrier();
             NM_T(6);
@@ -343,8 +373,12 @@
             build_list(nbuf);
             lds_barrier();
             load_we(c + 1, nbuf, 0, wev);
+            if (opsb && c > 0) emit_t(S.sLf, c - 1);
         } else if (F > 32 && c + 1 < ntile) {
             load_we(c + 1, nbuf, 0, wev);
+        } else if (F == 0 && opsb && c > 0) {
+            lds_barrier();
+            emit_t(S.sLf, c - 1);
         }
 #pragma unroll
         for (int k = 0; k < 4; ++k) asm volatile("" :: "v"(bdec[k]));
@@ -383,9 +417,26 @@
 #pragma unroll
                     for (int k = 0; k < 4; ++k) if (gd0 + k < D) dst[k] = dbv[k];
                 }
-            }
-        }
+                if (opsb) {
+                    h16_t* dc = ops.out_c + (size_t)erow * ops.ld_c + bd_off + gd0;
+                    if (full && (((size_t)dc) & 7) == 0) {
+                        nm_u2 pk;
+                        pk.x = nops_pack2(ops, dbv[0], dbv[1]); pk.y = nops_pack2(ops, dbv[2], dbv[3]);
+                        __builtin_nontemporal_store(pk, reinterpret_cast<nm_u2*>(dc));
+                    } else {
+#pragma unroll
+                        for (int k = 0; k < 4; ++k) if (gd0 + k < D) dc[k] = nops_cvt(ops, dbv[k]);
+                    }
+                }
+            }
+        }
+        dprev = evalid ? make_float4(dbv[0], dbv[1], dbv[2], dbv[3]) : make_float4(0.f, 0.f, 0.f, 0.f);
         NM_T(8);
+    }
+    if (opsb) {
+        park(S.sLb, dprev);
+        lds_barrier();
+        emit_t(S.sLb, ntile - 1);
     }
     lp += __shfl_xor(lp, 1);
     lp += __shfl_xor(lp, 2);
@@ -398,24 +449,26 @@
     }
 }
 
-template <bool SPLIT> __global__ void nade_fwd_mfma_kernel(int, int, int, const uint8_t*, long, const float*, int, const float*, const bf16_t*, const float*,
-                                                           float*, float*, float*, float*, const int*, int, const int*);
-template <>
-__global__ void __launch_bounds__(256)
-nade_fwd_mfma_kernel<false>(int tracks, int N, int D, const uint8_t* __restrict__ v, long v_track_stride, const float* __restrict__ bias, int ld_bias,
-                            const float* __restrict__ w_enc, const bf16_t* __restrict__ w_dec_bf, const float* __restrict__ row_weight,
-                            float* __restrict__ nll, float* __restrict__ cond_p, float* __restrict__ d_bias, float* __restrict__ a_final,
-                            const int* __restrict__ gate, int run_if, const int* __restrict__ n_rows_dev) {
-    nade_fwd_mfma_body<false>(tracks, N, D, v, v_track_stride, bias, ld_bias, w_enc, w_dec_bf, row_weight, nll, cond_p, d_bias, a_final, gate, run_if, n_rows_dev);
-}
-template <>
-__global__ void __launch_bounds__(256) __attribute__((amdgpu_waves_per_eu(2, 2)))
-nade_fwd_mfma_kernel<true>(int tracks, int N, int D, const uint8_t* __restrict__ v, long v_track_stride, const float* __restrict__ bias, int ld_bias,
-                           const float* __restrict__ w_enc, const bf16_t* __restrict__ w_dec_bf, const float* __restrict__ row_weight,
-                           float* __restrict__ nll, float* __restrict__ cond_p, float* __restrict__ d_bias, float* __restrict__ a_final,
-                           const int* __restrict__ gate, int run_if, const int* __restrict__ n_rows_dev) {
-    nade_fwd_mfma_body<true>(tracks, N, D, v, v_track_stride, bias, ld_bias, w_enc, w_dec_bf, row_weight, nll, cond_p, d_bias, a_final, gate, run_if, n_rows_dev);
-}
+template <bool SPLIT, bool OPS> __global__ void nade_fwd_mfma_kernel(int, int, int, const uint8_t*, long, const float*, int, const float*, const bf16_t*, const float*,
+                                                                     float*, float*, float*, float*, const int*, int, const int*, h16_t*, int, h16_t*, int, float*, int, int);
+#define NM_KERNEL(SPLIT, OPS, ATTR)                                                                                                                      \
+    template <>                                                                                                                                          \
+    __global__ void __launch_bounds__(256) ATTR                                                                                                          \
+    nade_fwd_mfma_kernel<SPLIT, OPS>(int tracks, int N, int D, const uint8_t* __restrict__ v, long v_track_stride, const float* __restrict__ bias,       \
+                                     int ld_bias, const float* __restrict__ w_enc, const bf16_t* __restrict__ w_dec_bf,                                  \
+                                     const float* __restrict__ row_weight, float* __restrict__ nll, float* __restrict__ cond_p,                          \
+                                     float* __restrict__ d_bias, float* __restrict__ a_final, const int* __restrict__ gate, int run_if,                  \
+                                     const int* __restrict__ n_rows_dev, h16_t* __restrict__ out_c, int ld_c, h16_t* __restrict__ out_t, int ld_t,       \
+                                     float* __restrict__ db, int f16, int slot_mask) {                                                                   \
+        const NadeOps ops = {out_c, out_t, db + (size_t)(blockIdx.x & slot_mask) * (tracks * (NM_H + D)), ld_c, ld_t, f16, 0, 0};                        \
+        nade_fwd_mfma_body<SPLIT, OPS>(tracks, N, D, v, v_track_stride, bias, ld_bias, w_enc, w_dec_bf, row_weight, nll, cond_p, d_bias, a_final, gate,  \
+                                       run_if, n_rows_dev, ops);                                                                                         \
+    }
+NM_KERNEL(false, false, )
+NM_KERNEL(false, true, )
+NM_KERNEL(true, false, __attribute__((amdgpu_waves_per_eu(2, 2))))
+NM_KERNEL(true, true, __attribute__((amdgpu_waves_per_eu(2, 2))))
+#undef NM_KERNEL
 
 extern "C" int mnn_nade_mfma_ok(int Hn) { return Hn == NM_H ? 1 : 0; }
 
@@ -426,40 +479,67 @@
                                            a_final, nullptr, 0, nullptr);
 }
 
-template <bool SPLIT>
-static int nm_launch(mnn_stream_t s, int tracks, int N, int D, int Hn, const uint8_t* v, long v_track_stride, const float* bias, int ld_bias,
+template <bool SPLIT, bool OPS>
+static int nm_launch_ops(mnn_stream_t s, int tracks, int N, int D, int Hn, const uint8_t* v, long v_track_stride, const float* bias, int ld_bias,
                      const float* w_enc, const void* w_dec16, const float* row_weight, float* nll, float* cond_p, float* d_bias, float* a_final,
-                     const int* gate, int run_if, const int* n_rows_dev) {
+                     const int* gate, int run_if, const int* n_rows_dev, const NadeOps& ops) {
     MNN_REQUIRE(tracks > 0 && N > 0 && D > 0 && Hn == NM_H, "mnn_nade_logprob_fwd_mfma: need tracks,N,D>0 and Hn == 256 (Hn=%d)", Hn);
     MNN_REQUIRE(v && bias && w_enc && w_dec16, "mnn_nade_logprob_fwd_mfma: null pointer");
     MNN_REQUIRE(ld_bias >= tracks * (Hn + D), "mnn_nade_logprob_fwd_mfma: ld_bias %d < tracks*(Hn+D)", ld_bias);
     MNN_REQUIRE(d_bias == nullptr || row_weight != nullptr, "mnn_nade_logprob_fwd_mfma: d_bias needs row_weight");
     MNN_REQUIRE(((uintptr_t)w_dec16 & 15) == 0, "mnn_nade_logprob_fwd_mfma: the 16-bit decoder weights must be 16-byte aligned");
+    MNN_REQUIRE(!OPS || d_bias != nullptr, "mnn_nade_logprob_fwd_mfma: ops need d_bias (and row_weight)");
     static bool attr_set[64];
     int dev = 0;
     MNN_HIP(hipGetDevice(&dev));
     MNN_REQUIRE(dev >= 0 && dev < 64, "mnn_nade_logprob_fwd_mfma: device index %d", dev);
     if (!attr_set[dev]) {
-        MNN_HIP(hipFuncSetAttribute((const void*)nade_fwd_mfma_kernel<SPLIT>, hipFuncAttributeMaxDynamicSharedMemorySize, (int)sizeof(NadeFwdSmemT<SPLIT>)));
+        MNN_HIP(hipFuncSetAttribute((const void*)nade_fwd_mfma_kernel<SPLIT, OPS>, hipFuncAttributeMaxDynamicSharedMemorySize, (int)sizeof(NadeFwdSmemT<SPLIT>)));
         attr_set[dev] = true;
     }
     dim3 grid(cdiv(N, 32), tracks);
-    hipLaunchKernelGGL(nade_fwd_mfma_kernel<SPLIT>, grid, dim3(256), sizeof(NadeFwdSmemT<SPLIT>), (hipStream_t)s, tracks, N, D, v, v_track_stride, bias,
-                       ld_bias, w_enc, (const bf16_t*)w_dec16, row_weight, nll, cond_p, d_bias, a_final, gate, run_if, n_rows_dev);
+    hipLaunchKernelGGL((nade_fwd_mfma_kernel<SPLIT, OPS>), grid, dim3(256), sizeof(NadeFwdSmemT<SPLIT>), (hipStream_t)s, tracks, N, D, v, v_track_stride, bias,
+                       ld_bias, w_enc, (const bf16_t*)w_dec16, row_weight, nll, cond_p, d_bias, a_final, gate, run_if, n_rows_dev, ops.out_c, ops.ld_c, ops.out_t, ops.ld_t, ops.db, ops.f16, ops.slot_mask);
     MNN_LAUNCH_CHECK();
     return MNN_OK;
+}
+
+template <bool SPLIT>
+static int nm_launch(mnn_stream_t s, int tracks, int N, int D, int Hn, const uint8_t* v, long v_track_stride, const float* bias, int ld_bias,
+                     const float* w_enc, const void* w_dec16, const float* row_weight, float* nll, float* cond_p, float* d_bias, float* a_final,
+                     const int* gate, int run_if, const int* n_rows_dev, const mnn_nade_ops* ops_abi) {
+    NadeOps ops;
+    const char* why = "";
+    MNN_REQUIRE(nops_from_abi(ops_abi, tracks, N, D, Hn, &ops, &why), "mnn_nade_logprob_fwd_mfma: ops: %s", why);
+    if (ops.out_c != nullptr)
+        return nm_launch_ops<SPLIT, true>(s, tracks, N, D, Hn, v, v_track_stride, bias, ld_bias, w_enc, w_dec16, row_weight, nll, cond_p, d_bias, a_final, gate,
+                                          run_if, n_rows_dev, ops);
+    return nm_launch_ops<SPLIT, false>(s, tracks, N, D, Hn, v, v_track_stride, bias, ld_bias, w_enc, w_dec16, row_weight, nll, cond_p, d_bias, a_final, gate,
+                                       run_if, n_rows_dev, ops);
 }
 
 extern "C" int mnn_nade_logprob_fwd_mfma_gated(mnn_stream_t s, int tracks, int N, int D, int Hn, const uint8_t* v, long v_track_stride,
                                                const float* bias, int ld_bias, const float* w_enc, const void* w_dec_bf16, const float* row_weight,
                                                float* nll, float* cond_p, float* d_bias, float* a_final, const int* gate, int run_if, const int* n_rows_dev) {
-    return nm_launch<false>(s, tracks, N, D, Hn, v, v_track_stride, bias, ld_bias, w_enc, w_dec_bf16, row_weight, nll, cond_p, d_bias, a_final, gate, run_if, n_rows_dev);
+    return nm_launch<false>(s, tracks, N, D, Hn, v, v_track_stride, bias, ld_bias, w_enc, w_dec_bf16, row_weight, nll, cond_p, d_bias, a_final, gate, run_if, n_rows_dev, nullptr);
+}
+extern "C" int mnn_nade_logprob_fwd_mfma_gated_ops(mnn_stream_t s, int tracks, int N, int D, int Hn, const uint8_t* v, long v_track_stride,
+                                                   const float* bias, int ld_bias, const float* w_enc, const void* w_dec_bf16, const float* row_weight,
+                                                   float* nll, float* cond_p, float* d_bias, float* a_final, const int* gate, int run_if, const int* n_rows_dev,
+                                                   const mnn_nade_ops* ops) {
+    return nm_launch<false>(s, tracks, N, D, Hn, v, v_track_stride, bias, ld_bias, w_enc, w_dec_bf16, row_weight, nll, cond_p, d_bias, a_final, gate, run_if, n_rows_dev, ops);
 }
 
 extern "C" int mnn_nade_logprob_fwd_mfma_f32(mnn_stream_t s, int tracks, int N, int D, int Hn, const uint8_t* v, long v_track_stride,
                                              const float* bias, int ld_bias, const float* w_enc, const void* w_dec_packed, const float* row_weight,
                                              float* nll, float* cond_p, float* d_bias, float* a_final, const int* gate, int run_if, const int* n_rows_dev) {
-    return nm_launch<true>(s, tracks, N, D, Hn, v, v_track_stride, bias, ld_bias, w_enc, w_dec_packed, row_weight, nll, cond_p, d_bias, a_final, gate, run_if, n_rows_dev);
+    return nm_launch<true>(s, tracks, N, D, Hn, v, v_track_stride, bias, ld_bias, w_enc, w_dec_packed, row_weight, nll, cond_p, d_bias, a_final, gate, run_if, n_rows_dev, nullptr);
+}
+extern "C" int mnn_nade_logprob_fwd_mfma_f32_ops(mnn_stream_t s, int tracks, int N, int D, int Hn, const uint8_t* v, long v_track_stride,
+                                                 const float* bias, int ld_bias, const float* w_enc, const void* w_dec_packed, const float* row_weight,
+                                                 float* nll, float* cond_p, float* d_bias, float* a_final, const int* gate, int run_if, const int* n_rows_dev,
+                                                 const mnn_nade_ops* ops) {
+    return nm_launch<true>(s, tracks, N, D, Hn, v, v_track_stride, bias, ld_bias, w_enc, w_dec_packed, row_weight, nll, cond_p, d_bias, a_final, gate, run_if, n_rows_dev, ops);
 }
 
 __global__ void __launch_bounds__(256) nade_f32_pack_kernel(const float* __restrict__ w, long n, int Hn, float* __restrict__ out) {
diff --git a/multinn_amd/csrc/nade_ops.h b/multinn_amd/csrc/nade_ops.h
--- /dev/null
+++ b/multinn_amd/csrc/nade_ops.h
@@ -0,0 +1,61 @@
+#pragma once
+#include "common.h"
+
+#ifdef NOPS_NO_ATOMIC
+#define NOPS_ADD(p, x) do { if ((x) == 1.2345e30f) *(p) = (x); } while (0)
+#else
+#define NOPS_ADD(p, x) atomicAdd(p, x)
+#endif
+#define NOPS_ST_T(v, p) __builtin_nontemporal_store(v, p)
+struct NadeOps {
+    h16_t* out_c;
+    h16_t* out_t;
+    float* db;
+    int ld_c, ld_t;
+    int f16;
+    int keep_f32;
+    int slot_mask;
+};
+
+__device__ __forceinline__ h16_t nops_cvt(const NadeOps o, float x) {
+    asm("" : "+v"(x));
+    return o.f16 ? f32_to_f16(x) : f32_to_bf16(x);
+}
+__device__ __forceinline__ uint32_t nops_pack2(const NadeOps o, float a, float b) { return (uint32_t)nops_cvt(o, a) | ((uint32_t)nops_cvt(o, b) << 16); }
+
+__device__ __forceinline__ void nops_zero_block(h16_t* __restrict__ out_c, int ld_c, h16_t* __restrict__ out_t, int ld_t, int col0, int ncol, int row0, int nrow, int N, int nthreads, bool transposed) {
+    if (out_c == nullptr || ncol <= 0) return;
+    const bool pairs = ((col0 | ncol | ld_c) & 1) == 0;
+    for (int n = 0; n < nrow && row0 + n < N; ++n) {
+        h16_t* row = out_c + (size_t)(row0 + n) * ld_c + col0;
+        if (pairs) for (int i = threadIdx.x; 2 * i < ncol; i += nthreads) reinterpret_cast<uint32_t*>(row)[i] = 0u;
+        else for (int i = threadIdx.x; i < ncol; i += nthreads) row[i] = 0;
+    }
+    if (!transposed) return;
+    const int nr2 = nrow >> 1;
+    for (int e = threadIdx.x; e < ncol * nr2; e += nthreads) {
+        const int i = e / nr2, n = e - i * nr2;
+        *reinterpret_cast<uint32_t*>(out_t + (size_t)(col0 + i) * ld_t + row0 + 2 * n) = 0u;
+    }
+}
+
+static inline bool nops_from_abi(const mnn_nade_ops* a, int tracks, int N, int D, int Hn, NadeOps* o, const char** why) {
+    memset(o, 0, sizeof(*o));
+    if (a == nullptr || (a->out_c == nullptr && a->out_t == nullptr && a->db == nullptr)) return true;
+    *why = "out_c, out_t and db come together";
+    if (!(a->out_c && a->out_t && a->db)) return false;
+    *why = "one track, Hn > 64 and a multiple of 8";
+    if (!(tracks == 1 && Hn > 64 && Hn % 8 == 0)) return false;
+    *why = "dtype must be MNN_BF16 or MNN_F16";
+    if (!(a->dtype == MNN_BF16 || a->dtype == MNN_F16)) return false;
+    *why = "ld_c >= tracks (Hn + D) and a multiple of 4, ld_t >= N and a multiple of 64";
+    if (!(a->ld_c >= tracks * (Hn + D) && a->ld_c % 4 == 0 && a->ld_t >= N && a->ld_t % 64 == 0)) return false;
+    *why = "db_slots must be 0 or a power of two up to 1024";
+    if (a->db_slots < 0 || a->db_slots > 1024 || (a->db_slots & (a->db_slots - 1)) != 0) return false;
+    *why = "out_c must be 8-byte aligned, out_t 16-byte aligned";
+    if (((uintptr_t)a->out_c & 7) != 0 || ((uintptr_t)a->out_t & 15) != 0) return false;
+    o->out_c = (h16_t*)a->out_c; o->out_t = (h16_t*)a->out_t; o->db = a->db;
+    o->ld_c = a->ld_c; o->ld_t = a->ld_t; o->f16 = a->dtype == MNN_F16 ? 1 : 0; o->keep_f32 = a->keep_f32;
+    o->slot_mask = a->db_slots > 1 ? a->db_slots - 1 : 0;
+    return true;
+}
diff --git a/multinn_amd/generators.py b/multinn_amd/generators.py
--- a/multinn_amd/generators.py
+++ b/multinn_amd/generators.py
@@ -397,6 +397,7 @@
         self._tracks = getattr(self, "_tracks", ["all"])
         super().__init__(num_dims, num_hidden, num_hidden_rnn, keep_prob, internal_bias, name, track_name, **kw)
         self._num_output = self.num_tracks * self.num_dims
+        self.nade_dense_ops = os.environ.get("MULTINN_NADE_DENSE_OPS", "1") != "0"
 
     tracks = property(lambda self: self._tracks)
     num_tracks = property(lambda self: len(self._tracks))
@@ -457,18 +458,18 @@
 
     nade_dense_above = float(os.environ.get("MULTINN_NADE_DENSE_ABOVE", "0.07"))
 
-    def _nade_fwd(self, v, out, rw, nll, cond_p, d_out, a_fin, n_rows_dev=None, unsafe=None):
+    def _nade_fwd(self, v, out, rw, nll, cond_p, d_out, a_fin, n_rows_dev=None, unsafe=None, dense_ops=None):
         M, D, Hn = self.num_tracks, self.num_dims, self.num_hidden[-1]
         exact = self._nade_exact()
         if self.nade_dense_above >= 1.0:
             return ops.nade_logprob_fwd_auto(v, out, self.store["nade/w_enc"], self.store["nade/w_dec"], self._wdec_bf, M, D, Hn, None, None,
-                                             1.0, rw, nll, cond_p, d_out, a_fin, exact=exact, n_rows_dev=n_rows_dev)
+                                             1.0, rw, nll, cond_p, d_out, a_fin, exact=exact, n_rows_dev=n_rows_dev, dense_ops=dense_ops)
         if getattr(self, "_gate", None) is None or self._gate.device != out.device:
             self._gate = torch.zeros(1 + ops.DENSITY_SLOTS, device=out.device, dtype=torch.int32)
         counted = bool(getattr(self, "_v_counted", False)) and rw is not None
         return ops.nade_logprob_fwd_auto(v, out, self.store["nade/w_enc"], self.store["nade/w_dec"], self._wdec_bf, M, D, Hn, self._gate[:1],
                                          self._gate[1:], self.nade_dense_above, rw, nll, cond_p, d_out, a_fin, exact=exact, counted=counted,
-                                         n_rows_dev=n_rows_dev, unsafe=unsafe)
+                                         n_rows_dev=n_rows_dev, unsafe=unsafe, dense_ops=dense_ops)
 
     nade_exact = os.environ.get("MULTINN_NADE_EXACT_MFMA", "1") != "0"
 
@@ -600,6 +601,13 @@
             if self.ldo != self.n_out and self.dtype == torch.float32:
                 d_out[:, self.n_out:].zero_()
         a_fin = torch.empty((M, N, Hn), device=dev) if train else None
+        dense = None
+        if train and self.nade_dense_ops and self.dtype in ops.H16 and M == 1 and Hn > 64 and Hn % 8 == 0:
+            Np = ops.round_up(N, 64)
+            dense = dict(do_c=torch.empty((N, self.ldo), device=dev, dtype=self.dtype),
+                         doT=(torch.zeros if Np != N else torch.empty)((self.n_out, Np), device=dev, dtype=self.dtype),
+                         db=torch.zeros((64, self.n_out), device=dev))
+        dops = ops.nade_dense_ops(M, N, D, Hn, dense["do_c"], dense["doT"], dense["db"]) if dense else None
         dyn = self.store.ls_dyn if (train and self.dtype == torch.float16) else None
         if compact is not None:
             ls = compact["hdr_f"][2:3] if (train and self.dtype == torch.float16) else 1.0
@@ -621,15 +629,15 @@
                 rw_g = rw_m if gs == 1.0 else rw_m * gs
         if self._nade_mfma():
             unsafe = torch.empty(1, device=dev, dtype=torch.int32) if (train and self.nade_dense_above < 1.0) else None
-            self._nade_fwd(v.view(M, N, D), out, rw_g if train else None, nll, cond_p, d_out, a_fin, n_rows_dev=nrows, unsafe=unsafe)
+            self._nade_fwd(v.view(M, N, D), out, rw_g if train else None, nll, cond_p, d_out, a_fin, n_rows_dev=nrows, unsafe=unsafe, dense_ops=dops)
         else:
             assert compact is None or Hn <= 256, "compacted rows: the f32 scan covers Hn <= 256"
             ops.nade_logprob_fwd(v.view(M, N, D), out, self.store["nade/w_enc"], self.store["nade/w_dec"], M, D, Hn,
-                                 rw_g if train else None, nll, cond_p, d_out, a_fin, n_rows_dev=nrows)
+                                 rw_g if train else None, nll, cond_p, d_out, a_fin, n_rows_dev=nrows, dense_ops=dops)
         loss = torch.zeros(1, device=dev)
         ops.weighted_sum(nll.view(-1), rw_m.repeat(M) if M > 1 else rw_m, loss)
         self._ctx = dict(x_tm=x_tm, v=v, rw=rw_m, y=y, lstm=ctx, out=out, d_out=d_out, a_fin=a_fin, kp=kp, seed=self.seed, B=B, T=T, ls=ls,
-                         compact=compact, unsafe=unsafe if self._nade_mfma() else None)
+                         compact=compact, unsafe=unsafe if self._nade_mfma() else None, dense=dense)
         self._nll_tm, self._cond_tm, self._loss = nll, cond_p, loss
         self._flat_idx = None
         self._lengths = lengths
@@ -693,9 +701,11 @@
         self.store.grad.zero_()
         d_out = cx["d_out"]
         compact = cx.get("compact")
+        dense = cx.get("dense")
         ops.nade_logprob_bwd(cx["v"].view(M, N, D), cx["out"], self.store["nade/w_enc"], self.store["nade/w_dec"], M, D, Hn, cx["a_fin"],
                              d_out, g["nade/w_enc"], g["nade/w_dec"], n_rows_dev=compact["hdr"] if compact else None,
-                             unsafe=cx.get("unsafe"))
+                             unsafe=cx.get("unsafe"),
+                             dense_ops=ops.nade_dense_ops(M, N, D, Hn, dense["do_c"], dense["doT"], dense["db"]) if dense else None)
         Np = ops.round_up(N, 64)
         zalloc = torch.zeros if Np != N else torch.empty
         yT = cx["lstm"][-1].get("yT") if cx["lstm"] else None
@@ -704,8 +714,11 @@
         if yT is None:
             yT = zalloc((R, Np), device=dev, dtype=self.dtype)
             ops.transpose(cx["y"].view(N, R), yT)
-        doT = zalloc((self.n_out, Np), device=dev, dtype=self.dtype)
-        if self.dtype == torch.float32:
+        doT = dense["doT"] if dense else zalloc((self.n_out, Np), device=dev, dtype=self.dtype)
+        if dense:
+            do_c = dense["do_c"]
+            ops.bias_grad(dense["db"], g["dense/bias"], accumulate=True)
+        elif self.dtype == torch.float32:
             ops.transpose(d_out[:, :self.n_out], doT)
             ops.bias_grad(d_out[:, :self.n_out], g["dense/bias"], accumulate=True)
             do_c = d_out
diff --git a/multinn_amd/ops.py b/multinn_amd/ops.py
--- a/multinn_amd/ops.py
+++ b/multinn_amd/ops.py
@@ -491,8 +491,27 @@
     _req(0 < Hn <= 256, "nade: Hn must be in 1..256")
 
 
+def nade_dense_ops(tracks, N, D, Hn, out_c, out_t, db, keep_f32=False):
+    n_out = tracks * (Hn + D)
+    _req(out_c.dtype in H16 and out_t.dtype == out_c.dtype and out_c.dim() == 2 and out_c.shape[0] == N and out_c.stride(1) == 1
+         and out_c.shape[1] >= n_out, "nade ops: out_c 16-bit [N, >= tracks*(Hn+D)]")
+    _req(out_t.dim() == 2 and out_t.shape[0] == n_out and out_t.stride(1) == 1 and out_t.shape[1] >= N and out_t.stride(0) % 64 == 0,
+         "nade ops: out_t 16-bit [tracks*(Hn+D), round_up(N, 64)]")
+    slots = db.shape[0] if db.dim() == 2 else 1
+    _req(db.dtype == torch.float32 and db.is_contiguous() and db.numel() == slots * n_out and slots & (slots - 1) == 0 and slots <= 1024,
+         "nade ops: db f32 [tracks*(Hn+D)] or [slots, tracks*(Hn+D)], slots a power of two")
+    st = _lib.NadeOps()
+    st.out_c, st.ld_c, st.out_t, st.ld_t, st.db = _ptr(out_c), out_c.stride(0), _ptr(out_t), out_t.stride(0), _ptr(db)
+    st.dtype, st.keep_f32, st.db_slots = dtype_code(out_c), 1 if keep_f32 else 0, slots
+    return st
+
+
+def _ops_ref(dense_ops):
+    return None if dense_ops is None else C.byref(dense_ops)
+
+
 def nade_logprob_fwd(v, bias, w_enc, w_dec, tracks, D, Hn, row_weight=None, nll=None, cond_p=None, d_bias=None, a_final=None, n_rows_dev=None,
-                     gate=None, run_if=0, unsafe=None):
+                     gate=None, run_if=0, unsafe=None, dense_ops=None):
     N = bias.shape[0]
     _nade_check(tracks, N, D, Hn, v, bias, w_enc, w_dec)
     if nll is not None:
@@ -507,6 +526,11 @@
     if a_final is not None:
         _req(a_final.dtype == torch.float32 and a_final.numel() == tracks * N * Hn and a_final.is_contiguous(), "nade: a_final f32 [tracks,N,Hn]")
     _req(unsafe is None or (unsafe.dtype == torch.int32 and unsafe.numel() == 1), "nade: unsafe int32[1]")
+    if dense_ops is not None:
+        call("mnn_nade_logprob_fwd_gated_ops", _stream(), tracks, N, D, Hn, _ptr(v), N * D, _ptr(bias), bias.stride(0), _ptr(w_enc), _ptr(w_dec),
+             _ptr(row_weight), _ptr(nll), _ptr(cond_p), _ptr(d_bias), _ptr(a_final), _ptr(gate), int(run_if), _ptr(n_rows_dev), _ptr(unsafe),
+             _ops_ref(dense_ops))
+        return
     if n_rows_dev is not None or gate is not None or unsafe is not None:
         call("mnn_nade_logprob_fwd_gated", _stream(), tracks, N, D, Hn, _ptr(v), N * D, _ptr(bias), bias.stride(0), _ptr(w_enc), _ptr(w_dec),
              _ptr(row_weight), _ptr(nll), _ptr(cond_p), _ptr(d_bias), _ptr(a_final), _ptr(gate), int(run_if), _ptr(n_rows_dev), _ptr(unsafe))
@@ -548,7 +572,7 @@
 
 
 def nade_logprob_fwd_auto(v, bias, w_enc, w_dec, w_dec_bf, tracks, D, Hn, gate, count, dense_above=0.07, row_weight=None, nll=None,
-                          cond_p=None, d_bias=None, a_final=None, exact=False, counted=False, n_rows_dev=None, unsafe=None):
+                          cond_p=None, d_bias=None, a_final=None, exact=False, counted=False, n_rows_dev=None, unsafe=None, dense_ops=None):
     N = bias.shape[0]
     _nade_check(tracks, N, D, Hn, v, bias, w_enc, w_dec)
     _req(w_dec_bf.dtype == (torch.float32 if exact else torch.bfloat16) and w_dec_bf.is_contiguous() and w_dec_bf.numel() == tracks * D * Hn,
@@ -566,6 +590,15 @@
     tail = (_ptr(row_weight), _ptr(nll), _ptr(cond_p), _ptr(d_bias), _ptr(a_final), _ptr(gate))
     mfma = "mnn_nade_logprob_fwd_mfma_f32" if exact else "mnn_nade_logprob_fwd_mfma_gated"
     nr = _ptr(n_rows_dev)
+    if dense_ops is not None:
+        if gate is None:
+            call(mfma + "_ops", _stream(), *common, _ptr(w_dec_bf), *tail, 0, nr, _ops_ref(dense_ops))
+            return
+        call("mnn_density_gate", _stream(), None if counted else _ptr(v), v.numel(), int(dense_above * v.numel()), _ptr(gate), _ptr(count))
+        call(mfma + "_ops", _stream(), *common, _ptr(w_dec_bf), *tail, 0, nr, _ops_ref(dense_ops))
+        _req(unsafe is None or (unsafe.dtype == torch.int32 and unsafe.numel() == 1), "nade auto: unsafe int32[1]")
+        call("mnn_nade_logprob_fwd_gated_ops", _stream(), *common, _ptr(w_dec), *tail, 1, nr, _ptr(unsafe), _ops_ref(dense_ops))
+        return
     if gate is None:
         call(mfma, _stream(), *common, _ptr(w_dec_bf), *tail, 0, nr)
         return
@@ -575,7 +608,7 @@
     call("mnn_nade_logprob_fwd_gated", _stream(), *common, _ptr(w_dec), *tail, 1, nr, _ptr(unsafe))
 
 
-def nade_logprob_bwd(v, bias, w_enc, w_dec, tracks, D, Hn, a_final, d_bias, d_w_enc, d_w_dec, n_rows_dev=None, unsafe=None):
+def nade_logprob_bwd(v, bias, w_enc, w_dec, tracks, D, Hn, a_final, d_bias, d_w_enc, d_w_dec, n_rows_dev=None, unsafe=None, dense_ops=None):
     _req(unsafe is None or (unsafe.dtype == torch.int32 and unsafe.numel() == 1), "nade bwd: unsafe int32[1]")
     N = bias.shape[0]
     _nade_check(tracks, N, D, Hn, v, bias, w_enc, w_dec)
@@ -583,6 +616,10 @@
     for w in (d_w_enc, d_w_dec):
         _req(w.dtype == torch.float32 and w.is_contiguous() and w.numel() == tracks * D * Hn, "nade bwd: grad weights f32 [tracks,D,Hn]")
     _req(a_final.dtype == torch.float32 and a_final.numel() == tracks * N * Hn and a_final.is_contiguous(), "nade bwd: a_final f32 [tracks,N,Hn]")
+    if dense_ops is not None:
+        call("mnn_nade_logprob_bwd_ops", _stream(), tracks, N, D, Hn, _ptr(v), N * D, _ptr(bias), bias.stride(0), _ptr(w_enc), _ptr(w_dec),
+             _ptr(a_final), _ptr(d_bias), _ptr(d_w_enc), _ptr(d_w_dec), _ptr(n_rows_dev), _ptr(unsafe), _ops_ref(dense_ops))
+        return
     call("mnn_nade_logprob_bwd", _stream(), tracks, N, D, Hn, _ptr(v), N * D, _ptr(bias), bias.stride(0), _ptr(w_enc), _ptr(w_dec),
          _ptr(a_final), _ptr(d_bias), _ptr(d_w_enc), _ptr(d_w_dec), _ptr(n_rows_dev), _ptr(unsafe))
 
```
